# skhu101/TDNN-F_NAS

Hardware: AMD Instinct MI355X
Metric: LF-MMI training frames/sec per node (SWBD 7q TDNN-F) (higher is better)
Workload: dtype f32

## Files before the change

### include/tdnnf_hip.h

```cpp
#ifndef TDNNF_HIP_H_
#define TDNNF_HIP_H_

#include <stddef.h>
#include <stdint.h>

#ifdef __cplusplus
extern "C" {
#endif

#define TDNNF_OK 0
#define TDNNF_EINVAL 1
#define TDNNF_EHIP 2

#define TDNNF_MAX_OFFSETS 16

typedef struct {
  float *data;
  int rows, cols, stride;
} tdnnf_mat;

typedef void *tdnnf_stream;
typedef struct tdnnf_ng tdnnf_ng;

const char *tdnnf_last_error(void);
// ... 213 lines not shown
int tdnnf_align_graphs_info(const tdnnf_align_graphs *, int graph, int *num_states, int *num_arcs, int *max_in_degree);
size_t tdnnf_align_workspace_bytes(const tdnnf_align_graphs *, int num_utts, const int *utt_graph, const int *utt_frames);
int tdnnf_align_best_path(const tdnnf_align_graphs *, int num_utts, const int *utt_graph, const int *utt_frames, const int *utt_row_begin,
                          int row_stride, const tdnnf_mat *nnet_output, float acoustic_scale, int *pdf_out_dev, int *state_out_dev,
                          double *results_dev, void *workspace_dev, size_t workspace_bytes, tdnnf_stream);

int tdnnf_align_best_path_labels(const tdnnf_align_graphs *, int num_utts, const int *utt_graph, const int *utt_frames, const int *utt_row_begin,
                                 int row_stride, const tdnnf_mat *nnet_output, float acoustic_scale, int *pdf_out_dev, int *state_out_dev,
                                 int *label_out_dev, int *arc_out_dev , double *results_dev, void *workspace_dev,
                                 size_t workspace_bytes, tdnnf_stream);

size_t tdnnf_align_posteriors_workspace_bytes(const tdnnf_align_graphs *, int num_utts, const int *utt_graph, const int *utt_frames,
                                              int want_posteriors);
int tdnnf_align_posteriors(const tdnnf_align_graphs *, int num_utts, const int *utt_graph, const int *utt_frames, const int *utt_row_begin,
                           int row_stride, const tdnnf_mat *nnet_output, float acoustic_scale, float weight, tdnnf_mat *post_out ,
                           double *results_dev, void *workspace_dev, size_t workspace_bytes, tdnnf_stream);

int tdnnf_align_graphs_pdfs(const tdnnf_align_graphs *, int graph, int *num, int *pdfs_out);
int tdnnf_align_posteriors_compact_layout(const tdnnf_align_graphs *, int num_utts, const int *utt_graph, const int *utt_frames, long long *elems_out,
                                          long long *utt_begin_out);
int tdnnf_align_posteriors_compact(const tdnnf_align_graphs *, int num_utts, const int *utt_graph, const int *utt_frames, const int *utt_row_begin,
                                   int row_stride, const tdnnf_mat *nnet_output, float acoustic_scale, float weight, float *post_compact_dev,
                                   size_t post_compact_elems, double *results_dev, void *workspace_dev, size_t workspace_bytes, tdnnf_stream);

size_t tdnnf_align_posteriors_sparse_workspace_bytes(const tdnnf_align_graphs *, int num_utts, const int *utt_graph, const int *utt_frames,
                                                     int max_per_frame);
int tdnnf_align_posteriors_sparse(const tdnnf_align_graphs *, int num_utts, const int *utt_graph, const int *utt_frames, const int *utt_row_begin,
                                  int row_stride, const tdnnf_mat *nnet_output, float acoustic_scale, float weight, float min_post, int max_per_frame,
                                  int *pdf_out_dev, float *post_out_dev, int *count_out_dev, double *results_dev, void *workspace_dev,
                                  size_t workspace_bytes, tdnnf_stream);

int tdnnf_align_graphs_labels(const tdnnf_align_graphs *, int graph, int *num, int *labels_out);
int tdnnf_align_label_posteriors_compact_layout(const tdnnf_align_graphs *, int num_utts, const int *utt_graph, const int *utt_frames,
                                                long long *elems_out, long long *utt_begin_out);
int tdnnf_align_label_posteriors_compact(const tdnnf_align_graphs *, int num_utts, const int *utt_graph, const int *utt_frames,
                                         const int *utt_row_begin, int row_stride, const tdnnf_mat *nnet_output, float acoustic_scale, float weight,
                                         float *post_compact_dev, size_t post_compact_elems, double *results_dev, void *workspace_dev,
                                         size_t workspace_bytes, tdnnf_stream);
size_t tdnnf_align_label_posteriors_sparse_workspace_bytes(const tdnnf_align_graphs *, int num_utts, const int *utt_graph, const int *utt_frames,
                                                           int max_per_frame);
int tdnnf_align_label_posteriors_sparse(const tdnnf_align_graphs *, int num_utts, const int *utt_graph, const int *utt_frames,
                                        const int *utt_row_begin, int row_stride, const tdnnf_mat *nnet_output, float acoustic_scale, float weight,
                                        float min_post, int max_per_frame, int *label_out_dev, float *post_out_dev, int *count_out_dev,
                                        double *results_dev, void *workspace_dev, size_t workspace_bytes, tdnnf_stream);

int tdnnf_ng_create(int rank, int update_period, float num_samples_history, float alpha, tdnnf_ng **out);
void tdnnf_ng_destroy(tdnnf_ng *);
int tdnnf_ng_freeze(tdnnf_ng *, int freeze);
int tdnnf_ng_precondition(tdnnf_ng *, tdnnf_mat *X, float *scale_host, tdnnf_stream);
size_t tdnnf_ng_stats_pass_workspace_bytes(int rank, int Di, int num_taps, int N);
int tdnnf_ng_stats_pass(const tdnnf_tdnn_indexes *ix, const tdnnf_mat *X, int Di, const float *eff_dev, const float *WT_dev,
                        const float *W_dev, int ldw, const float *bias_dev, tdnnf_mat *H, double *sumsq_dev, int sumsq_cap, int form,
                        void *workspace_dev, size_t workspace_bytes, tdnnf_stream);
const float *tdnnf_ng_scale_dev(const tdnnf_ng *);

size_t tdnnf_constrain_orthonormal_workspace_bytes(int rows, int cols);
int tdnnf_constrain_orthonormal(float scale, float *M_dev, int rows, int cols, int ld, void *workspace_dev,
                                size_t workspace_bytes, tdnnf_stream);
int tdnnf_axpy(const float *x_dev, float a, float *y_dev, size_t n, tdnnf_stream);
int tdnnf_dot(const float *x_dev, const float *y_dev, size_t n, double *result_host, tdnnf_stream);
size_t tdnnf_max_change_workspace_bytes(int num_comp);
int tdnnf_update_with_max_change(float *params_dev, float *delta_dev, int num_comp, const long long *comp_begin_host,
                                 const float *max_change_host, float max_param_change, float max_change_scale,
                                 float scale, int zero_delta, void *workspace_dev, size_t workspace_bytes,
                                 float *info_dev, tdnnf_stream);

int tdnnf_splice_input(const tdnnf_mat *feats, const tdnnf_mat *ivectors, int num_seq, int num_splice,
                       tdnnf_mat *out, tdnnf_stream);
int tdnnf_reorder_rows(const tdnnf_mat *in, int num_seq, int rho, int to_rho, tdnnf_mat *out, tdnnf_stream);

#define TDNNF_NET_MAX_LAYERS 32
typedef struct {
  int feat_dim, ivector_dim, num_pdfs;
  int hidden_dim, prefinal_small_dim;
  int num_layers;
  int bottleneck_dim[TDNNF_NET_MAX_LAYERS];
  int time_stride[TDNNF_NET_MAX_LAYERS];
  float bypass_scale;
  int frames_per_chunk, num_sequences;
  int frame_subsampling;
  float leaky_hmm, xent_regularize, chain_l2_regularize;
  float l2_hidden, l2_output;
  float max_change_hidden, max_change_output, max_param_change;
  float relu_self_repair_scale;
  float batchnorm_stats_scale;
  int darts_num_offsets;
  int darts_flags;
  float darts_temp_proportion;
  int use_natural_gradient;
  int bn_num_choices;
  int bn_choice_dims[8];
  int bn_mode;
  float bn_flops_scale;
  float bn_temp_proportion;
  int cv_update;
  int gemm_precision;
  int use_layer_offsets;
  int offset_left[TDNNF_NET_MAX_LAYERS];
  int offset_right[TDNNF_NET_MAX_LAYERS];
  int use_dropout;
} tdnnf_net_config;
typedef struct tdnnf_net tdnnf_net;

typedef struct tdnnf_egs_reader tdnnf_egs_reader;
typedef struct tdnnf_egs_writer tdnnf_egs_writer;
typedef struct tdnnf_eg tdnnf_eg;
// ... 116 lines not shown
```

### tdnn-f_nas_amd/csrc/abi_ng.hip

```cpp
#include <stdint.h>
#include <string.h>

#include <algorithm>

#include "gemm_f32.h"
#include "ng.h"

using namespace tdnnf;

extern "C" {

const float *tdnnf_ng_scale_dev(const tdnnf_ng *ng) { return ng && ng->dev ? ng->scale_f : nullptr; }

size_t tdnnf_ng_stats_pass_workspace_bytes(int rank, int Di, int num_taps, int N) { return ng_pform_ws_bytes(pad4(rank), Di, num_taps, N) + 64; }

int tdnnf_ng_stats_pass(const tdnnf_tdnn_indexes *ix, const tdnnf_mat *X, int Di, const float *eff, const float *WT, const float *W, int ldw,
                        const float *bias, tdnnf_mat *H, double *sumsq, int sumsq_cap, int use_valu, void *workspace, size_t workspace_bytes,
                        tdnnf_stream stream) {
  TDNNF_REQUIRE(ix && X && X->data && H && H->data && Di > 0 && ix->num_offsets >= 1 && ix->num_offsets <= kMaxSeg && ix->row_stride >= 1,
                "ng_stats_pass: bad arguments");
  const int K = ix->num_offsets, N = H->rows, Rp = H->cols;
  for (int i = 0; i < K; i++)
    TDNNF_REQUIRE(ix->row_offsets[i] >= 0 && (long long)(N - 1) * ix->row_stride + ix->row_offsets[i] < X->rows && Di <= X->cols,
                  "ng_stats_pass: tap %d reads outside X (%d x %d)", i, X->rows, X->cols);
  TDNNF_REQUIRE(!sumsq || sumsq_cap >= rows_gemm_sumsq_blocks(N), "ng_stats_pass: sumsq needs %d entries", rows_gemm_sumsq_blocks(N));
  hipStream_t s = (hipStream_t)stream;
  NgInput in;
  memset(&in, 0, sizeof(in));
  in.x = view(X); in.ix = *ix; in.Di = Di; in.ones = bias ? 1 : 0; in.N = N; in.eff = eff;
  if (use_valu == 2) {
    TDNNF_REQUIRE(W && ldw >= K * Di && sumsq && H->stride == Rp && workspace && ng_pform_ok(Rp, in, workspace_bytes),
                  "ng_stats_pass: the one-pass form takes >= 2 taps of one matrix whole 128-row tiles apart, N %% 128 == 0, N >= 32768, taps x rank <= 64, no coefficients");
    return ng_pform_pass(W, Rp, ldw, bias, in, H->data, sumsq, workspace, s);
  }
  if (use_valu) {
    const NgRowdotArgs v = ng_pass_rowdot_args(WT, Rp, bias, in, H->data, H->stride, sumsq, sumsq_cap);
    TDNNF_REQUIRE(WT && ng_rowdot_ok(v), "ng_stats_pass: the vector-ALU kernel takes rank 20 / 40 / 80 and 16-byte aligned rows");
    TDNNF_HIP(ng_rowdot(v, s));
    return TDNNF_OK;
  }
  TDNNF_REQUIRE(W && ldw >= K * Di, "ng_stats_pass: the MFMA form needs W (rank x ldw)");
  GemmPrecisionScope exact_f32(2);
  TDNNF_HIP(rows_gemm(ng_pass_gemm_args(W, ldw, Rp, bias, in, H->data, H->stride, sumsq), true, s));
  return TDNNF_OK;
}

int tdnnf_ng_create(int rank, int update_period, float num_samples_history, float alpha, tdnnf_ng **out) {
  TDNNF_REQUIRE(out && rank >= 0 && update_period >= 1 && num_samples_history > 0 && alpha >= 0, "ng_create: bad configuration");
  tdnnf_ng *ng = new tdnnf_ng();
  ng->rank = rank;
  ng->Rp = 0;
  ng->update_period = update_period;
  ng->t = 0;
  ng->D = ng->Dp = 0;
  ng->frozen = 0;
  ng->num_samples_history = num_samples_history;
  ng->alpha = alpha;
  ng->epsilon = 1.0e-10f;
  ng->delta = 5.0e-04f;
  ng->rho = 0;
  ng->dev = nullptr;
  ng->pin = nullptr;
  ng->scratch = nullptr;
  ng->scratch_floats = 0;
  ng->pending = 0;
  ng->job_done = 0;
  ng->ev_job = nullptr;
  ng->ev_wait = nullptr;
  ng->must_reorth = false;
  *out = ng;
  return TDNNF_OK;
}

int tdnnf_ng_freeze(tdnnf_ng *ng, int freeze) {
  TDNNF_REQUIRE(ng, "ng_freeze: null object");
  ng->frozen = freeze ? 1 : 0;
  return TDNNF_OK;
}

void tdnnf_ng_destroy(tdnnf_ng *ng) {
  if (!ng) return;
  if (ng->pending) ng_pool_wait(ng);
  hipFree(ng->dev);
  hipHostFree(ng->pin);
  hipFree(ng->scratch);
  if (ng->ev_job) hipEventDestroy(ng->ev_job);
  delete ng;
}

int tdnnf_ng_precondition(tdnnf_ng *ng, tdnnf_mat *X, float *scale_host, tdnnf_stream stream) {
  TDNNF_REQUIRE(ng && mat_ok(X) && X->rows > 0 && X->cols > 0, "ng_precondition: bad arguments");
  hipStream_t s = (hipStream_t)stream;
  NgCallScope scope;
  if (X->cols == 1) {
    if (scale_host) *scale_host = 1.0f;
    return TDNNF_OK;
  }
// ... 37 lines not shown
```

### tdnn-f_nas_amd/csrc/abi_tdnn.hip

```cpp
#include <dlfcn.h>
#include <stdlib.h>
#include <string.h>

#include <string>

#include "common.h"
#include "gemm_f32.h"
#include "planes_gemm.h"

namespace tdnnf {

static thread_local std::string g_last_error;

void set_error(const char *fmt, ...) {
  char buf[1024];
  va_list ap;
  va_start(ap, fmt);
  vsnprintf(buf, sizeof(buf), fmt, ap);
  va_end(ap);
  g_last_error = buf;
}
int hip_status(hipError_t e, const char *what) {
  set_error("HIP error %d (%s) in %s", (int)e, hipGetErrorString(e), what);
  return TDNNF_EHIP;
// ... 4 lines not shown
  return o;
}

namespace {
typedef int (*roctx_push_t)(const char *);
typedef int (*roctx_pop_t)();
roctx_push_t g_roctx_push = nullptr;
roctx_pop_t g_roctx_pop = nullptr;
bool roctx_ready() {
  static const bool ok = [] {
    const char *e = getenv("TDNNF_ROCTX");
    if (e && atoi(e) == 0) return false;
    for (const char *lib : {"librocprofiler-sdk-roctx.so", "librocprofiler-sdk-roctx.so.1", "libroctx64.so", "libroctx64.so.4"}) {
      void *h = dlopen(lib, RTLD_NOW | RTLD_GLOBAL);
      if (!h) continue;
      g_roctx_push = (roctx_push_t)dlsym(h, "roctxRangePushA");
      g_roctx_pop = (roctx_pop_t)dlsym(h, "roctxRangePop");
      if (g_roctx_push && g_roctx_pop) return true;
    }
    return false;
  }();
  return ok;
}
}
TraceRange::TraceRange(const char *name) : on(roctx_ready()) {
  if (on) g_roctx_push(name);
}
TraceRange::~TraceRange() {
  if (on) g_roctx_pop();
}

bool tdnn_rows_ok(const tdnnf_tdnn_indexes *ix, int rows_in, int N) {
  if (!ix || ix->num_offsets < 1 || ix->num_offsets > TDNNF_MAX_OFFSETS || ix->row_stride < 1) return false;
  for (int i = 0; i < ix->num_offsets; i++) {
    const long long need = (long long)ix->row_offsets[i] + (long long)ix->row_stride * N - (ix->row_stride - 1);
    if (ix->row_offsets[i] < 0 || (N > 0 && rows_in < need)) return false;
  }
  return true;
}

}

using namespace tdnnf;

extern "C" {

const char *tdnnf_last_error(void) { return g_last_error.c_str(); }
int tdnnf_abi_version(void) { return 1; }

static int *option_slot(const char *name) {
  Options &o = options();
  if (!name) return nullptr;
  const struct { const char *n; int *p; } table[] = {{"ng_grouped", &o.ng_grouped}, {"ng_fuse", &o.ng_fuse}, {"ng_early_in", &o.ng_early_in},
                                                     {"wgrad_stream", &o.wgrad_stream}, {"gemm_ring", &o.gemm_ring}, {"planes", &o.planes}, {"den_split", &o.den_split}, {"phase_events", &o.phase_events}, {"wgrad_lag", &o.wgrad_lag}, {"ng_bk", &o.ng_bk}, {"ng_valu", &o.ng_valu}, {"ng_pform", &o.ng_pform}, {"planes_group", &o.planes_group}, {"xent_behind_den", &o.xent_behind_den}, {"ng_early_fork", &o.ng_early_fork}, {"ng_diag_skip", &o.ng_diag_skip}, {"wgrad_small", &o.wgrad_small}, {"splitk_per_cu", &o.splitk_per_cu}, {"gemm_alt_taps", &o.gemm_alt_taps}, {"reverse_passes", &o.reverse_passes}, {"splitk_partial_round", &o.splitk_partial_round}, {"wgrad_on_caller", &o.wgrad_on_caller}, {"den_mw_test_abort", &o.den_mw_test_abort}, {"planes_check_bound", &o.planes_check_bound}, {"den_gamma_pairs", &o.den_gamma_pairs}, {"num_form", &o.num_form}, {"align_form", &o.align_form}, {"align_checkpoint", &o.align_checkpoint}, {"align_path_checkpoint", &o.align_path_checkpoint}, {"num_frontier_cap", &o.num_frontier_cap}, {"gemm_arith_test", &o.gemm_arith_test}};
  for (auto &e : table)
    if (strcmp(e.n, name) == 0) return e.p;
  return nullptr;
}
int tdnnf_set_option(const char *name, int value) {
  int *p = option_slot(name);
  TDNNF_REQUIRE(p, "set_option: unknown option '%s' (ng_grouped, ng_fuse, ng_early_in, wgrad_stream, gemm_ring, planes, den_split, align_checkpoint, align_path_checkpoint)", name ? name : "(null)");
  *p = value;
  return TDNNF_OK;
}
int tdnnf_get_option(const char *name, int *value) {
  int *p = option_slot(name);
  TDNNF_REQUIRE(p && value, "get_option: unknown option '%s'", name ? name : "(null)");
  *value = *p;
  return TDNNF_OK;
}

}

namespace tdnnf {
int tdnn_propagate_impl(const tdnnf_tdnn_indexes *ix, const tdnnf_mat *in, const float *W, int ldw, int Do, int Di,
                        const float *bias, const float *eff_coef, int init_mode, int relu, tdnnf_mat *out, tdnnf_stream stream,
                        float *colstats, int *colstats_rows) {
  TDNNF_REQUIRE(mat_ok(in) && mat_ok(out) && W, "tdnn_propagate: bad matrices");
  TDNNF_REQUIRE(Do > 0 && Di > 0 && in->cols == Di && out->cols == Do, "tdnn_propagate: dims: in.cols=%d Di=%d out.cols=%d Do=%d",
                in ? in->cols : -1, Di, out ? out->cols : -1, Do);
  TDNNF_REQUIRE(tdnn_rows_ok(ix, in->rows, out->rows), "tdnn_propagate: input has too few rows for the time offsets");
  TDNNF_REQUIRE(ldw >= ix->num_offsets * Di, "tdnn_propagate: ldw < K*Di");
  TDNNF_REQUIRE(init_mode >= 0 && init_mode <= 2 && (init_mode != 1 || bias), "tdnn_propagate: init_mode 1 needs a bias");
  RowsGemmArgs a;
  memset(&a, 0, sizeof(a));
  a.A = in->data;
  a.lda = (long long)in->stride * ix->row_stride;
  a.B = W;
  a.ldb = ldw;
  a.C = out->data;
  a.ldc = out->stride;
  a.M = out->rows;
  a.N = Do;
  a.bias = bias;
  a.coef = eff_coef;
  a.init_mode = init_mode;
  a.relu = relu;
  a.colstats = colstats;
  a.colstats_rows = colstats_rows;
  a.nseg = ix->num_offsets;
  for (int i = 0; i < a.nseg; i++) {
    a.seg[i].a_off = (long long)ix->row_offsets[i] * in->stride;
    a.seg[i].b_off = (long long)i * Di;
    a.seg[i].klen = Di;
    a.seg[i].m_lo = 0;
    a.seg[i].m_hi = out->rows;
  }
// ... 201 lines not shown
```

### tdnn-f_nas_amd/csrc/common.h

```cpp
#pragma once
#include <hip/hip_runtime.h>
#include <stdarg.h>
#include <stdio.h>

#include "tdnnf_hip.h"

namespace tdnnf {

struct MatView {
  float *data;
  int rows, cols, stride;
};
inline MatView view(const tdnnf_mat *m) { return MatView{m->data, m->rows, m->cols, m->stride}; }

void set_error(const char *fmt, ...);
int hip_status(hipError_t e, const char *what);

inline bool mat_ok(const tdnnf_mat *m) {
  return m && m->rows >= 0 && m->cols >= 0 && m->stride >= m->cols && (m->data || m->rows * m->cols == 0);
}
inline bool same_dim(const tdnnf_mat *a, const tdnnf_mat *b) { return a->rows == b->rows && a->cols == b->cols; }

inline bool vec4_ok(const MatView &m) {
  return (reinterpret_cast<uintptr_t>(m.data) & 15) == 0 && m.stride % 4 == 0 && m.cols % 4 == 0;
}

#define TDNNF_REQUIRE(cond, ...)            \
  do {                                      \
    if (!(cond)) {                          \
      ::tdnnf::set_error(__VA_ARGS__);      \
      return TDNNF_EINVAL;                  \
    }                                       \
  } while (0)

#define TDNNF_HIP(expr)                                         \
  do {                                                          \
    hipError_t e__ = (expr);                                    \
    if (e__ != hipSuccess) return ::tdnnf::hip_status(e__, #expr); \
  } while (0)

#define TDNNF_LAUNCH_CHECK() TDNNF_HIP(hipGetLastError())

struct Options {
  int ng_grouped = 1;
  int ng_fuse = 1;
  int ng_early_in = 1;
  int wgrad_stream = -1;
  int gemm_ring = 1;
  int planes = 1;
  int den_mw_test_abort = 0;
  int planes_group = 1;
  int planes_check_bound = 0;
  int wgrad_lag = 3;
  int wgrad_on_caller = 0;
  int splitk_partial_round = 1;
  int reverse_passes = 0;
  int gemm_alt_taps = 1;
  int splitk_per_cu = 2;
  int wgrad_small = 0;
  int ng_bk = 0;
  int ng_early_fork = 1;
  int xent_behind_den = -1;
  int ng_pform = 1;
  int ng_valu = 0;
  int ng_diag_skip = 0;
  int phase_events = 0;
  int den_split = -1;
  int num_form = 0;
  int gemm_arith_test = 0;
  int num_frontier_cap = 0;
  int align_form = 0;
  int align_checkpoint = 0;
  int align_path_checkpoint = 0;
  int den_gamma_pairs = 0;
};
Options &options();

struct TraceRange {
  explicit TraceRange(const char *name);
  ~TraceRange();
  bool on;
};

__host__ __device__ inline float floor_keep_nan(float x, float f) { return x < f ? f : x; }

inline int grid_for(long long work, int block, int cap = 2048) {
  long long g = (work + block - 1) / block;
  if (g > cap) g = cap;
  if (g < 1) g = 1;
  return (int)g;
}
#ifdef __HIPCC__
template <class T>
struct as_given { typedef T type; };
template <class... P>
__attribute__((visibility("hidden"))) inline hipError_t launch_vec_or_scalar(bool vec, int rows, int cols, void (*k4)(P...), void (*k1)(P...), hipStream_t s, typename as_given<P>::type... args) {
  const long long work = (long long)rows * (vec ? cols / 4 : cols);
  void (*k)(P...) = vec ? k4 : k1;
  hipLaunchKernelGGL(k, dim3(grid_for(work, 256)), dim3(256), 0, s, args...);
  return hipGetLastError();
}
#endif

inline unsigned long long tdnnf_decision(unsigned long long step, unsigned long long k) {
  unsigned long long z = step * 0x9E3779B97F4A7C15ULL + k * 0xBF58476D1CE4E5B9ULL + 0x94D049BB133111EBULL;
  z = (z ^ (z >> 30)) * 0xBF58476D1CE4E5B9ULL;
  z = (z ^ (z >> 27)) * 0x94D049BB133111EBULL;
  return (z ^ (z >> 31)) >> 8;
}

bool log_softmax_propagate_with_aux(const tdnnf_mat *in, tdnnf_mat *out, tdnnf_mat *aux, float aux_scale, hipStream_t s);
float chain_supervision_weight(const tdnnf_supervision *sp);
bool chain_supervision_needs_assign(const tdnnf_supervision *sp);
size_t chain_split_region_bytes(const tdnnf_den_graph *g, int B, int T);
int chain_den(const tdnnf_den_graph *g, const tdnnf_supervision *sp, const tdnnf_mat *y, float leaky, tdnnf_mat *deriv, void *ws, hipStream_t s,
              bool beside_other_work = false, hipStream_t caller_aux = nullptr, hipEvent_t ev_recursions = nullptr, bool *ev_recorded = nullptr);
// ... 25 lines not shown
```

### tdnn-f_nas_amd/csrc/fused.h

```cpp
#pragma once
#include "common.h"

namespace tdnnf {

struct PlanesSink {
  void *P;
  long long R;
  const float *rec;
};
hipError_t bn_apply_bypass(MatView x, const float *memo, int D, int period, MatView prev, float bypass, MatView out, hipStream_t s,
                           const float *mask = nullptr, int B = 1, const PlanesSink *planes = nullptr);

struct BwdPlanes {
  void *P;
  long long R;
  int lead;
  float *rec;
};

struct NgFuse {
  const float *W;
  int Rp, ldw;
  float *H;
  double *part;
  int part_cap;
};
bool bn_relu_bwd_ng_ok(MatView x, MatView dz, MatView d_aff, int Rp);
bool bn_relu_bwd_ng_pays(int rows);

size_t bn_relu_bwd_workspace_bytes(int rows, int cols);
hipError_t bn_relu_bwd(MatView x, MatView dz, float *memo, float target_rms, bool bn_test_mode, double *relu_stats, bool store_relu_stats,
                       bool self_repair, float self_repair_scale, MatView d_aff, float *bias_acc, float bias_scale,
                       void *ws, size_t ws_bytes, hipStream_t s, const float *mask = nullptr, int B = 1,
                       const NgFuse *ng = nullptr,
                       double *oderiv_stats = nullptr,
                       const BwdPlanes *planes = nullptr);

}
```

### tdnn-f_nas_amd/csrc/fused.hip

```cpp
#include <algorithm>

#include "batchnorm.h"
#include "device.h"
#include "ew_dev.h"
#include "fused.h"
#include "gemm_f32.h"
#include "launch_forms.h"
#include "planes_gemm.h"

namespace tdnnf {
namespace {

__device__ __forceinline__ void store_planes4(const PlanesSink &pk, float ps, long long ra, int c, const float (&v)[4]) {
  typedef _Float16 h4 __attribute__((ext_vector_type(4)));
  h4 hi, lo;
#pragma unroll
  for (int j = 0; j < 4; j++) {
    const float w = v[j] * ps;
    hi[j] = (_Float16)w;
    lo[j] = (_Float16)(w - (float)hi[j]);
  }
  const int kb = c >> 4, k = c & 15, half = (k >> 3) ^ (int)((ra >> 3) & 1);
  _Float16 *dst = reinterpret_cast<_Float16 *>(pk.P) + (((long long)kb * 2) * pk.R + ra) * 16 + half * 8 + (k & 7);
  *reinterpret_cast<h4 *>(dst) = hi;
  *reinterpret_cast<h4 *>(dst + pk.R * 16) = lo;
}

template <int VEC, bool PLANES>
__global__ __launch_bounds__(256) void bn_apply_bypass_kernel(MatView x, const float *mean, const float *scale, int D, int period,
                                                              MatView prev, float bypass, MatView out, const float *mask, int B, PlanesSink pk, int rev) {
  const int cv = x.cols / VEC;
  const float ps = PLANES ? pk.rec[0] : 1.0f;
  const int ncb = PLANES ? cv / 8 : 1;
  const long long total = PLANES ? (long long)((x.rows + 7) / 8) * 8 * cv : (long long)x.rows * cv;
  for (long long e0 = blockIdx.x * 256LL + threadIdx.x; e0 < total; e0 += gridDim.x * 256LL) {
    const long long e = rev ? total - 1 - e0 : e0;
    int r, c;
    if (PLANES) {
      const long long blk = e >> 6;
      r = (int)(blk / ncb) * 8 + (int)((e >> 3) & 7);
      c = ((int)(blk % ncb) * 8 + (int)(e & 7)) * VEC;
      if (r >= x.rows) continue;
    } else {
      r = (int)(e / cv);
      c = (int)(e % cv) * VEC;
    }
    const int cd = c % period;
    if (cd >= D) continue;
    float xv[4], pv[4] = {0, 0, 0, 0}, o[4];
    ld(x.data + (long long)r * x.stride + c, xv, VEC == 4);
    if (prev.data) ld(prev.data + (long long)r * prev.stride + c, pv, VEC == 4);
    const float *mk = mask ? mask + (long long)(x.cols > D ? c / period : r % B) * D + cd : nullptr;
    float mu[4], sc[4], mv[4] = {1.f, 1.f, 1.f, 1.f};
    ld(mean + cd, mu, VEC == 4);
    ld(scale + cd, sc, VEC == 4);
    if (mk) ld(mk, mv, VEC == 4);
#pragma unroll
    for (int j = 0; j < VEC; j++) o[j] = (xv[j] - mu[j]) * sc[j] * mv[j] + bypass * pv[j];
    st(out.data + (long long)r * out.stride + c, o, VEC == 4);
    if constexpr (PLANES && VEC == 4) store_planes4(pk, ps, r, c, o);
// ... 272 lines not shown
      }
      *reinterpret_cast<float4 *>(As + (rr + 32 * i) * LD + c4 * 4) = make_float4(o[i][0], o[i][1], o[i][2], o[i][3]);
    }
#pragma unroll
    for (int j = 0; j < NT; j++) {
      const int idx = t + 256 * j, n = idx >> 3, kk = (idx & 7) * 4;
      *reinterpret_cast<float4 *>(Bs + n * LD + kk) = wv[j];
    }
    if (k0 + BK < D) request(k0 + BK);
#pragma unroll
    for (int i = 0; i < 4; i++) {
      const int r = r0 + rr + 32 * i;
      if (FULL || r < x.rows) {
        st(d_aff.data + (long long)r * d_aff.stride + col, o[i], true);
        if constexpr (PLANES) store_planes4(pk, pks, (long long)pk_lead + r, col, o[i]);
      }
    }
#pragma unroll
    for (int j = 0; j < 4; j++) {
      float v = cs[j];
      v += __shfl_xor(v, 8, 64);
      v += __shfl_xor(v, 16, 64);
      v += __shfl_xor(v, 32, 64);
      if (lane < 8) colred[wave][lane * 4 + j] = v;
    }
    __syncthreads();
    {
      const float *as = As + (wave * 32 + li) * LD + lh * 4;
      const float *bs = Bs + li * LD + lh * 4;
#pragma unroll
      for (int kg = 0; kg < BK / 8; kg++) {
        const float4 a = *reinterpret_cast<const float4 *>(as + kg * 8);
#pragma unroll
        for (int j = 0; j < NT; j++) {
          const float4 b = *reinterpret_cast<const float4 *>(bs + j * 32 * LD + kg * 8);
          acc[j] = __builtin_amdgcn_mfma_f32_32x32x2f32(a.x, b.x, acc[j], 0, 0, 0);
          acc[j] = __builtin_amdgcn_mfma_f32_32x32x2f32(a.y, b.y, acc[j], 0, 0, 0);
          acc[j] = __builtin_amdgcn_mfma_f32_32x32x2f32(a.z, b.z, acc[j], 0, 0, 0);
          acc[j] = __builtin_amdgcn_mfma_f32_32x32x2f32(a.w, b.w, acc[j], 0, 0, 0);
        }
      }
    }
    if (t < BK) partial[(long long)blk * D + k0 + t] = (colred[0][t] + colred[1][t]) + (colred[2][t] + colred[3][t]);
    __syncthreads();
  }
#pragma unroll
  for (int j = 0; j < NT; j++) {
    const int n = j * 32 + li;
#pragma unroll
    for (int e = 0; e < 16; e++) {
      const int r = r0 + wave * 32 + (e & 3) + 8 * (e >> 2) + 4 * lh;
      if (n < ng.Rp && r < x.rows) ng.H[(long long)r * ng.Rp + n] = acc[j][e];
    }
  }
  double v = ssq;
  for (int o = 32; o > 0; o >>= 1) v += __shfl_xor(v, o, 64);
  if (lane == 0) red[wave] = v;
  __syncthreads();
  if (t == 0) ng.part[blk] = (red[0] + red[1]) + (red[2] + red[3]);
  if (blk == 0)
    for (int i = gridDim.x + t; i < ng.part_cap; i += 256) ng.part[i] = 0.0;
}

template <int NT, bool MASK, bool PLANES>
__global__ __launch_bounds__(256) void bn_relu_bwd_apply_ng_kernel(MatView x, MatView dz, const float *memo, int D, const double *repair_stats,
                                                                   float self_repair_scale, MatView d_aff, float *partial, const float *mask, int B,
                                                                   NgFuse ng, PlanesSink pk, int pk_lead, int rev) {
  const int blk = rev ? (int)gridDim.x - 1 - (int)blockIdx.x : (int)blockIdx.x;
  if (blk * 128 + 128 <= x.rows)
    bn_relu_bwd_apply_ng_body<NT, MASK, true, PLANES>(x, dz, memo, D, repair_stats, self_repair_scale, d_aff, partial, mask, B, ng, pk, pk_lead, blk);
  else bn_relu_bwd_apply_ng_body<NT, MASK, false, PLANES>(x, dz, memo, D, repair_stats, self_repair_scale, d_aff, partial, mask, B, ng, pk, pk_lead, blk);
}

}

hipError_t bn_apply_bypass(MatView x, const float *memo, int D, int period, MatView prev, float bypass, MatView out, hipStream_t s, const float *mask, int B,
                           const PlanesSink *planes) {
  if (x.rows == 0) return hipSuccess;
  const bool vec = vec4_ok(x) && vec4_ok(out) && (!prev.data || vec4_ok(prev)) && D % 4 == 0 && (reinterpret_cast<uintptr_t>(memo) & 15) == 0 &&
                   (!mask || (reinterpret_cast<uintptr_t>(mask) & 15) == 0);
  const long long work = (long long)x.rows * (vec ? x.cols / 4 : x.cols);
  if (planes && !(vec && x.cols == D && D % 32 == 0 && planes->P && planes->rec)) return hipErrorInvalidValue;
  ProfHbmRange prof(4, 4.0 * x.rows * x.cols * ((prev.data ? 3.0 : 2.0) + (planes ? 1.0 : 0.0)), s);
  const PlanesSink none{nullptr, 0, nullptr};
  const int rev = vec && !planes ? options().reverse_passes & 1 : 0;
  count_fused(kFusedBypassFirst + (planes ? kFusedPlanes : vec ? kFusedVec4 : kFusedScalar) * 8 + (x.cols > D ? kFusedFlagSuper : 0) + (mask ? kFusedFlagMask : 0) +
              (rev ? kFusedFlagRev : 0));
  if (planes) hipLaunchKernelGGL((bn_apply_bypass_kernel<4, true>), dim3(grid_for((long long)((x.rows + 7) / 8) * 8 * (x.cols / 4), 256)), dim3(256), 0, s, x, memo, memo + 2 * D, D, period, prev, bypass, out, mask, B, *planes, 0);
  else if (vec) hipLaunchKernelGGL((bn_apply_bypass_kernel<4, false>), dim3(grid_for(work, 256)), dim3(256), 0, s, x, memo, memo + 2 * D, D, period, prev, bypass, out, mask, B, none, rev);
  else hipLaunchKernelGGL((bn_apply_bypass_kernel<1, false>), dim3(grid_for(work, 256)), dim3(256), 0, s, x, memo, memo + 2 * D, D, period, prev, bypass, out, mask, B, none, 0);
  return hipGetLastError();
}

bool bn_relu_bwd_ng_ok(MatView x, MatView dz, MatView d_aff, int Rp) {
  return vec4_ok(x) && vec4_ok(dz) && vec4_ok(d_aff) && x.cols % 32 == 0 && Rp >= 1 && Rp <= 96 && x.rows >= 1;
}

bool bn_relu_bwd_ng_pays(int rows) {
  const int slots = 2 * device_cus();
  const int blocks = (rows + 127) / 128, rounds = (blocks + slots - 1) / slots;
  return 4 * blocks >= 3 * rounds * slots;
}

size_t bn_relu_bwd_workspace_bytes(int rows, int cols) {
  ColReducePlan p = colreduce_plan(rows, cols);
  const size_t blocks128 = ((size_t)rows + 127) / 128;
// ... 87 lines not shown
```

### tdnn-f_nas_amd/csrc/gemm_f32.h

```cpp
#pragma once
#include <hip/hip_runtime.h>
#include <stddef.h>
#include <stdint.h>
#include <string.h>

#include <vector>

#include "prof.h"

namespace tdnnf {

constexpr int kMaxSeg = 16;

struct GemmSeg {
  long long a_off;
  long long b_off;
  int klen;
  int m_lo, m_hi;
};

struct RowsGemmArgs {
  const float *A;
  long long lda;
  const float *B;
  long long ldb;
  float *C;
  long long ldc;
  int M, N;
  const float *bias;
  const float *coef;
  int init_mode;
  int relu;
  int c_vec;
  const float *add;
  long long ldadd;
  float add_scale;
  int add_lo, add_hi;
  int ksplit;
  int kchunk;
  float *partial;
  double *sumsq;
  int sumsq_cap;
  float *colstats;
  int *colstats_rows;
  int colstats_stride;
  int prec;
  int serial_epilogue;
  int alt_seg_order;
  int nseg;
  GemmSeg seg[kMaxSeg];
  const float *col_scale;
  const float *col_offset;
  int post_add;
  const int *row_map;
};
inline bool rows_gemm_has_post(const RowsGemmArgs &a) { return a.col_scale || a.col_offset || a.post_add || a.row_map; }

struct SplitKScratchOverride {
  float *prev_buf;
  size_t prev_bytes;
  SplitKScratchOverride(float *buf, size_t bytes);
  ~SplitKScratchOverride();
};

struct GemmPrecisionScope {
  int prev;
  explicit GemmPrecisionScope(int prec);
  ~GemmPrecisionScope();
};
int gemm_precision_default();
struct TransposedWeightsScope {
  const float *prev_w, *prev_wt;
  long long prev_n;
  TransposedWeightsScope(const float *w_base, const float *wt_base, long long n);
  ~TransposedWeightsScope();
};
const float *transposed_weights(const float *W);

inline bool aligned16(const void *p) { return (reinterpret_cast<uintptr_t>(p) & 15) == 0; }

inline int rows_gemm_colstats_cap(int M) { return (M + 63) / 64 + 64; }
inline int rows_gemm_sumsq_blocks(int M) { return (M + 127) / 128 > 1024 ? (M + 127) / 128 : 1024; }

hipError_t rows_gemm(const RowsGemmArgs &args, bool b_kcontig, hipStream_t stream);
inline hipError_t rows_gemm_1seg(const float *A, long long lda, const float *B, long long ldb, bool b_kcontig, float *C, long long ldc, int M, int N, int K,
                                 int init_mode, const float *coef, double *sumsq, hipStream_t stream) {
  RowsGemmArgs a;
  memset(&a, 0, sizeof(a));
  a.A = A; a.lda = lda; a.B = B; a.ldb = ldb; a.C = C; a.ldc = ldc; a.M = M; a.N = N;
  a.init_mode = init_mode; a.coef = coef; a.sumsq = sumsq; a.nseg = 1;
  a.seg[0].klen = K; a.seg[0].m_lo = 0; a.seg[0].m_hi = M;
  return rows_gemm(a, b_kcontig, stream);
}

struct RowsGemmGroup;
// ... 28 lines not shown
```

### tdnn-f_nas_amd/csrc/launch_forms.h

```cpp
#pragma once
#include <atomic>

namespace tdnnf {

enum RowsForm {
  kFormPlain,
  kFormRing,
  kFormSplitK,
  kFormPartialS2,
  kFormPartialS8 = kFormPartialS2 + 6,
  kFormMainSplitTail,
  kFormMainPlainTail,
  kFormSumsqPlain,
  kFormSumsqSplitK,
  kFormPost,
  kFormGrouped,
  kRowsForms
};
constexpr int kRowsTiles = 9, kRowsAriths = 3;

template <int WM, int WN, int TM, int TN, int BK>
constexpr int rows_tile_index() {
  constexpr int BM = WM * TM * 32, BN = WN * TN * 32;
  constexpr int t = (BM == 128 && BN == 32 && BK == 32) ? 0 : (BM == 128 && BN == 32 && BK == 64) ? 1 : (BM == 128 && BN == 64 && BK == 32) ? 2
                  : (BM == 128 && BN == 96 && BK == 16) ? 3 : (BM == 128 && BN == 96 && BK == 32) ? 4 : (BM == 128 && BN == 160 && BK == 16) ? 5
                  : (BM == 64 && BN == 128 && BK == 16) ? 6 : (BM == 128 && BN == 128 && BK == 16) ? 7 : (BM == 128 && BN == 128 && BK == 32) ? 8 : -1;
  static_assert(t >= 0, "a rows GEMM tile without a counter: add it here and to kRowsTileNames (launch_forms.hip)");
  return t;
}
constexpr int rows_form_index(int tile, int arith, int form) { return (tile * kRowsAriths + arith) * kRowsForms + form; }

enum {
  kPlanesPlain = kRowsTiles * kRowsAriths * kRowsForms,
  kPlanesMainSplitTail,
  kPlanesMainPlainTail,
  kWgradFirst,
  kWgradPlanes = kWgradFirst + 5 * kRowsAriths,
  kWgradLastSlabs,
  kRowsLastSlices,
  kRowsVec4Launches,
  kRowsScalarLaunches,
  kPlanesAltChunked,
  kLaunchFormCounters
};

std::atomic<long long> *launch_form_counters();
inline void count_form(int index) { launch_form_counters()[index].fetch_add(1, std::memory_order_relaxed); }
inline void note_rows_slices(int ksplit) { launch_form_counters()[kRowsLastSlices].store(ksplit, std::memory_order_relaxed); }
inline void note_wgrad_slabs(int splits) { launch_form_counters()[kWgradLastSlabs].store(splits, std::memory_order_relaxed); }

enum { kFusedVec4, kFusedScalar, kFusedPlanes, kFusedKinds };
constexpr int kFusedFlagSuper = 1, kFusedFlagMask = 2, kFusedFlagRev = 4;
constexpr int kFusedNgFlagMask = 1, kFusedNgFlagPlanes = 2, kFusedNgFlagRev = 4;
enum FusedForm {
  kFusedBypassFirst,
  kFusedReduceFirst = kFusedBypassFirst + kFusedKinds * 8,
  kFusedFinalizeTrain = kFusedReduceFirst + 4,
  kFusedFinalizeTest,
  kFusedApplyFirst,
  kFusedApplyUnrolled = kFusedApplyFirst + kFusedKinds * 4,
  kFusedApplyTail,
  kFusedApplyShortChunk,
  kFusedNgFirst,
  kFusedNgPartialBlock = kFusedNgFirst + 3 * 8,
  kFusedNgFullBlocks,
  kFusedRepair,
  kFusedFormCounters
};
std::atomic<long long> *fused_form_counters();
inline void count_fused(int index) { fused_form_counters()[index].fetch_add(1, std::memory_order_relaxed); }

}
```

### tdnn-f_nas_amd/csrc/launch_forms.hip

```cpp
#include "launch_forms.h"

#include <stdio.h>

#include "common.h"

namespace tdnnf {

std::atomic<long long> *launch_form_counters() {
  static std::atomic<long long> counters[kLaunchFormCounters];
  return counters;
}

std::atomic<long long> *fused_form_counters() {
  static std::atomic<long long> counters[kFusedFormCounters];
  return counters;
}

namespace {
const char *const kFusedKindNames[kFusedKinds] = {"vec4", "scalar", "planes"};
const char *const kRowsTileNames[kRowsTiles] = {"128x32k32", "128x32k64", "128x64k32", "128x96k16", "128x96k32", "128x160k16", "64x128k16", "128x128k16", "128x128k32"};
const char *const kArithNames[kRowsAriths] = {"f32", "bf16x3", "bf16x6"};
const char *const kRowsFormNames[kRowsForms] = {"plain", "ring", "splitk", "partial_s2", "partial_s3", "partial_s4", "partial_s5", "partial_s6", "partial_s7", "partial_s8",
                                                "main_split_tail", "main_plain_tail", "sumsq_plain", "sumsq_splitk", "post", "grouped"};
const char *const kWgradTileNames[5] = {"128x128", "160x128", "128x160", "32x128", "64x64"};
}

}

using namespace tdnnf;

extern "C" {

const char *tdnnf_gemm_launch_form_name(int index) {
  static thread_local char buf[64];
  if (index < 0 || index >= kLaunchFormCounters) return nullptr;
  if (index < kPlanesPlain) {
    const int form = index % kRowsForms, arith = (index / kRowsForms) % kRowsAriths, tile = index / (kRowsForms * kRowsAriths);
    snprintf(buf, sizeof(buf), "rows.%s.%s.%s", kRowsTileNames[tile], kArithNames[arith], kRowsFormNames[form]);
  } else if (index == kPlanesPlain) {
    snprintf(buf, sizeof(buf), "planes.plain");
  } else if (index == kPlanesMainSplitTail) {
    snprintf(buf, sizeof(buf), "planes.main_split_tail");
  } else if (index == kPlanesMainPlainTail) {
    snprintf(buf, sizeof(buf), "planes.main_plain_tail");
  } else if (index < kWgradPlanes) {
    const int i = index - kWgradFirst;
    snprintf(buf, sizeof(buf), "wgrad.%s.%s", kWgradTileNames[i / kRowsAriths], kArithNames[i % kRowsAriths]);
  } else if (index == kWgradPlanes) {
    snprintf(buf, sizeof(buf), "wgrad.planes");
  } else if (index == kWgradLastSlabs) {
    snprintf(buf, sizeof(buf), "wgrad.last_slabs");
  } else if (index == kRowsLastSlices) {
    snprintf(buf, sizeof(buf), "rows.last_slices");
  } else if (index == kRowsVec4Launches) {
    snprintf(buf, sizeof(buf), "rows.launches_vec4");
  } else if (index == kRowsScalarLaunches) {
    snprintf(buf, sizeof(buf), "rows.launches_scalar");
  } else {
    snprintf(buf, sizeof(buf), "planes.alt_chunked");
  }
  return buf;
}

int tdnnf_gemm_launch_forms(long long *counts, int capacity, int reset) {
  std::atomic<long long> *c = launch_form_counters();
  for (int i = 0; i < kLaunchFormCounters; i++) {
    if (counts && i < capacity) counts[i] = c[i].load(std::memory_order_relaxed);
    if (reset) c[i].store(0, std::memory_order_relaxed);
  }
  return kLaunchFormCounters;
}

const char *tdnnf_fused_launch_form_name(int index) {
  static thread_local char buf[64];
  if (index < 0 || index >= kFusedFormCounters) return nullptr;
  if (index < kFusedReduceFirst) {
    const int i = index - kFusedBypassFirst, f = i % 8;
    snprintf(buf, sizeof(buf), "apply_bypass.%s%s%s%s", kFusedKindNames[i / 8], f & kFusedFlagSuper ? ".super" : "", f & kFusedFlagMask ? ".mask" : "",
             f & kFusedFlagRev ? ".rev" : "");
  } else if (index < kFusedFinalizeTrain) {
    const int i = index - kFusedReduceFirst;
    snprintf(buf, sizeof(buf), "bwd.reduce.%s.%s", i & 2 ? "scalar" : "vec4", i & 1 ? "stats" : "nostats");
  } else if (index == kFusedFinalizeTrain) {
    snprintf(buf, sizeof(buf), "bwd.finalize.train");
  } else if (index == kFusedFinalizeTest) {
    snprintf(buf, sizeof(buf), "bwd.finalize.test");
  } else if (index < kFusedApplyUnrolled) {
    const int i = index - kFusedApplyFirst, f = i % 4;
    snprintf(buf, sizeof(buf), "bwd.apply.%s%s%s", kFusedKindNames[i / 4], f & 1 ? ".mask" : "", f & 2 ? ".rev" : "");
  } else if (index == kFusedApplyUnrolled) {
    snprintf(buf, sizeof(buf), "bwd.apply.rows_unrolled");
  } else if (index == kFusedApplyTail) {
    snprintf(buf, sizeof(buf), "bwd.apply.rows_tail");
  } else if (index == kFusedApplyShortChunk) {
    snprintf(buf, sizeof(buf), "bwd.apply.short_last_chunk");
  } else if (index < kFusedNgPartialBlock) {
    const int i = index - kFusedNgFirst, f = i % 8;
    snprintf(buf, sizeof(buf), "bwd.apply_ng.nt%d%s%s%s", i / 8 + 1, f & kFusedNgFlagMask ? ".mask" : "", f & kFusedNgFlagPlanes ? ".planes" : "",
             f & kFusedNgFlagRev ? ".rev" : "");
  } else if (index == kFusedNgPartialBlock) {
    snprintf(buf, sizeof(buf), "bwd.apply_ng.partial_block");
  } else if (index == kFusedNgFullBlocks) {
    snprintf(buf, sizeof(buf), "bwd.apply_ng.full_blocks");
  } else {
    snprintf(buf, sizeof(buf), "bwd.repair");
  }
  return buf;
}

int tdnnf_fused_launch_forms(long long *counts, int capacity, int reset) {
  std::atomic<long long> *c = fused_form_counters();
  for (int i = 0; i < kFusedFormCounters; i++) {
// ... 8 lines not shown
```

### tdnn-f_nas_amd/csrc/net.h

```cpp
#pragma once
#include <hip/hip_runtime.h>

#include <algorithm>
#include <string>
#include <utility>
#include <vector>

#include <map>

#include "batchnorm.h"
#include "common.h"
#include "planes_gemm.h"
#include "tdnnf_hip.h"

namespace tdnnf {
struct RowsGemmGroup;
struct PlanesSplitGroup;

struct NgGroup;
struct NgFin;
struct UpdGroup;

struct Grid {
  int t0, step, n;
// ... 42 lines not shown
  int c_arch, arch_draw0;
  float *arch_p, *arch_mask, *lin_masked;
};

}

struct tdnnf_net {
  tdnnf_net_config cfg = {};
  std::vector<tdnnf::CompDesc> comps;
  long long num_params = 0;
  float *params = nullptr, *grads = nullptr;
  float *paramsT = nullptr;
  int planes_np = 0;
  struct PlaneSlot {
    void *P = nullptr, *PT = nullptr;
    size_t bytesP = 0, bytesPT = 0;
    float *scale = nullptr;
    long long last[5] = {-1, -1, -1, -1, -1};
  };
  std::map<const float *, PlaneSlot> plane_slots;
  std::vector<tdnnf::PlanesOperand> pw;
  std::vector<float *> pw_scale;
  void *planes_ws = nullptr;
  double *fro_buf = nullptr;
  int B = 0, T = 0, Tout = 0;
  tdnnf::Grid g_lda = {}, g_feat = {};
  tdnnf::Tdnn tdnn1 = {};
  std::vector<tdnnf::TdnnfLayer> layers;
  int c_lda = 0, c_prefinal_l = 0;
  struct Head {
    int c_affine = 0, c_linear = 0, c_output = 0;
    float *aff_relu = nullptr, *bn1_out = nullptr, *lin_out = nullptr, *bn2_out = nullptr, *y = nullptr;
    float *bn1_memo = nullptr, *bn2_memo = nullptr;
    double *bn1_stats = nullptr, *bn2_stats = nullptr, *relu_stats = nullptr;
  } head[2];
  float *xent_logsoftmax = nullptr;
  char *arena = nullptr;
  size_t arena_bytes = 0;
  float *lda_in = nullptr, *lda_out = nullptr, *t1_relu = nullptr, *t1_bn = nullptr;
  float *t1_bn_memo = nullptr;
  double *t1_bn_stats = nullptr, *t1_relu_stats = nullptr;
  float *prefinal_l_out = nullptr;
  float *dA = nullptr, *dB = nullptr, *dC = nullptr, *d_small = nullptr, *d_small2 = nullptr;
  float *d_y = nullptr, *d_xent = nullptr;
  float *tapgrad = nullptr;
  double *tapdots = nullptr;
  const float *draws = nullptr;
  std::vector<tdnnf_ng *> ng_in, ng_out;
  float *orthoT = nullptr;
  struct NgComp {
    float *H_in = nullptr, *H_out = nullptr, *T = nullptr, *bsum = nullptr;
    double *part_in = nullptr, *part_out = nullptr;
    int N = 0;
  };
  std::vector<NgComp> ngc;
  float *ng_bsum_all = nullptr;
  size_t ng_bsum_floats = 0;
  float *ngTmp = nullptr;
  void *ng_side_ws = nullptr;
  size_t ngset_ws_bytes = 0;
  struct NgBucket {
    int key;
    std::vector<int> comps;
    tdnnf::NgGroup *group;
  };
  std::vector<NgBucket> ng_buckets;
  std::vector<int> ng_cur;
  tdnnf::NgFin *ngfin = nullptr;
  bool ng_grouped = true;
  hipEvent_t ev_ngc = nullptr;
  hipStream_t s3 = nullptr;
  hipEvent_t ev_s3 = nullptr;
  hipEvent_t ev_fin0 = nullptr, ev_fin = nullptr;
  float *s3_scratch = nullptr;
  size_t s3_scratch_bytes = 0;
  bool wg_on = false;
  hipStream_t s4 = nullptr;
  hipEvent_t ev_pg[4] = {nullptr, nullptr, nullptr, nullptr}, ev_pg_in = nullptr;
  int wg_lag = 3;
  float *dC2 = nullptr, *dS[2] = {nullptr, nullptr};
  unsigned pg_count = 0;
  void *ws4 = nullptr;
  void *ws2 = nullptr;
  float *s2_scratch = nullptr;
  float *s4_scratch = nullptr;
  hipStream_t s5 = nullptr;
  void *ws5 = nullptr;
  float *s5_scratch = nullptr;
  struct EarlyIn {
    unsigned char xin[256];
    long long recorded = -1, done = -1;
  };
  std::vector<EarlyIn> early;
  long long fb_count = 0;
  bool early_on = false, early_any = false;
  bool early_group = false;
  tdnnf::RowsGemmGroup *early_launch = nullptr;
  tdnnf::PlanesSplitGroup *wsplit_group = nullptr;
  hipEvent_t ev_early_in = nullptr, ev_early = nullptr;
  size_t s4_scratch_bytes = 0;
  bool wg_two = false;
  float *gtmp = nullptr;
  std::vector<char> oderiv_nonzero_own;
  std::vector<char> *oderiv_nonzero = &oderiv_nonzero_own;
  tdnnf::BnSync bn_sync{nullptr, nullptr, nullptr, 1};
  enum { kPhases = 8 };
// ... 83 lines not shown
```

### tdnn-f_nas_amd/csrc/net_arena.hip

```cpp
#include <string>

#include "common.h"
#include "fused.h"
#include "gemm_f32.h"
#include "gemm_ring.h"
#include "net_model.h"
#include "ng.h"

namespace tdnnf {
namespace {

struct Rows {
  int N0, No;
  int max_rows;
  int max_lin_rows;
  int big_rows() const { return std::max(max_rows, std::max(N0, No)); }
};
Rows rows_of(const tdnnf_net *n) {
  Rows r{N_of(n->g_lda, n->B), n->Tout * n->B, 0, 0};
  r.max_rows = r.N0;
  for (auto &L : n->layers) {
    r.max_rows = std::max(r.max_rows, std::max(N_of(L.gout, n->B), N_of(L.gin, n->B)));
    r.max_lin_rows = std::max(r.max_lin_rows, N_of(L.lin.out, n->B));
  }
  return r;
}
float *small_mat(const tdnnf_net *n, Arena &A, const Rows &r) {
  return A.mat(std::max(r.max_lin_rows, r.No), std::max(n->cfg.prefinal_small_dim, 512));
}
size_t bsum_floats(const CompDesc &cd) { return ((size_t)cd.rows + 15) & ~(size_t)15; }

void take_activations(tdnnf_net *n, Arena &A, const Rows &r) {
  const tdnnf_net_config &c = n->cfg;
  const int B = n->B, Hd = c.hidden_dim, S = c.prefinal_small_dim, P = c.num_pdfs;
  const int lda_dim = 3 * c.feat_dim + c.ivector_dim;
  n->lda_in = A.mat(r.N0, lda_dim);
  n->lda_out = A.mat(r.N0, lda_dim);
  n->t1_relu = A.mat(r.N0, Hd);
  n->t1_bn = A.mat(r.N0, Hd);
  n->t1_bn_memo = A.take<float>(bn_memo_floats(Hd));
  n->t1_bn_stats = A.take<double>(bn_stats_doubles(Hd));
  n->t1_relu_stats = A.take<double>(relu_stats_doubles(Hd));
  for (auto &L : n->layers) {
    const int nl = N_of(L.lin.out, B), no = N_of(L.gout, B);
    L.lin_out = A.mat(nl, L.bn);
    L.lin_perm = L.perm ? A.mat(nl, L.bn) : nullptr;
    L.arch_p = L.arch_mask = L.lin_masked = nullptr;
    if (L.c_arch >= 0) {
      L.arch_p = A.take<float>(8);
      L.arch_mask = A.take<float>(L.bn + 4);
      L.lin_masked = A.mat(nl, L.bn);
    }
    L.relu_out = A.mat(no, Hd);
    L.noop_out = A.mat(no, Hd);
    L.bn_memo = A.take<float>(bn_memo_floats(Hd));
    L.lin.memo = L.lin.darts ? A.take<float>(2 * TDNNF_MAX_OFFSETS) : nullptr;
    L.aff.memo = L.aff.darts ? A.take<float>(2 * TDNNF_MAX_OFFSETS) : nullptr;
    L.lin.active = L.lin.darts ? A.take<int>(TDNNF_MAX_OFFSETS + 1) : nullptr;
    L.aff.active = L.aff.darts ? A.take<int>(TDNNF_MAX_OFFSETS + 1) : nullptr;
    L.bn_stats = A.take<double>(bn_stats_doubles(Hd));
// ... 87 lines not shown
  slot(n->dC, r.big_rows(), Hd, true);
  slot(n->d_small, small_rows, small_cols, true);
  slot(n->d_small2, small_rows, small_cols, true);
  n->planes_ws = A.take<char>(planes_sumsq_ws_bytes() + 64);
  n->fro_buf = A.take<double>(finalize_grid(std::max(Hd, S)) + 8);
  for (size_t i = 0; i < n->comps.size(); i++) {
    const CompDesc &cd = n->comps[i];
    if (cd.plain || cd.rows < 2 || (int)i == n->c_lda) continue;
    PlanesOperand &o = n->pw[i];
    o.rows = cd.rows; o.cols = cd.cols; o.ld = cd.cols; o.np = np; o.lead = 0;
    o.R = planes_slot_t_rows(cd.rows);
    o.Rt = planes_slot_t_rows(cd.cols);
    o.P = A.take<char>(planes_bytes(np, o.R, planes_kblocks(cd.cols)) + 64);
    o.PT = A.take<char>(planes_bytes(np, o.Rt, planes_t_kblocks(cd.rows)) + 64);
    n->pw_scale[i] = A.take<float>(4);
    o.scale = n->pw_scale[i];
  }
}

size_t take_ortho_transpose(tdnnf_net *n, Arena &A) {
  size_t tall = 0, tall_ws = 0;
  for (auto &cd : n->comps)
    if (cd.orthonormal != 0.f && cd.rows > cd.cols) {
      tall = std::max(tall, (size_t)cd.rows * cd.cols);
      tall_ws = std::max(tall_ws, tdnnf_constrain_orthonormal_workspace_bytes(cd.cols, cd.rows));
    }
  n->orthoT = tall ? A.take<float>(tall + 16) : nullptr;
  return tall_ws;
}

size_t take_natural_gradient(tdnnf_net *n, Arena &A, const Rows &r) {
  n->s3_scratch = nullptr;
  n->s3_scratch_bytes = 0;
  n->ng_grouped = options().ng_grouped != 0;
  n->ngc.assign(n->comps.size(), tdnnf_net::NgComp());
  if (!n->cfg.use_natural_gradient) return 0;
  size_t ng_ws = 0, mtmp = 0;
  for (const WeightComp &w : weight_comps(n)) {
    const CompDesc &cd = n->comps[w.comp];
    if (!cd.updatable || cd.plain) continue;
    const int Dx = cd.cols + (cd.has_bias ? 1 : 0), ldT = (Dx + 3) & ~3, rows = w.rows_out;
    int rank_in, rank_out;
    ng_ranks(cd, &rank_in, &rank_out);
    const int Rpi = (rank_in + 3) & ~3, Rpo = (rank_out + 3) & ~3;
    mtmp = std::max(mtmp, std::max((size_t)cd.rows * Rpi, (size_t)Rpo * ldT));
    ng_ws = std::max(ng_ws, std::max(ng_stats_workspace_bytes(rank_in, Dx, w.K, rows), ng_stats_workspace_bytes(rank_out, cd.rows, 1, rows)));
    auto &C = n->ngc[w.comp];
    C.N = rows;
    C.H_in = A.take<float>((size_t)rows * Rpi + 64);
    C.H_out = A.take<float>((size_t)rows * Rpo + 64);
    C.T = A.take<float>((size_t)cd.rows * ldT + 16);
    C.part_in = A.take<double>((size_t)rows_gemm_sumsq_blocks(rows) + 8);
    C.part_out = A.take<double>((size_t)rows_gemm_sumsq_blocks(rows) + 8);
  }
  size_t tot = 0;
  for (size_t i = 0; i < n->comps.size(); i++)
    if (n->ngc[i].N > 0) tot += bsum_floats(n->comps[i]);
  n->ng_bsum_floats = tot;
  n->ng_bsum_all = A.take<float>(tot + 16);
  size_t o = 0;
  for (size_t i = 0; i < n->comps.size(); i++)
    if (n->ngc[i].N > 0) {
      n->ngc[i].bsum = n->ng_bsum_all ? n->ng_bsum_all + o : nullptr;
      o += bsum_floats(n->comps[i]);
    }
  n->ngset_ws_bytes = wgrad_workspace_bytes(80, 80, 1, r.big_rows()) + 256;
  n->ngTmp = A.take<float>(mtmp + 64);
  n->ng_side_ws = A.take<char>(n->ngset_ws_bytes);
  n->s3_scratch_bytes = 16u << 20;
  n->s3_scratch = A.take<float>(n->s3_scratch_bytes / sizeof(float));
  return ng_ws;
}

void take_workspace(tdnnf_net *n, Arena &A, const Rows &r, size_t ng_ws, size_t tall_ws) {
  const tdnnf_net_config &c = n->cfg;
  const int Hd = c.hidden_dim, S = c.prefinal_small_dim, P = c.num_pdfs;
  size_t ws = 0;
  auto upd = [&](size_t b) { ws = std::max(ws, b); };
  for (const WeightComp &w : weight_comps(n)) {
    const CompDesc &cd = n->comps[w.comp];
    upd(wgrad_workspace_bytes(cd.rows, cd.cols / w.K, w.K, w.rows_out));
  }
  upd(colreduce_bytes(r.max_rows, Hd));
  upd(sizeof(float) * 2 * (size_t)Hd * rows_gemm_colstats_cap(r.big_rows()));
  upd(bn_relu_bwd_workspace_bytes(r.max_rows, Hd));
  for (auto &L : n->layers) upd(tdnnf_constrain_orthonormal_workspace_bytes(L.bn, L.lin.K * Hd));
  upd(colreduce_bytes(r.No, P));
  upd(tdnnf_constrain_orthonormal_workspace_bytes(S, Hd));
  upd(tdnnf_max_change_workspace_bytes((int)n->comps.size()));
  upd(ng_ws);
  upd(tall_ws);
  if (c.bn_num_choices > 0) upd(sizeof(float) * (size_t)((r.max_lin_rows + 511) / 512 + 1) * 512);
  n->ws_bytes = ws + 256;
  n->ws = A.take<char>(n->ws_bytes);
}

void take_side_streams(tdnnf_net *n, Arena &A) {
  n->early_on = n->cfg.use_natural_gradient && n->ng_grouped && (options().ng_early_in >= 2 || (options().ng_early_in != 0 && !n->wg_on));
  n->early_group = n->early_on && n->wg_on && options().ng_early_in == 3;
  const bool s4_used = n->wg_on || n->early_on;
  n->ws4 = s4_used ? A.take<char>(n->ws_bytes) : nullptr;
  n->s4_scratch_bytes = s4_used ? (32u << 20) : 0;
  n->s4_scratch = s4_used ? A.take<float>(n->s4_scratch_bytes / sizeof(float)) : nullptr;
  const bool two = n->wg_on && options().wgrad_stream != 1;
  n->ws2 = two ? A.take<char>(n->ws_bytes) : nullptr;
  n->s2_scratch = two ? A.take<float>(n->s4_scratch_bytes / sizeof(float)) : nullptr;
// ... 44 lines not shown
```

### tdnn-f_nas_amd/csrc/net_step_grad.hip

```cpp
#include "net_step.h"

namespace tdnnf {
namespace {
__global__ void add_scaled_taps_kernel(const float *G, const float *coef, float *acc, int Do, int KDi, int Di) {
  const long long total = (long long)Do * KDi;
  for (long long e = blockIdx.x * 256LL + threadIdx.x; e < total; e += gridDim.x * 256LL) acc[e] += coef[(e % KDi) / Di] * G[e];
}
__global__ void scaled_taps_to_kernel(const float *G, const float *coef, int Do, int KDi, int Di, float *T, int ldT) {
  const long long total = (long long)Do * KDi;
  for (long long e = blockIdx.x * 256LL + threadIdx.x; e < total; e += gridDim.x * 256LL) {
    const int o = (int)(e / KDi), c = (int)(e % KDi);
    T[(size_t)o * ldT + c] = (coef ? coef[c / Di] : 1.0f) * G[e];
  }
}
__global__ void commit_grads_kernel(float *grads, const float *gtmp, long long n, const double *results) {
  if (results[5] == 0.0) return;
  for (long long i = blockIdx.x * 256LL + threadIdx.x; i < n; i += gridDim.x * 256LL) grads[i] += gtmp[i];
}
}

int Step::wait_last_wgrads(hipStream_t st, unsigned streams) {
  for (unsigned b = 1; b <= streams && b <= n->pg_count; b++) TDNNF_HIP(hipStreamWaitEvent(st, n->ev_pg[(n->pg_count - b) & 3], 0));
  return TDNNF_OK;
}
float *Step::bias_target(int comp) const {
  if (n->comps[comp].lr_factor == 0.f) return nullptr;
  if (!use_ng) return net_Bg(n, comp);
  return n->ngc[comp].bsum;
}
Step::WgradSide Step::wgrad_side(bool on_caller) const {
  if (!n->wg_on || on_caller) return {s, n->ws, nullptr};
  const int ns = (n->wg_two ? 2 : 1) + (n->s5 ? 1 : 0), k = (int)(n->pg_count % (unsigned)ns);
  if (k == 0) return {n->s4, n->ws4, n->s4_scratch};
  if (k == 1 && n->wg_two) return {n->s2, n->ws2, n->s2_scratch};
  return {n->s5, n->ws5, n->s5_scratch};
}
int Step::handed_off(hipStream_t sw, bool on_caller) {
  if (!n->wg_on || on_caller) return TDNNF_OK;
  TDNNF_HIP(hipEventRecord(n->ev_pg[n->pg_count & 3], sw));
  const unsigned lag = lag3 ? 3u : 1u;
  if (n->pg_count >= lag) TDNNF_HIP(hipStreamWaitEvent(s, n->ev_pg[(n->pg_count - lag) & 3], 0));
  n->pg_count++;
  return TDNNF_OK;
}
int Step::param_grad(int comp, const tdnnf_tdnn_indexes &ix, int K, int Di, int Do, tdnnf_mat *x, tdnnf_mat *dyv, const float *eff, bool bias_done,
                     const int *active, int max_active, bool from_tapgrad) {
  const int ldw = K * Di;
  float *bias_acc = net_Bg(n, comp);
  if (n->comps[comp].lr_factor == 0.f) return TDNNF_OK;
  const bool on_caller = n->wg_on && options().wgrad_on_caller != 0 && n->early_any && !den_joined;
  if (on_caller) caller_used = true;
  const WgradSide side = wgrad_side(on_caller);
  const hipStream_t sw = side.st;
  void *const wsw = side.ws;
  if (n->wg_on && !on_caller) CK(record_wait(n->ev_pg_in, s, sw));
  SplitKScratchOverride sw_scratch(side.scratch, side.scratch ? n->s4_scratch_bytes : 0);
  if (!use_ng) {
    CK(tdnn_update_simple_impl(&ix, x, dyv, Do, Di, eff, 1.0f, net_Wg(n, comp), ldw, bias_done ? nullptr : bias_acc, wsw, n->ws_bytes, active, max_active, sw));
    return handed_off(sw, on_caller);
  }
  const int N = dyv->rows, ones = bias_acc ? 1 : 0, Dx = ldw + ones, ldT = (Dx + 3) & ~3;
  auto &C = n->ngc[comp];
  TDNNF_REQUIRE(C.T && C.N == N, "net_forward_backward: component %s has no natural-gradient buffers for %d rows", n->comps[comp].name.c_str(), N);
  float *T = C.T;
  const bool grouped = n->ng_grouped && ng_dim(n->ng_in[comp]) != 0 && ng_dim(n->ng_out[comp]) != 0;
  const bool overwrite = !from_tapgrad && !active && eff == nullptr && (ones || ldT == ldw);
  if (!overwrite) TDNNF_HIP(hipMemsetAsync(T, 0, sizeof(float) * (size_t)Do * ldT, sw));
  if (from_tapgrad)
    hipLaunchKernelGGL(scaled_taps_to_kernel, dim3(grid_for((long long)Do * ldw, 256)), dim3(256), 0, sw, n->tapgrad, eff, Do, ldw, Di, T, ldT);
  else
    CK(tdnn_update_simple_impl(&ix, x, dyv, Do, Di, eff, 1.0f, T, ldT, nullptr, wsw, n->ws_bytes, active, max_active, sw, overwrite));
  if (ones) {
    if (!bias_done) TDNNF_HIP(colsum_add(view(dyv), 1.0f, C.bsum, wsw, sw));
    if (!grouped) ng_set_column(C.bsum, Do, T, ldT, ldw, sw);
  }
  NgInput xin;
  memset(&xin, 0, sizeof(xin));
  xin.x = view(x); xin.ix = ix; xin.Di = Di; xin.ones = ones; xin.N = N; xin.eff = eff; xin.active = active; xin.max_active = max_active;
  static_assert(sizeof(NgInput) <= sizeof(tdnnf_net::EarlyIn::xin), "EarlyIn::xin too small");
  if (n->early_on && n->early[comp].done == n->fb_count) {
    TDNNF_REQUIRE(memcmp(n->early[comp].xin, &xin, sizeof(xin)) == 0, "net_forward_backward: the input of component %s moved between minibatches",
                  n->comps[comp].name.c_str());
    if (n->early_group) {
      TDNNF_HIP(hipStreamWaitEvent(sw, n->ev_early, 0));
      CK(ng_stats_main_finish(n->ng_in[comp], xin, C.H_in, wsw, n->ws_bytes, sw));
    }
  } else {
    CK(ng_stats_main(n->ng_in[comp], xin, C.H_in, C.part_in, wsw, n->ws_bytes, sw));
  }
  if (n->early_on) {
    memcpy(n->early[comp].xin, &xin, sizeof(xin));
    n->early[comp].recorded = n->fb_count;
  }
  NgInput yin;
  memset(&yin, 0, sizeof(yin));
  yin.x = view(dyv); yin.ix.row_stride = 1; yin.ix.num_offsets = 1; yin.Di = Do; yin.N = N;
  if (fused_comp == comp) {
    fused_comp = -1;
    CK(ng_stats_main_finish(n->ng_out[comp], yin, C.H_out, wsw, n->ws_bytes, sw));
  } else {
    CK(ng_stats_main(n->ng_out[comp], yin, C.H_out, C.part_out, wsw, n->ws_bytes, sw));
  }
  if (grouped) {
    n->ng_cur.push_back(comp);
  } else {
    CK(record_wait(n->ev_ngc, sw, n->s3));
    SplitKScratchOverride side_scratch(n->s3_scratch, n->s3_scratch_bytes);
    CK(ng_chain_one(n->ng_in[comp], n->ng_out[comp], C.H_in, C.part_in, C.H_out, C.part_out, T, Do, Dx, ldT, ldw, net_Wg(n, comp), bias_acc,
                    n->ng_side_ws, n->ngset_ws_bytes, n->ngTmp, n->s3));
  }
  CK(handed_off(sw, on_caller));
  if (from_tapgrad && n->wg_on) TDNNF_HIP(hipStreamWaitEvent(s, n->ev_pg[(n->pg_count - 1) & 3], 0));
  return TDNNF_OK;
}
int Step::affine_grad(int comp, const PlanesOperand &p_dy, const PlanesOperand &p_x, tdnnf_mat *x, tdnnf_mat *dyv, bool bias_done) {
  PlanesHintScope ph(hint_of(p_dy), hint_of(p_x));
  return param_grad(comp, ix1, 1, x->cols, dyv->cols, x, dyv, nullptr, bias_done, nullptr, 0, false);
}
int Step::tdnn_wgrad(Tdnn &td, const PlanesOperand &p_dy, const PlanesOperand &p_x, tdnnf_mat *x, tdnnf_mat *dyv, const float *eff, bool bias_done) {
  PlanesHintScope ph(hint_of(p_dy), hint_of(p_x));
  const int ldw = td.K * td.Di;
  bool tap_ready = false;
  if (td.darts && !(c.darts_flags & TDNNF_DARTS_UNIFORM_SAMPLE)) {
    tap_ready = true;
    TDNNF_HIP(hipMemsetAsync(n->tapgrad, 0, sizeof(float) * (size_t)td.Do * ldw, s));
    CK(tdnnf_tdnn_update_simple(&td.ix, x, dyv, td.Do, td.Di, nullptr, 1.0f, n->tapgrad, ldw, nullptr, n->ws, n->ws_bytes, s));
    CK(tdnnf_tdnn_darts_alpha_update(n->tapgrad, ldw, net_W(n, td.comp), ldw, td.Do, td.Di, td.K, td.memo, c.darts_flags, td.share,
                                     c.darts_temp_proportion, 1.0f, net_Ag(n, td.comp), n->tapdots, s));
    if (!use_ng) {
      hipLaunchKernelGGL(add_scaled_taps_kernel, dim3(grid_for((long long)td.Do * ldw, 256)), dim3(256), 0, s, n->tapgrad, eff,
                         net_Wg(n, td.comp), td.Do, ldw, td.Di);
      if (!bias_done) TDNNF_HIP(colsum_add(view(dyv), 1.0f, net_Bg(n, td.comp), n->ws, s));
      return TDNNF_OK;
    }
  }
  const bool compact = two_taps(td);
  return param_grad(td.comp, td.ix, td.K, td.Di, td.Do, x, dyv, eff, bias_done, compact ? td.active : nullptr, compact ? 2 : 0, tap_ready);
}
int Step::close_bucket(int key) {
  if (use_ng) CK(ng_close(key));
  for (auto &gb : n->buckets) {
    if (gb.close_key != key) continue;
    hipStream_t cs = s;
    if (!use_ng && n->wg_on && n->pg_count > 0) CK(wait_last_wgrads(s, side_streams()));
    if (use_ng) {
      CK(record_wait(gb.handoff, s, n->s3));
      cs = n->s3;
    }
    const long long cnt = gb.end - gb.begin;
    if (cnt > 0)
      hipLaunchKernelGGL(commit_grads_kernel, dim3(grid_for(cnt, 256)), dim3(256), 0, cs, n->grads + gb.begin, n->gtmp + gb.begin, cnt, results);
    TDNNF_HIP(hipEventRecord(gb.ready, cs));
  }
  return TDNNF_OK;
// ... 21 lines not shown
      early_refresh = early_refresh || did;
    }
  }
  if (early_refresh) TDNNF_HIP(hipEventRecord(n->ev_fin, n->s3));
  return TDNNF_OK;
}
int Step::finish_refreshes() {
  if (use_ng && n->ng_grouped) {
    if (!n->ngfin) {
      bool ready = false;
      for (tdnnf_ng *g : all_ng()) ready = ready || ng_dim(g) != 0;
      if (ready) CK(ng_fin_create(all_ng(), &n->ngfin));
    }
    if (n->ngfin) {
      int did = 0;
      SplitKScratchOverride side_scratch(n->s3_scratch, n->s3_scratch_bytes);
      CK(ng_fin_run(n->ngfin, n->s3, true, &did));
      if (did) {
        TDNNF_HIP(hipEventRecord(n->ev_fin, n->s3));
        early_refresh = true;
      }
    }
  }
  if (early_refresh) TDNNF_HIP(hipStreamWaitEvent(s, n->ev_fin, 0));
  return TDNNF_OK;
}
bool Step::is_head_comp(int comp) const {
  return comp == n->c_prefinal_l || comp == n->head[0].c_affine || comp == n->head[0].c_linear || comp == n->head[0].c_output ||
         comp == n->head[1].c_affine || comp == n->head[1].c_linear || comp == n->head[1].c_output;
}
bool Step::early_eligible(int comp, int which) const {
  const auto &E = n->early[comp];
  if (E.done == n->fb_count || (which == 0 && is_head_comp(comp))) return false;
  if (E.recorded != n->fb_count - 1 || !n->ng_in[comp] || !n->ng_out[comp] || ng_dim(n->ng_in[comp]) == 0 || ng_dim(n->ng_out[comp]) == 0) return false;
  return n->comps[comp].lr_factor != 0.f && n->ngc[comp].H_in;
}
int Step::launch_early_in(int which) {
  if (!(use_ng && n->early_on)) return TDNNF_OK;
  std::vector<int> who;
  for (int comp = (int)n->comps.size() - 1; comp >= 0; comp--)
    if (early_eligible(comp, which)) who.push_back(comp);
  if (who.empty()) return TDNNF_OK;
  CK(record_wait(n->ev_early_in, s, n->s4));
  if (early_refresh) TDNNF_HIP(hipStreamWaitEvent(n->s4, n->ev_fin, 0));
  NgInput xin;
  if (n->early_group) {
    std::vector<RowsGemmArgs> calls;
    std::vector<int> grouped;
    for (int comp : who) {
      memcpy(&xin, n->early[comp].xin, sizeof(xin));
      RowsGemmArgs a;
      CK(ng_stats_main_prepare(n->ng_in[comp], xin, n->ngc[comp].H_in, n->ngc[comp].part_in, n->s4, &a));
      if (!rows_gemm_group_ok(a)) continue;
      calls.push_back(a);
      grouped.push_back(comp);
    }
    if (calls.empty()) return TDNNF_OK;
    TDNNF_HIP(rows_gemm_group(calls, &n->early_launch, n->s4));
    for (int comp : grouped) n->early[comp].done = n->fb_count;
  } else {
    SplitKScratchOverride early_scratch(n->s4_scratch, n->s4_scratch_bytes);
    for (int comp : who) {
      memcpy(&xin, n->early[comp].xin, sizeof(xin));
      CK(ng_stats_main(n->ng_in[comp], xin, n->ngc[comp].H_in, n->ngc[comp].part_in, n->ws4, n->ws_bytes, n->s4));
      n->early[comp].done = n->fb_count;
    }
  }
  TDNNF_HIP(hipEventRecord(n->ev_early, n->s4));
  n->early_any = true;
  return TDNNF_OK;
}
int Step::out_stats_fuse(int comp, MatView xv, MatView dzv, MatView dv, NgFuse &f) {
  fused_comp = -1;
  if (!c.use_natural_gradient || n->ng_out.empty() || !n->ng_out[comp] || n->comps[comp].lr_factor == 0.f) return 0;
  if (options().ng_fuse == 0) return 0;
  const bool fuse_always = options().ng_fuse == 2;
  auto &C = n->ngc[comp];
  const float *W = nullptr;
  int Rp = 0, ldw = 0;
  CK(ng_external_begin(n->ng_out[comp], dv.cols, &W, &Rp, &ldw, s));
  if (!W || !bn_relu_bwd_ng_ok(xv, dzv, dv, Rp) || !(fuse_always || bn_relu_bwd_ng_pays(dv.rows))) return 0;
  f.W = W; f.Rp = Rp; f.ldw = ldw; f.H = C.H_out; f.part = C.part_out; f.part_cap = rows_gemm_sumsq_blocks(dv.rows);
  fused_comp = comp;
  return 1;
}
int Step::ng_close(int key) {
  if (n->ng_cur.empty()) return TDNNF_OK;
  bool closes = false;
  for (auto &gb : n->buckets) closes = closes || gb.close_key == key;
  if (!closes) return TDNNF_OK;
  tdnnf_net::NgBucket *nb = nullptr;
  for (auto &b : n->ng_buckets)
    if (b.key == key) nb = &b;
  if (!nb) {
    std::vector<NgGroupComp> gc;
    for (int comp : n->ng_cur) {
      const CompDesc &cd = n->comps[comp];
      auto &C = n->ngc[comp];
      NgGroupComp g;
      g.in = n->ng_in[comp]; g.out = n->ng_out[comp];
      g.T = C.T; g.Do = cd.rows; g.ldw = cd.cols; g.Dx = cd.cols + (cd.has_bias ? 1 : 0); g.ldT = (g.Dx + 3) & ~3;
      g.bsum = cd.has_bias ? C.bsum : nullptr;
      g.H_in = C.H_in; g.H_out = C.H_out; g.part_in = C.part_in; g.part_out = C.part_out; g.N = C.N;
      g.W_acc = net_Wg(n, comp); g.bias_acc = net_Bg(n, comp);
      gc.push_back(g);
    }
    NgGroup *grp = nullptr;
    CK(ng_group_create(gc, &grp));
    n->ng_buckets.push_back(tdnnf_net::NgBucket{key, n->ng_cur, grp});
    nb = &n->ng_buckets.back();
  }
  TDNNF_REQUIRE(nb->comps == n->ng_cur, "net_forward_backward: the components of gradient bucket %d changed between minibatches", key);
  if (n->wg_on && n->pg_count > 0) {
    CK(wait_last_wgrads(n->s3, side_streams()));
    if (caller_used) CK(record_wait(n->ev_ngc, s, n->s3));
    caller_used = false;
  } else {
    CK(record_wait(n->ev_ngc, s, n->s3));
  }
  if (n->early_any) TDNNF_HIP(hipStreamWaitEvent(n->s3, n->ev_early, 0));
  CK(ng_group_run(nb->group, n->s3));
  n->ng_cur.clear();
  return TDNNF_OK;
}

}
```

### tdnn-f_nas_amd/csrc/ng.h

```cpp
#pragma once
#include <hip/hip_runtime.h>
#include <stddef.h>

#include <vector>

#include "common.h"
#include "gemm_f32.h"
#include "tdnnf_hip.h"

struct tdnnf_ng {
  int rank, Rp, update_period, t, D, Dp, frozen;
  float num_samples_history, alpha, epsilon, delta, rho;
  std::vector<float> d;
  float *dev;
  float *W, *WT, *WWT, *wlast, *J, *W1, *Kd, *Ld, *Ad, *coeff, *tmpR, *neg_one, *scale_f;
  double *scal;
  float *pin;
  float *h_K, *h_L, *h_At, *h_coeff, *h_scale;
  double *h_tr0;
  float *scratch;
  size_t scratch_floats;
  int pending, job_done, job_N;
  hipEvent_t ev_job;
  hipEvent_t ev_wait;
  int device;
  bool cur_upd;
  int cur_N, cur_ones;
  std::vector<float> d_next;
  float rho_next;
  bool must_reorth;
  std::vector<double> sqrt_e1, inv_sqrt_e1;
};

#define TDNNF_NG_LOCAL __attribute__((visibility("hidden")))

namespace tdnnf {

inline int pad4(int x) { return (x + 3) & ~3; }
inline size_t pad4z(size_t x) { return (x + 3) & ~(size_t)3; }

struct NgCallScope {
  ProfClassOverride prof_as_ng{3};
  GemmPrecisionScope exact_f32{2};
};

struct NgInput {
  MatView x;
  tdnnf_tdnn_indexes ix;
  int Di, ones, N;
  const float *eff;
  const int *active;
  int max_active;
};

constexpr int kWtPadRows = 64;
struct NgRowdotArgs {
  const float *X;
  long long ldx;
  int row_stride;
  int nseg, Di;
  long long seg_off[16];
  const float *eff;
  const float *WT;
  int Rp;
  const float *bias;
  float *H;
  int ldh, N;
  double *part;
  int part_cap;
};
bool ng_rowdot_ok(const NgRowdotArgs &a);
hipError_t ng_rowdot(const NgRowdotArgs &a, hipStream_t s);

size_t ng_stats_workspace_bytes(int rank, int D, int K, int N);
int ng_stats_step(tdnnf_ng *ng, const NgInput &in, float *H, void *ws, size_t ws_bytes, hipStream_t s);
int ng_stats_main(tdnnf_ng *ng, const NgInput &in, float *H, double *part, void *ws, size_t ws_bytes, hipStream_t s);
int ng_stats_side(tdnnf_ng *ng, const float *H, const double *part, void *ws, size_t ws_bytes, hipStream_t s);
int ng_stats_main_prepare(tdnnf_ng *ng, const NgInput &in, float *H, double *part, hipStream_t s, RowsGemmArgs *out);
int ng_stats_main_finish(tdnnf_ng *ng, const NgInput &in, const float *H, void *ws, size_t ws_bytes, hipStream_t s);
int ng_finalize_if_ready(tdnnf_ng *ng, hipStream_t s, int *did);
int ng_external_begin(tdnnf_ng *ng, int D, const float **W, int *Rp, int *ldw, hipStream_t s);
int ng_dim(const tdnnf_ng *ng);

size_t ng_project_tmp_floats(const tdnnf_ng *in, const tdnnf_ng *out, int Do, int ldT);
int ng_project(tdnnf_ng *in, tdnnf_ng *out, float *T, int Do, int Dx, int ldT, float *tmp, hipStream_t s);

TDNNF_NG_LOCAL void ng_set_column(const float *v, int rows, float *T, int ldT, int col, hipStream_t s);
TDNNF_NG_LOCAL int ng_chain_one(tdnnf_ng *in, tdnnf_ng *out, const float *H_in, const double *part_in, const float *H_out, const double *part_out,
                                float *T, int Do, int Dx, int ldT, int ldw, float *W_acc, float *bias_acc, void *side_ws, size_t side_ws_bytes, float *tmp, hipStream_t s);

inline bool ng_updating(const tdnnf_ng *ng) { return !ng->frozen && (ng->t <= 10 || (ng->t - 10) % ng->update_period == 0); }
TDNNF_NG_LOCAL int ng_init_default(tdnnf_ng *ng, int D, hipStream_t s);
TDNNF_NG_LOCAL int ng_finalize(tdnnf_ng *ng, hipStream_t s);
TDNNF_NG_LOCAL void ng_refresh_submit(tdnnf_ng *ng, int N, hipEvent_t wait_event);
TDNNF_NG_LOCAL void ng_refresh_installed(tdnnf_ng *ng);
TDNNF_NG_LOCAL RowsGemmArgs ng_pass_gemm_args(const float *W, int ldw, int Rp, const float *bias, const NgInput &in, float *H, int ldh, double *part);
TDNNF_NG_LOCAL NgRowdotArgs ng_pass_rowdot_args(const float *WT, int Rp, const float *bias, const NgInput &in, float *H, int ldh, double *part,
                                                int part_cap);
TDNNF_NG_LOCAL size_t ng_pform_ws_bytes(int Rp, int Di, int K, int N);
TDNNF_NG_LOCAL bool ng_pform_ok(int Rp, const NgInput &in, size_t ws_bytes);
TDNNF_NG_LOCAL int ng_pform_pass(const float *W, int Rp, int ldw, const float *bias, const NgInput &in, float *H, double *part, void *ws, hipStream_t s);


struct NgGroupComp {
  tdnnf_ng *in, *out;
  float *T;
  int Do, Dx, ldT, ldw;
  const float *bsum;
  const float *H_in, *H_out;
  const double *part_in, *part_out;
  int N;
  float *W_acc, *bias_acc;
};
struct NgGroup;
int ng_group_create(const std::vector<NgGroupComp> &comps, NgGroup **out);
void ng_group_destroy(NgGroup *g);
int ng_group_run(NgGroup *g, hipStream_t s);
struct NgFin;
int ng_fin_create(const std::vector<tdnnf_ng *> &objs, NgFin **out);
void ng_fin_destroy(NgFin *f);
int ng_fin_run(NgFin *f, hipStream_t s, bool wait, int *did);
void ng_pool_wait(tdnnf_ng *ng);
bool ng_pool_done(tdnnf_ng *ng);
int ng_finalize_one(tdnnf_ng *ng, hipStream_t s);

}
```

### tdnn-f_nas_amd/csrc/ng_group.hip

```cpp
#include <math.h>
#include <string.h>

#include <algorithm>
#include <vector>

#include "gemm_f32.h"
#include "ggemm.h"
#include "ng.h"
#include "ng_group_kernels.h"

namespace tdnnf {

struct NgGroup {
  std::vector<NgGroupComp> comps;
  std::vector<tdnnf_ng *> objs;
  char *dev = nullptr;
  PairDesc *pairs = nullptr;
  CompDesc *cdesc = nullptr;
  float *lpart = nullptr;
  int npairs = 0, nslabs = 0, commit_blocks = 0;
  size_t l_lds = 0;
  DevList stage[4], kstage;
  hipEvent_t ev_staged = nullptr;
};

int ng_group_create(const std::vector<NgGroupComp> &comps, NgGroup **out) {
  TDNNF_REQUIRE(out && !comps.empty(), "ng_group_create: no components");
  NgGroup *g = new NgGroup();
  g->comps = comps;
  std::vector<PairDesc> pairs;
  std::vector<CompDesc> cdesc;
  GemmList st[4], kst;
  size_t qp_floats = 0;
  std::vector<size_t> q_off, p_off;
  int slab_total = 0, blk = 0;
  for (const NgGroupComp &c : comps) {
    TDNNF_REQUIRE(c.in && c.out && c.in->D == c.Dx && c.in->Dp == c.ldT && c.out->D == c.Do && c.in->rank > 0 && c.out->rank > 0 && c.in->Rp <= 96 &&
                      c.out->Rp <= 96 && c.N > 0,
                  "ng_group_create: a preconditioner is not initialised for its component (or its rank is outside 1..96)");
    q_off.push_back(qp_floats);
    qp_floats += ((size_t)c.Do * c.in->Rp + 63) & ~(size_t)63;
    p_off.push_back(qp_floats);
    qp_floats += ((size_t)c.out->Rp * c.ldT + 63) & ~(size_t)63;
    for (int side = 0; side < 2; side++) {
      tdnnf_ng *ng = side == 0 ? c.in : c.out;
      g->objs.push_back(ng);
      PairDesc p;
      memset(&p, 0, sizeof(p));
      p.H = side == 0 ? c.H_in : c.H_out;
      p.part = side == 0 ? c.part_in : c.part_out;
      p.Ld = ng->Ld;
      p.WWT = ng->WWT;
      p.scal = ng->scal;
      p.scale_f = ng->scale_f;
      p.Kd = ng->Kd;
      TDNNF_HIP(hipHostGetDevicePointer((void **)&p.hK, ng->h_K, 0));
      TDNNF_HIP(hipHostGetDevicePointer((void **)&p.hL, ng->h_L, 0));
      TDNNF_HIP(hipHostGetDevicePointer((void **)&p.h_tr0, ng->h_tr0, 0));
      p.ones_term = (side == 0 && c.bsum) ? (double)c.N : 0.0;
      p.N = c.N;
      p.Rp = ng->Rp;
      p.nt = (ng->Rp + 31) / 32;
      p.npart = rows_gemm_sumsq_blocks(c.N);
      int rps = std::max(256, (c.N + 31) / 32);
      rps = (rps + 7) & ~7;
      p.rows_per_slab = rps;
      p.nslab = (c.N + rps - 1) / rps;
      p.slab0 = slab_total;
      slab_total += p.nslab;
      pairs.push_back(p);
      kst.add(ng->J, ng->Dp, 1, ng->J, 1, ng->Dp, ng->Kd, ng->Rp, ng->Rp, ng->Rp, ng->Dp, 1.0f, 0);
    }
    CompDesc d;
    memset(&d, 0, sizeof(d));
    d.T = c.T;
    d.bsum = c.bsum;
    d.sa = c.in->scale_f;
    d.sb = c.out->scale_f;
    d.W_acc = c.W_acc;
    d.bias_acc = c.bias_acc;
    d.Do = c.Do;
    d.ldT = c.ldT;
    d.ldw = c.ldw;
    d.Dx = c.Dx;
    d.blk0 = blk;
    blk += (int)(((long long)c.Do * c.Dx + 1023) / 1024);
    cdesc.push_back(d);
  }
  g->npairs = (int)pairs.size();
  g->nslabs = slab_total;
  g->commit_blocks = blk;
  size_t bytes = 0;
  bytes = carve_room(bytes, sizeof(PairDesc) * pairs.size());
  bytes = carve_room(bytes, sizeof(CompDesc) * cdesc.size());
  bytes = carve_room(bytes, sizeof(float) * (size_t)slab_total * kLSlabFloats);
  bytes = carve_room(bytes, sizeof(float) * qp_floats);
  auto build = [&](float *qp) {
    for (auto &l : st) l = GemmList();
    for (size_t i = 0; i < comps.size(); i++) {
      const NgGroupComp &c = comps[i];
      float *Q = qp + q_off[i], *P = qp + p_off[i];
      const int Rx = c.in->Rp, Ry = c.out->Rp;
      st[0].add(c.T, c.ldT, 1, c.in->WT, Rx, 1, Q, Rx, c.Do, Rx, c.Dx, 1.0f, 0);
      st[1].add(Q, Rx, 1, c.in->W, c.in->Dp, 1, c.T, c.ldT, c.Do, c.ldT, Rx, -1.0f, 1);
      st[2].add(c.out->W, c.out->Dp, 1, c.T, c.ldT, 1, P, c.ldT, Ry, c.ldT, c.Do, 1.0f, 0);
      st[3].add(c.out->WT, Ry, 1, P, c.ldT, 1, c.T, c.ldT, c.Do, c.ldT, Ry, -1.0f, 1);
    }
  };
  build(nullptr);
  GemmList *lists[5] = {&st[0], &st[1], &st[2], &st[3], &kst};
  DevList *dls[5] = {&g->stage[0], &g->stage[1], &g->stage[2], &g->stage[3], &g->kstage};
  bytes = devlists_room(bytes, lists, 5) + 1024;
  if (hipMalloc((void **)&g->dev, bytes) != hipSuccess) {
    set_error("ng_group_create: cannot allocate %zu bytes", bytes);
    delete g;
    return TDNNF_EHIP;
  }
  char *cur = g->dev;
  g->pairs = carve<PairDesc>(cur, pairs.size());
  g->cdesc = carve<CompDesc>(cur, cdesc.size());
  g->lpart = carve<float>(cur, (size_t)slab_total * kLSlabFloats);
  float *qp = carve<float>(cur, qp_floats);
  build(qp);
  int rc = devlists_upload(cur, lists, dls, 5);
  if (rc) return rc;
  TDNNF_HIP(hipMemcpy(g->pairs, pairs.data(), sizeof(PairDesc) * pairs.size(), hipMemcpyHostToDevice));
  TDNNF_HIP(hipMemcpy(g->cdesc, cdesc.data(), sizeof(CompDesc) * cdesc.size(), hipMemcpyHostToDevice));
  TDNNF_HIP(hipEventCreateWithFlags(&g->ev_staged, hipEventDisableTiming | hipEventBlockingSync));
  g->l_lds = sizeof(float) * 2 * kLSlabFloats;
  static bool attr_done = false;
  if (!attr_done) {
    (void)hipFuncSetAttribute((const void *)ng_l_partial_kernel, hipFuncAttributeMaxDynamicSharedMemorySize, (int)g->l_lds);
    attr_done = true;
  }
  *out = g;
  return TDNNF_OK;
}

void ng_group_destroy(NgGroup *g) {
  if (!g) return;
  for (tdnnf_ng *ng : g->objs)
    if (ng->pending && ng->ev_wait == g->ev_staged) ng_pool_wait(ng);
  if (g->ev_staged) (void)hipEventDestroy(g->ev_staged);
  (void)hipFree(g->dev);
  delete g;
}

int ng_group_run(NgGroup *g, hipStream_t s) {
  TDNNF_REQUIRE(g, "ng_group_run: null group");
  const int nc = (int)g->comps.size();
  const bool upd = g->objs[0]->cur_upd;
  for (tdnnf_ng *ng : g->objs)
    TDNNF_REQUIRE(ng->cur_upd == upd && ng->cur_N > 0 && !ng->pending, "ng_group_run: the group's preconditioners are out of step");
  hipLaunchKernelGGL(ng_set_columns_kernel, dim3(nc), dim3(256), 0, s, g->cdesc);
  hipLaunchKernelGGL(ng_l_partial_kernel, dim3(g->nslabs), dim3(256), g->l_lds, s, g->pairs, g->npairs, g->lpart);
  hipLaunchKernelGGL(ng_l_finish_kernel, dim3(g->npairs), dim3(1024), 0, s, g->pairs, g->lpart);
  if (upd) {
    int rc = launch_list(g->kstage, s);
    if (rc) return rc;
    hipLaunchKernelGGL(ng_stage_kernel, dim3(g->npairs), dim3(256), 0, s, g->pairs);
    TDNNF_HIP(hipEventRecord(g->ev_staged, s));
  }
  for (int i = 0; i < 4; i++) {
    int rc = launch_list(g->stage[i], s);
    if (rc) return rc;
  }
  hipLaunchKernelGGL(ng_commit_group_kernel, dim3(g->commit_blocks), dim3(256), 0, s, g->cdesc, nc);
  TDNNF_LAUNCH_CHECK();
  for (tdnnf_ng *ng : g->objs) {
    if (upd) ng_refresh_submit(ng, ng->cur_N, g->ev_staged);
    ng->cur_N = 0;
    ng->t += 1;
  }
  return TDNNF_OK;
}

struct NgFin {
  std::vector<tdnnf_ng *> objs;
  char *dev = nullptr;
  FinDesc *fd = nullptr;
  int nf = 0, blocks = 0;
  DevList w1, wwt;
};

int ng_fin_create(const std::vector<tdnnf_ng *> &objs_in, NgFin **out) {
  TDNNF_REQUIRE(out, "ng_fin_create: null argument");
  NgFin *f = new NgFin();
  for (tdnnf_ng *ng : objs_in)
    if (ng && ng->rank > 0 && ng->D != 0) f->objs.push_back(ng);
  std::vector<FinDesc> fd;
  GemmList w1, wwt;
  int blk = 0;
  for (tdnnf_ng *ng : f->objs) {
    FinDesc d;
    d.J = ng->J; d.W = ng->W; d.W1 = ng->W1; d.WT = ng->WT; d.wlast = ng->wlast;
    TDNNF_HIP(hipHostGetDevicePointer((void **)&d.h_coeff, ng->h_coeff, 0));
    d.Rp = ng->Rp; d.D = ng->D; d.Dp = ng->Dp;
    d.blk0 = blk;
    blk += (int)(((long long)ng->Rp * ng->Dp + 1023) / 1024);
    fd.push_back(d);
    float *hAt = nullptr;
    TDNNF_HIP(hipHostGetDevicePointer((void **)&hAt, ng->h_At, 0));
    w1.add(hAt, ng->Rp, 1, ng->J, ng->Dp, 1, ng->W1, ng->Dp, ng->Rp, ng->Dp, ng->Rp, 1.0f, 0);
    wwt.add(ng->W, ng->Dp, 1, ng->W, 1, ng->Dp, ng->WWT, ng->Rp, ng->Rp, ng->Rp, ng->Dp, 1.0f, 0);
  }
  f->nf = (int)fd.size();
  f->blocks = blk;
  if (f->nf == 0) {
    *out = f;
    return TDNNF_OK;
  }
  GemmList *lists[2] = {&w1, &wwt};
  DevList *dls[2] = {&f->w1, &f->wwt};
  const size_t bytes = devlists_room(carve_room(0, sizeof(FinDesc) * fd.size()), lists, 2) + 1024;
  if (hipMalloc((void **)&f->dev, bytes) != hipSuccess) {
    set_error("ng_fin_create: cannot allocate %zu bytes", bytes);
    delete f;
    return TDNNF_EHIP;
  }
  char *cur = f->dev;
  f->fd = carve<FinDesc>(cur, fd.size());
  int rc = devlists_upload(cur, lists, dls, 2);
  if (rc) return rc;
  TDNNF_HIP(hipMemcpy(f->fd, fd.data(), sizeof(FinDesc) * fd.size(), hipMemcpyHostToDevice));
  *out = f;
  return TDNNF_OK;
}
// ... 43 lines not shown
```

### tdnn-f_nas_amd/csrc/ng_group_kernels.h

```cpp
#pragma once
#include <hip/hip_runtime.h>
#include <math.h>

#include "ggemm.h"

namespace tdnnf {
namespace {

struct PairDesc {
  const float *H;
  const double *part;
  float *Ld;
  const float *WWT;
  double *scal;
  float *scale_f;
  const float *Kd;
  float *hK, *hL;
  double *h_tr0;
  double ones_term;
  int N, Rp, nt, npart;
  int slab0, nslab, rows_per_slab;
};
__device__ __forceinline__ int ntile_pairs(int nt) { return nt * (nt + 1) / 2; }
constexpr int kLSlabFloats = 6 * 1024;

template <auto Start, class Desc>
__device__ __forceinline__ int last_start_le(const Desc *d, int n, int blk) {
  int lo = 0, hi = n - 1;
  while (lo < hi) {
    const int mid = (lo + hi + 1) >> 1;
    if (d[mid].*Start <= blk) lo = mid;
    else hi = mid - 1;
  }
  return lo;
}

template <int NT>
__device__ __forceinline__ void l_partial_body(const PairDesc &p, int slab, float *partial, float *lds) {
  constexpr int NP = NT * (NT + 1) / 2;
  const int t = threadIdx.x, lane = t & 63, wave = t >> 6, li = lane & 31, lh = lane >> 5;
  const int Rp = p.Rp, r0 = slab * p.rows_per_slab, r1 = min(p.N, r0 + p.rows_per_slab);
  f32x16 acc[NP];
#pragma unroll
  for (int q = 0; q < NP; q++)
#pragma unroll
    for (int r = 0; r < 16; r++) acc[q][r] = 0.f;
  bool cv[NT];
#pragma unroll
  for (int c = 0; c < NT; c++) cv[c] = c * 32 + li < Rp;
  constexpr int U = 4;
  for (int base = r0 + 2 * wave; base < r1; base += 8 * U) {
    float a[U][NT];
#pragma unroll
    for (int u = 0; u < U; u++) {
      const int row = base + 8 * u + lh;
      const float *h = p.H + (size_t)row * Rp + li;
#pragma unroll
      for (int c = 0; c < NT; c++) a[u][c] = (row < r1 && cv[c]) ? h[c * 32] : 0.f;
    }
#pragma unroll
    for (int u = 0; u < U; u++) {
      int q = 0;
#pragma unroll
      for (int i = 0; i < NT; i++)
#pragma unroll
        for (int j = i; j < NT; j++, q++) acc[q] = __builtin_amdgcn_mfma_f32_32x32x2f32(a[u][i], a[u][j], acc[q], 0, 0, 0);
    }
  }
  float *mine = lds + (size_t)(wave & 1) * NP * 1024;
  if (wave >= 2) {
#pragma unroll
    for (int q = 0; q < NP; q++)
#pragma unroll
      for (int r = 0; r < 16; r++) mine[(q * 16 + r) * 64 + lane] = acc[q][r];
  }
  __syncthreads();
  if (wave < 2) {
#pragma unroll
    for (int q = 0; q < NP; q++)
#pragma unroll
      for (int r = 0; r < 16; r++) acc[q][r] += mine[(q * 16 + r) * 64 + lane];
  }
  __syncthreads();
  if (wave == 1) {
#pragma unroll
    for (int q = 0; q < NP; q++)
#pragma unroll
      for (int r = 0; r < 16; r++) lds[(q * 16 + r) * 64 + lane] = acc[q][r];
  }
  __syncthreads();
  if (wave == 0) {
    float *out = partial + (size_t)(p.slab0 + slab) * kLSlabFloats;
#pragma unroll
    for (int q = 0; q < NP; q++)
#pragma unroll
      for (int r = 0; r < 16; r++) out[(q * 16 + r) * 64 + lane] = acc[q][r] + lds[(q * 16 + r) * 64 + lane];
  }
}

__global__ __launch_bounds__(256) void ng_l_partial_kernel(const PairDesc *pairs, int npairs, float *partial) {
  extern __shared__ float lds[];
  const PairDesc &p = pairs[last_start_le<&PairDesc::slab0>(pairs, npairs, (int)blockIdx.x)];
  const int slab = blockIdx.x - p.slab0;
  if (p.nt == 1) l_partial_body<1>(p, slab, partial, lds);
  else if (p.nt == 2) l_partial_body<2>(p, slab, partial, lds);
  else l_partial_body<3>(p, slab, partial, lds);
}

__global__ __launch_bounds__(1024) void ng_l_finish_kernel(const PairDesc *pairs, const float *partial) {
  __shared__ double red[3][16];
  const PairDesc &p = pairs[blockIdx.x];
  const int t = threadIdx.x, Rp = p.Rp, nt = p.nt;
  double a = 0, b = 0, c = 0;
  for (int i = t; i < p.npart; i += 1024) a += p.part[i];
  int q = 0;
  for (int ti = 0; ti < nt; ti++)
    for (int tj = ti; tj < nt; tj++, q++) {
      const int e = t, r = e >> 6, lane = e & 63;
      const int m = ti * 32 + (r & 3) + 8 * (r >> 2) + 4 * (lane >> 5), n = tj * 32 + (lane & 31);
      if (m >= Rp || n >= Rp) continue;
      const float *src = partial + (size_t)p.slab0 * kLSlabFloats + (size_t)q * 1024 + e;
      float v = 0.f;
      int s = 0;
      for (; s + 7 < p.nslab; s += 8) {
        float w[8];
#pragma unroll
        for (int u = 0; u < 8; u++) w[u] = src[(size_t)(s + u) * kLSlabFloats];
#pragma unroll
        for (int u = 0; u < 8; u++) v += w[u];
      }
      for (; s < p.nslab; s++) v += src[(size_t)s * kLSlabFloats];
      p.Ld[m * Rp + n] = v;
      const double w = (double)v * (double)p.WWT[m * Rp + n];
      if (ti != tj) {
        p.Ld[n * Rp + m] = v;
        c += 2.0 * w;
      } else {
        c += w;
        if (m == n) b += v;
      }
    }
  for (int o = 32; o > 0; o >>= 1) {
    a += __shfl_xor(a, o, 64);
    b += __shfl_xor(b, o, 64);
    c += __shfl_xor(c, o, 64);
  }
  if ((t & 63) == 0) {
    red[0][t >> 6] = a;
    red[1][t >> 6] = b;
    red[2][t >> 6] = c;
  }
  __syncthreads();
  if (t == 0) {
    double tr0 = p.ones_term, trL = 0, trLW = 0;
    for (int w = 0; w < 16; w++) {
      tr0 += red[0][w];
      trL += red[1][w];
      trLW += red[2][w];
    }
    const double tr1 = tr0 - 2.0 * trL + trLW;
    p.scal[0] = tr0;
    p.scal[1] = tr1;
    *p.scale_f = (tr0 <= 0.0 || !(tr1 > 0.0)) ? 1.0f : (float)sqrt(tr0 / tr1);
  }
}

__global__ __launch_bounds__(256) void ng_stage_kernel(const PairDesc *pairs) {
  const PairDesc &p = pairs[blockIdx.x];
  const int n = p.Rp * p.Rp;
  for (int i = threadIdx.x; i < n; i += 256) {
    p.hK[i] = p.Kd[i];
    p.hL[i] = p.Ld[i];
  }
  if (threadIdx.x == 0) *p.h_tr0 = p.scal[0];
}

struct CompDesc {
  float *T;
  const float *bsum, *sa, *sb;
  float *W_acc, *bias_acc;
  int Do, ldT, ldw, Dx;
  int blk0;
};
__global__ __launch_bounds__(256) void ng_set_columns_kernel(const CompDesc *comps) {
// ... 62 lines not shown
```

### tdnn-f_nas_amd/csrc/ng_kernels.h

```cpp
#pragma once
#include <hip/hip_runtime.h>

#include "gemm_f32.h"

namespace tdnnf {
namespace {

__global__ void stack_taps_kernel(const float *W, int Rp, int Dp, int Di, int K, float *WP) {
  const long long total = (long long)K * Rp * Di;
  for (long long e = blockIdx.x * 256LL + threadIdx.x; e < total; e += gridDim.x * 256LL) {
    const int k = (int)(e % Di), ir = (int)(e / Di), i = ir / Rp, r = ir % Rp;
    WP[e] = W[(size_t)r * Dp + (size_t)i * Di + k];
  }
}
struct PformTaps {
  int K, o[kMaxSeg];
};
__global__ __launch_bounds__(256) void pform_combine_kernel(const float *P, int ldp, PformTaps tp, int Rp, const float *bias, float *H, int N,
                                                            const double *psum, double *part, int part_cap) {
  const int m0 = blockIdx.x * 128, per = Rp / 4;
  for (int e = threadIdx.x; e < 128 * per; e += 256) {
    const int m = m0 + e / per, q = e % per;
    if (m >= N) break;
    float4 v = make_float4(0.f, 0.f, 0.f, 0.f);
    if (bias) v = *reinterpret_cast<const float4 *>(bias + 4 * q);
    for (int i = 0; i < tp.K; i++) {
      const float4 t = *reinterpret_cast<const float4 *>(P + (size_t)(m + tp.o[i]) * ldp + i * Rp + 4 * q);
      v.x += t.x; v.y += t.y; v.z += t.z; v.w += t.w;
    }
    *reinterpret_cast<float4 *>(H + (size_t)m * Rp + 4 * q) = v;
  }
  if (threadIdx.x == 0) {
    double sacc = 0;
    for (int i = 0; i < tp.K; i++) sacc += psum[blockIdx.x + tp.o[i] / 128];
    part[blockIdx.x] = sacc;
  }
  for (int i = gridDim.x + blockIdx.x * 256 + threadIdx.x; i < part_cap; i += gridDim.x * 256) part[i] = 0.0;
}
__global__ void scatter_col_kernel(const float *v, int R, float *J, int ld, int col) {
  const int r = blockIdx.x * blockDim.x + threadIdx.x;
  if (r < R) J[(size_t)r * ld + col] = v[r];
}
__global__ __launch_bounds__(256) void ng_scalars_kernel(const double *partial, int nb, double ones_term, const float *L, const float *WWT,
                                                         int Rp, double *scal, float *scale_f) {
  __shared__ double red[3][4];
  double a = 0, b = 0, c = 0;
  for (int i = threadIdx.x; i < nb; i += 256) a += partial[i];
  for (int i = threadIdx.x; i < Rp * Rp; i += 256) {
    const double l = L[i];
    c += l * (double)WWT[i];
    if (i / Rp == i % Rp) b += l;
  }
  for (int o = 32; o > 0; o >>= 1) {
    a += __shfl_xor(a, o, 64);
    b += __shfl_xor(b, o, 64);
    c += __shfl_xor(c, o, 64);
  }
  if ((threadIdx.x & 63) == 0) {
    red[0][threadIdx.x >> 6] = a;
    red[1][threadIdx.x >> 6] = b;
    red[2][threadIdx.x >> 6] = c;
  }
  __syncthreads();
  if (threadIdx.x == 0) {
    const double tr0 = (red[0][0] + red[0][1]) + (red[0][2] + red[0][3]) + ones_term;
    const double trL = (red[1][0] + red[1][1]) + (red[1][2] + red[1][3]);
    const double trLW = (red[2][0] + red[2][1]) + (red[2][2] + red[2][3]);
    const double tr1 = tr0 - 2.0 * trL + trLW;
    scal[0] = tr0;
    scal[1] = tr1;
    *scale_f = (tr0 <= 0.0 || !(tr1 > 0.0)) ? 1.0f : (float)sqrt(tr0 / tr1);
  }
}

__global__ void set_column_kernel(const float *v, int rows, float *T, int ldT, int col) {
  const int r = blockIdx.x * blockDim.x + threadIdx.x;
  if (r < rows) {
    T[(size_t)r * ldT + col] = v[r];
    for (int c = col + 1; c < ldT; c++) T[(size_t)r * ldT + c] = 0.f;
  }
}
__global__ void ng_commit_kernel(const float *T, int ldT, int Do, int ldw, const float *sa, const float *sb, float *W_acc, float *bias_acc) {
  const float sc = sa[0] * sb[0];
// ... 13 lines not shown
```

### tdnn-f_nas_amd/csrc/ng_stats.hip

```cpp
#include <string.h>

#include <algorithm>

#include "gemm_f32.h"
#include "ng.h"
#include "ng_kernels.h"

namespace tdnnf {
namespace {

size_t part_bytes(int N) { return ((size_t)rows_gemm_sumsq_blocks(N) * sizeof(double) + 63) & ~(size_t)63; }
size_t stats_ws_bytes(int Rp, int Di, int K, int N) {
  return part_bytes(N) + std::max(std::max(wgrad_workspace_bytes(Rp, Rp, 1, N), wgrad_workspace_bytes(Rp, Di, K, N)), ng_pform_ws_bytes(Rp, Di, K, N));
}

constexpr int kPformSpanCap = 4096;
struct TapSpan {
  int lo, hi;
};
TapSpan tap_span(const tdnnf_tdnn_indexes &ix) {
  TapSpan t{ix.row_offsets[0], ix.row_offsets[0]};
  for (int i = 1; i < ix.num_offsets; i++) {
    t.lo = std::min(t.lo, ix.row_offsets[i]);
    t.hi = std::max(t.hi, ix.row_offsets[i]);
  }
  return t;
}

}

size_t ng_pform_ws_bytes(int Rp, int Di, int K, int N) {
  if (K < 2 || K * Rp > 64) return 0;
  const size_t M = (size_t)N + kPformSpanCap;
  return sizeof(float) * ((size_t)K * Rp * Di + 64) + sizeof(float) * (M * K * Rp + 64) + sizeof(double) * ((size_t)rows_gemm_sumsq_blocks((int)M) + 8) + 256;
}
bool ng_pform_ok(int Rp, const NgInput &in, size_t ws_bytes) {
  const int K = in.ix.num_offsets, N = in.N;
  if (!options().ng_pform || K < 2 || K * Rp > 64 || in.eff || in.active || in.ix.row_stride != 1 || N % 128 != 0 || N < 32768) return false;
  const TapSpan sp = tap_span(in.ix);
  for (int i = 0; i < K; i++)
    if ((in.ix.row_offsets[i] - sp.lo) % 128 != 0) return false;
  if (sp.hi - sp.lo > kPformSpanCap || in.Di % 4 != 0 || (in.x.stride % 4) != 0 || in.Di < 1024) return false;
  return ws_bytes >= ng_pform_ws_bytes(Rp, in.Di, K, N);
}
int ng_pform_pass(const float *W, int Rp, int ldw, const float *bias, const NgInput &in, float *H, double *part, void *ws, hipStream_t s) {
  const int K = in.ix.num_offsets, N = in.N, Di = in.Di;
  const TapSpan sp = tap_span(in.ix);
  PformTaps tp;
  memset(&tp, 0, sizeof(tp));
  tp.K = K;
  for (int i = 0; i < K; i++) tp.o[i] = in.ix.row_offsets[i] - sp.lo;
  const int M = N + (sp.hi - sp.lo);
  float *WP = (float *)ws;
  float *P = WP + (((size_t)K * Rp * Di + 63) & ~(size_t)63);
  double *psum = (double *)(P + (((size_t)M * K * Rp + 63) & ~(size_t)63));
  hipLaunchKernelGGL(stack_taps_kernel, dim3(grid_for((long long)K * Rp * Di, 256)), dim3(256), 0, s, W, Rp, ldw, Di, K, WP);
  TDNNF_HIP(rows_gemm_1seg(in.x.data + (size_t)sp.lo * in.x.stride, in.x.stride, WP, Di, true, P, K * Rp, M, K * Rp, Di, 2, nullptr, psum, s));
  hipLaunchKernelGGL(pform_combine_kernel, dim3(N / 128), dim3(256), 0, s, P, K * Rp, tp, Rp, bias, H, N, psum, part,
                     rows_gemm_sumsq_blocks(N));
  TDNNF_HIP(hipGetLastError());
  return TDNNF_OK;
}

RowsGemmArgs ng_pass_gemm_args(const float *W, int ldw, int Rp, const float *bias, const NgInput &in, float *H, int ldh, double *part) {
  const int N = in.N, K = in.ix.num_offsets, Di = in.Di;
  RowsGemmArgs a;
  memset(&a, 0, sizeof(a));
  a.A = in.x.data; a.lda = (long long)in.x.stride * in.ix.row_stride; a.B = W; a.ldb = ldw; a.C = H; a.ldc = ldh; a.M = N; a.N = Rp;
  a.bias = bias;
  a.init_mode = bias ? 1 : 2;
  a.coef = in.eff;
  a.sumsq = part;
  a.nseg = K;
  for (int i = 0; i < K; i++) {
    a.seg[i].a_off = (long long)in.ix.row_offsets[i] * in.x.stride;
    a.seg[i].b_off = (long long)i * Di;
    a.seg[i].klen = Di;
    a.seg[i].m_lo = 0;
    a.seg[i].m_hi = N;
  }
  return a;
}
NgRowdotArgs ng_pass_rowdot_args(const float *WT, int Rp, const float *bias, const NgInput &in, float *H, int ldh, double *part, int part_cap) {
  const int K = in.ix.num_offsets;
  NgRowdotArgs v;
  memset(&v, 0, sizeof(v));
  v.X = in.x.data; v.ldx = in.x.stride; v.row_stride = in.ix.row_stride; v.nseg = K; v.Di = in.Di; v.eff = in.eff; v.WT = WT; v.Rp = Rp;
  v.bias = bias; v.H = H; v.ldh = ldh; v.N = in.N; v.part = part; v.part_cap = part_cap;
  for (int i = 0; i < K; i++) v.seg_off[i] = (long long)in.ix.row_offsets[i] * in.x.stride;
  return v;
}

namespace {

const float *ones_column(const tdnnf_ng *ng, const NgInput &in) { return in.ones ? ng->wlast : nullptr; }

int stats_after_h(tdnnf_ng *ng, const NgInput &in, const float *H, void *wg_ws, size_t wg_bytes, bool upd, hipStream_t s) {
  const int N = in.N, K = in.ix.num_offsets, Di = in.Di, Rp = ng->Rp, Dp = ng->Dp, D = ng->D;
  ng->cur_upd = upd;
  ng->cur_N = N;
  ng->cur_ones = in.ones;
  if (!upd) return TDNNF_OK;
  TDNNF_REQUIRE(wg_ws && wg_bytes >= wgrad_workspace_bytes(Rp, Di, K, N), "ng: workspace too small");
  TDNNF_HIP(hipMemsetAsync(ng->J, 0, sizeof(float) * (size_t)Rp * Dp, s));
  if (in.ones) TDNNF_HIP(hipMemsetAsync(ng->tmpR, 0, sizeof(float) * Rp, s));
  WgradArgs j;
  memset(&j, 0, sizeof(j));
  j.dY = H; j.lddy = Rp; j.X = in.x.data; j.ldx = in.x.stride; j.Do = Rp; j.Di = Di; j.K = K; j.N = N; j.row_stride = in.ix.row_stride;
  for (int i = 0; i < K; i++) j.row_offsets[i] = in.ix.row_offsets[i];
  j.coef = in.eff; j.scale = 1.f; j.G = ng->J; j.ldg = Dp; j.accumulate = 1; j.bias_acc = in.ones ? ng->tmpR : nullptr;
  j.active = in.active; j.max_active = in.max_active;
  TDNNF_HIP(wgrad(j, wg_ws, wg_bytes, s));
  if (in.ones) hipLaunchKernelGGL(scatter_col_kernel, dim3((Rp + 63) / 64), dim3(64), 0, s, ng->tmpR, Rp, ng->J, Dp, D - 1);
  return TDNNF_OK;
}

int stats_main(tdnnf_ng *ng, const NgInput &in, float *H, double *part, void *wg_ws, size_t wg_bytes, bool upd, hipStream_t s) {
  const int N = in.N, K = in.ix.num_offsets, Di = in.Di, Rp = ng->Rp, Dp = ng->Dp;
  const float *bias = ones_column(ng, in);
  const NgRowdotArgs v = ng_pass_rowdot_args(ng->WT, Rp, bias, in, H, Rp, part, rows_gemm_sumsq_blocks(N));
  const int skip = options().ng_diag_skip;
  if (skip && ng->D != 0 && (((skip & 1) && K == 2 && Di >= 1024) || ((skip & 2) && !(K == 2 && Di >= 1024)))) {
    TDNNF_HIP(hipMemsetAsync(H, 0, sizeof(float) * (size_t)N * Rp, s));
    TDNNF_HIP(hipMemsetAsync(part, 0, sizeof(double) * rows_gemm_sumsq_blocks(N), s));
  } else if (ng_pform_ok(Rp, in, wg_bytes)) {
    int rc = ng_pform_pass(ng->W, Rp, Dp, bias, in, H, part, wg_ws, s);
    if (rc) return rc;
  } else if (options().ng_valu && !in.active && ng_rowdot_ok(v)) {
    TDNNF_HIP(ng_rowdot(v, s));
  } else {
    TDNNF_HIP(rows_gemm(ng_pass_gemm_args(ng->W, Dp, Rp, bias, in, H, Rp, part), true, s));
  }
  return stats_after_h(ng, in, H, wg_ws, wg_bytes, upd, s);
}

int stats_side(tdnnf_ng *ng, const float *H, const double *part, void *wg_ws, size_t wg_bytes, hipStream_t s) {
  const int N = ng->cur_N, Rp = ng->Rp, Dp = ng->Dp;
  TDNNF_REQUIRE(wg_ws && wg_bytes >= wgrad_workspace_bytes(Rp, Rp, 1, N), "ng: workspace too small");
  WgradArgs w;
  memset(&w, 0, sizeof(w));
  w.dY = H; w.lddy = Rp; w.X = H; w.ldx = Rp; w.Do = Rp; w.Di = Rp; w.K = 1; w.N = N; w.row_stride = 1; w.scale = 1.f;
  w.G = ng->Ld; w.ldg = Rp; w.accumulate = 0;
  TDNNF_HIP(wgrad(w, wg_ws, wg_bytes, s));
  hipLaunchKernelGGL(ng_scalars_kernel, dim3(1), dim3(256), 0, s, part, rows_gemm_sumsq_blocks(N), ng->cur_ones ? (double)N : 0.0, ng->Ld, ng->WWT,
                     Rp, ng->scal, ng->scale_f);
  if (!ng->cur_upd) return TDNNF_OK;
  TDNNF_HIP(rows_gemm_1seg(ng->J, Dp, ng->J, Dp, true, ng->Kd, Rp, Rp, Rp, Dp, 2, nullptr, nullptr, s));
  const size_t fRR = (size_t)Rp * Rp;
  TDNNF_HIP(hipMemcpyAsync(ng->h_K, ng->Kd, sizeof(float) * fRR, hipMemcpyDeviceToHost, s));
  TDNNF_HIP(hipMemcpyAsync(ng->h_L, ng->Ld, sizeof(float) * fRR, hipMemcpyDeviceToHost, s));
  TDNNF_HIP(hipMemcpyAsync(ng->h_tr0, ng->scal, sizeof(double), hipMemcpyDeviceToHost, s));
  TDNNF_HIP(hipEventRecord(ng->ev_job, s));
  ng_refresh_submit(ng, N, ng->ev_job);
  return TDNNF_OK;
}

int stats_core(tdnnf_ng *ng, const NgInput &in, float *H, void *ws, size_t ws_bytes, bool upd, hipStream_t s) {
  TDNNF_REQUIRE(ws && ws_bytes >= stats_ws_bytes(ng->Rp, in.Di, in.ix.num_offsets, in.N), "ng: workspace too small");
  double *part = (double *)ws;
  void *wg_ws = (char *)ws + part_bytes(in.N);
  const size_t wg_bytes = ws_bytes - part_bytes(in.N);
  int rc = stats_main(ng, in, H, part, wg_ws, wg_bytes, upd, s);
  if (rc) return rc;
  return stats_side(ng, H, part, wg_ws, wg_bytes, s);
}

int init_from(tdnnf_ng *ng, const NgInput &in, int D, float *H, void *ws, size_t ws_bytes, hipStream_t s) {
  int rc = ng_init_default(ng, D, s);
  if (rc) return rc;
  if (ng->rank > 0) {
    const int iters = in.N <= ng->rank ? 1 : 3;
    for (int i = 0; i < iters; i++) {
      if ((rc = stats_core(ng, in, H, ws, ws_bytes, true, s))) return rc;
      if ((rc = ng_finalize(ng, s))) return rc;
    }
  }
  ng->t = 0;
  return TDNNF_OK;
}

int input_dim(const NgInput &in) { return in.ix.num_offsets * in.Di + (in.ones ? 1 : 0); }

struct NgFirstUse {
  const NgInput &in;
  float *H;
  void *ws;
  size_t ws_bytes;
};
int begin_call(tdnnf_ng *ng, int D, const NgFirstUse *first, bool reset_cur_N, hipStream_t s) {
  if (ng->D == 0 && first) {
    int rc = init_from(ng, first->in, D, first->H, first->ws, first->ws_bytes, s);
    if (rc) return rc;
  }
  TDNNF_REQUIRE(ng->D == D, "ng: dimension changed from %d to %d", ng->D, D);
  if (reset_cur_N) ng->cur_N = 0;
  return ng_finalize(ng, s);
}

}

size_t ng_stats_workspace_bytes(int rank, int D, int K, int N) {
  const int Rp = pad4(std::max(1, std::min(rank, D - 1)));
  const int Di = K > 0 ? D / K : D;
  return stats_ws_bytes(Rp, Di, std::max(K, 1), N) + 64;
}
int ng_dim(const tdnnf_ng *ng) { return ng->D; }

int ng_stats_step(tdnnf_ng *ng, const NgInput &in, float *H, void *ws, size_t ws_bytes, hipStream_t s) {
  const int K = in.ix.num_offsets;
  TDNNF_REQUIRE(ng && H && in.N > 0 && K >= 1 && K <= kMaxSeg && in.Di > 0, "ng_stats_step: bad arguments");
  NgCallScope scope;
  const NgFirstUse first{in, H, ws, ws_bytes};
  int rc = begin_call(ng, input_dim(in), &first, false, s);
  if (rc || ng->rank == 0) return rc;
  rc = stats_core(ng, in, H, ws, ws_bytes, ng_updating(ng), s);
  ng->t += 1;
  return rc;
}

int ng_stats_main(tdnnf_ng *ng, const NgInput &in, float *H, double *part, void *ws, size_t ws_bytes, hipStream_t s) {
  const int K = in.ix.num_offsets;
  TDNNF_REQUIRE(ng && H && part && in.N > 0 && K >= 1 && K <= kMaxSeg && in.Di > 0, "ng_stats_main: bad arguments");
  NgCallScope scope;
  const NgFirstUse first{in, H, ws, ws_bytes};
  int rc = begin_call(ng, input_dim(in), &first, true, s);
  if (rc || ng->rank == 0) return rc;
  return stats_main(ng, in, H, part, ws, ws_bytes, ng_updating(ng), s);
}

int ng_stats_main_prepare(tdnnf_ng *ng, const NgInput &in, float *H, double *part, hipStream_t s, RowsGemmArgs *out) {
  const int K = in.ix.num_offsets, D = input_dim(in);
  TDNNF_REQUIRE(ng && H && part && out && in.N > 0 && K >= 1 && K <= kMaxSeg && ng->D == D, "ng_stats_main_prepare: bad arguments");
  if (ng->rank == 0) {
    memset(out, 0, sizeof(*out));
    ng->cur_N = 0;
    return TDNNF_OK;
  }
  NgCallScope scope;
  int rc = begin_call(ng, D, nullptr, true, s);
  if (rc) return rc;
  *out = ng_pass_gemm_args(ng->W, ng->Dp, ng->Rp, ones_column(ng, in), in, H, ng->Rp, part);
  return TDNNF_OK;
}
int ng_stats_main_finish(tdnnf_ng *ng, const NgInput &in, const float *H, void *ws, size_t ws_bytes, hipStream_t s) {
  TDNNF_REQUIRE(ng && H && ng->D != 0 && ng->rank > 0 && in.N > 0, "ng_stats_main_finish: bad arguments");
  NgCallScope scope;
  return stats_after_h(ng, in, H, ws, ws_bytes, ng_updating(ng), s);
}

int ng_external_begin(tdnnf_ng *ng, int D, const float **W, int *Rp, int *ldw, hipStream_t s) {
  TDNNF_REQUIRE(ng && W && Rp && ldw, "ng_external_begin: bad arguments");
  *W = nullptr;
  if (ng->D == 0 || ng->rank == 0) return TDNNF_OK;
  int rc = begin_call(ng, D, nullptr, true, s);
  if (rc) return rc;
  *W = ng->W;
  *Rp = ng->Rp;
  *ldw = ng->Dp;
  return TDNNF_OK;
}

int ng_stats_side(tdnnf_ng *ng, const float *H, const double *part, void *ws, size_t ws_bytes, hipStream_t s) {
  TDNNF_REQUIRE(ng && H && part, "ng_stats_side: bad arguments");
  if (ng->rank == 0 || ng->cur_N == 0) return TDNNF_OK;
  NgCallScope scope;
  int rc = stats_side(ng, H, part, ws, ws_bytes, s);
  ng->t += 1;
  return rc;
}

size_t ng_project_tmp_floats(const tdnnf_ng *in, const tdnnf_ng *out, int Do, int ldT) {
  const size_t q = in ? (size_t)Do * in->Rp : 0, p = out ? (size_t)out->Rp * ldT : 0;
  return std::max(q, p) + 16;
}

int ng_project(tdnnf_ng *in, tdnnf_ng *out, float *T, int Do, int Dx, int ldT, float *tmp, hipStream_t s) {
  TDNNF_REQUIRE(T && tmp && ldT % 4 == 0 && ldT >= Dx, "ng_project: bad arguments");
  NgCallScope scope;
  if (in && in->rank > 0) {
    TDNNF_REQUIRE(in->D == Dx && in->Dp == ldT, "ng_project: input-side dimension mismatch");
// ... 30 lines not shown
```

### tdnn-f_nas_amd/csrc/rows_gemm.hip

```cpp
#include <algorithm>
#include <cstring>
#include <vector>

#include "colreduce.h"
#include "common.h"
#include "device.h"
#include "gemm_f32.h"
#include "gemm_ring.h"
#include "launch_forms.h"
#include "planes_gemm.h"
#include "rows_gemm_kernels.h"

namespace tdnnf {
namespace {

float *g_scratch_override = nullptr;
size_t g_scratch_override_bytes = 0;
int g_gemm_prec = 0;
const float *g_tw_w = nullptr, *g_tw_wt = nullptr;
long long g_tw_n = 0;

struct KRange {
  long long ktot;
  bool k4;
// ... 215 lines not shown
    at.C = a.C + (long long)m_main * a.ldc;
    for (int i = 0; i < at.nseg; i++) {
      at.seg[i].m_lo -= m_main;
      at.seg[i].m_hi -= m_main;
    }
    at.add_lo -= m_main;
    at.add_hi -= m_main;
    if (stats) {
      at.colstats = a.colstats + (long long)main_mt * a.N;
      at.colstats_stride = am.colstats_stride;
    }
    if (tail_split) {
      {
        ProfScope ps(cls, flops * at.M / a.M, s);
        launch_split_k<WM, WN, TM, TN, BK>(at, (at.M + BM - 1) / BM, ntn, S_tail, ktot, scratch, b_kc, vec, s);
        count_rows_form<WM, WN, TM, TN, BK>(kFormMainSplitTail);
      }
      if (stats) {
        MatView ct{at.C, at.M, at.N, (int)at.ldc};
        hipError_t e = colreduce_partial_into(1, ct, ct, tail_plan.chunks, tail_plan.rows_per_chunk, am.colstats_stride, at.colstats, s);
        if (e != hipSuccess) return e;
      }
      return hipGetLastError();
    }
    ProfScope ps(cls, flops * at.M / a.M, s);
    const hipError_t e = launch_rows<WM, WN, TM, TN, BK>(at, b_kc, vec, s);
    count_rows_form<WM, WN, TM, TN, BK>(kFormMainPlainTail);
    return e;
  }
  ProfScope ps(cls, flops, s);
  if (stats) {
    RowsGemmArgs as = a;
    as.colstats_stride = ntm;
    *a.colstats_rows = ntm;
    return launch_rows<WM, WN, TM, TN, BK>(as, b_kc, vec, s);
  }
  return launch_rows<WM, WN, TM, TN, BK>(a, b_kc, vec, s);
}

template <int WM, int WN, int TM, int TN, int BK>
hipError_t launch_rows_sumsq(const RowsGemmArgs &a, bool b_kc, bool vec, hipStream_t s) {
  constexpr int BM = WM * TM * 32;
  const int tiles = (a.M + BM - 1) / BM, slots = rows_slots<WM, WN, TM, TN, BK>(0);
  const auto [ktot, k4] = k_range(a);
  float *scratch = nullptr;
  size_t scratch_bytes = 0;
  if (tiles * 4 <= slots && k4 && ktot >= 16 * BK && (scratch = splitk_scratch(&scratch_bytes))) {
    const long long kt = (ktot + BK - 1) / BK;
    int S = slots / tiles;
    if (S > kt / 4) S = (int)(kt / 4);
    if (S > 16) S = 16;
    const size_t need = sizeof(float) * (size_t)S * a.M * ((a.N + 3) & ~3);
    if (S >= 2 && need <= scratch_bytes && tiles * S <= a.sumsq_cap) {
      launch_split_k<WM, WN, TM, TN, BK>(a, tiles, 1, S, ktot, scratch, b_kc, vec, s);
      count_rows_form<WM, WN, TM, TN, BK>(kFormSumsqSplitK);
      return hipGetLastError();
    }
  }
  return launch_rows<WM, WN, TM, TN, BK>(a, b_kc, vec, s, kFormSumsqPlain);
}

template <int WM, int WN, int TM, int TN, int BK>
hipError_t launch_rows_post(const RowsGemmArgs &a, bool vec, int cls, double flops, hipStream_t s) {
  constexpr int BM = WM * TM * 32, BN = WN * TN * 32;
  const int ntm = (a.M + BM - 1) / BM, ntn = (a.N + BN - 1) / BN;
  constexpr size_t lds = rows_lds_bytes<BM, BN, BK>(true);
  static const bool opted = opt_in_lds(rows_gemm_post_kernel<WM, WN, TM, TN, BK, 4>, lds) && opt_in_lds(rows_gemm_post_kernel<WM, WN, TM, TN, BK, 1>, lds);
  (void)opted;
  ProfScope ps(cls, flops, s);
  note_launch(0, vec);
  count_rows_form<WM, WN, TM, TN, BK>(kFormPost);
  if (vec) hipLaunchKernelGGL((rows_gemm_post_kernel<WM, WN, TM, TN, BK, 4>), dim3(ntm * ntn), dim3(256), lds, s, a, ntm, ntn);
  else hipLaunchKernelGGL((rows_gemm_post_kernel<WM, WN, TM, TN, BK, 1>), dim3(ntm * ntn), dim3(256), lds, s, a, ntm, ntn);
  return hipGetLastError();
}

inline long long floordiv(long long a, long long b) { return a >= 0 ? a / b : -((-a + b - 1) / b); }

bool planes_try_rows(const RowsGemmArgs &a, bool b_kc, int np, double flops, hipStream_t s, hipError_t *err) {
  const PlanesOperand *ha = planes_hint_a(), *hb = planes_hint_b();
  if (!ha || !hb || ha->np != np || hb->np != np || !ha->P || a.sumsq || a.ksplit > 1 || a.nseg > 16) return false;
  if (ha->coef || (a.coef == nullptr) != (hb->coef == nullptr)) return false;
  long long coef_t0 = 0;
  if (a.coef) {
    coef_t0 = a.coef - hb->coef;
    if (coef_t0 < 0 || coef_t0 >= 16 || hb->coef_period <= 0) return false;
  }
  if (a.lda != ha->ld || a.A < ha->base || (a.A - ha->base) % ha->ld != 0) return false;
  const long long arow0 = (a.A - ha->base) / ha->ld;
  const int BM = planes_gemm_tile_rows(a.N), BN = planes_gemm_tile_cols(a.N);
  const long long m_pad = (long long)((a.M + BM - 1) / BM) * BM, n_pad = (long long)((a.N + BN - 1) / BN) * BN;
  PlanesGemmArgs g;
  memset(&g, 0, sizeof(g));
  g.np = np;
  g.A = ha->P; g.RA = ha->R; g.scale_a = ha->scale; g.scale_b = hb->scale;
  if (a.ldb != hb->ld || a.B < hb->base) return false;
  const long long boff0 = a.B - hb->base;
  if (b_kc) {
    if (!hb->P) return false;
    g.B = hb->P; g.RB = hb->R;
  } else {
    if (!hb->PT) return false;
    g.B = hb->PT; g.RB = hb->Rt;
  }
  for (int i = 0; i < a.nseg; i++) {
    const GemmSeg &sg = a.seg[i];
    const long long shift = floordiv(sg.a_off, ha->ld), c0 = sg.a_off - shift * ha->ld;
    if (c0 % 16 != 0 || c0 + sg.klen > ha->cols || sg.klen <= 0) return false;
    const long long first = arow0 + shift;
    const int lo = sg.m_lo > 0 ? sg.m_lo : 0, hi = sg.m_hi < a.M ? sg.m_hi : a.M;
    if (hi <= lo) return false;
    if (first + lo < 0 || first + hi > ha->rows) return false;
// ... 99 lines not shown
        count_form(gt.ksplit >= 2 ? kPlanesMainSplitTail : kPlanesMainPlainTail);
        if (gt.ksplit >= 2) {
          *err = planes_gemm(gt, s);
          if (*err == hipSuccess) *err = planes_splitk_finish(gt, s);
        } else {
          gt.ksplit = 0;
          gt.partial = nullptr;
          *err = planes_gemm(gt, s);
        }
        if (stats && *err == hipSuccess) {
          MatView ct{gt.C, tail_rows, a.N, (int)gt.ldc};
          *err = colreduce_partial_into(1, ct, ct, tail_plan.chunks, tail_plan.rows_per_chunk, gm.colstats_stride, a.colstats + (long long)main_mt * a.N, s);
        }
        return true;
      }
    }
  }
  count_form(kPlanesPlain);
  *err = planes_gemm(g, s);
  return true;
}

}

SplitKScratchOverride::SplitKScratchOverride(float *buf, size_t bytes) : prev_buf(g_scratch_override), prev_bytes(g_scratch_override_bytes) {
  g_scratch_override = buf;
  g_scratch_override_bytes = bytes;
}
SplitKScratchOverride::~SplitKScratchOverride() {
  g_scratch_override = prev_buf;
  g_scratch_override_bytes = prev_bytes;
}
GemmPrecisionScope::GemmPrecisionScope(int prec) : prev(g_gemm_prec) { g_gemm_prec = prec; }
GemmPrecisionScope::~GemmPrecisionScope() { g_gemm_prec = prev; }
int gemm_precision_default() { return g_gemm_prec; }
TransposedWeightsScope::TransposedWeightsScope(const float *w_base, const float *wt_base, long long n) : prev_w(g_tw_w), prev_wt(g_tw_wt), prev_n(g_tw_n) {
  g_tw_w = w_base;
  g_tw_wt = wt_base;
  g_tw_n = n;
}
TransposedWeightsScope::~TransposedWeightsScope() {
  g_tw_w = prev_w;
  g_tw_wt = prev_wt;
  g_tw_n = prev_n;
}
const float *transposed_weights(const float *W) {
  if (!g_tw_w || !g_tw_wt || W < g_tw_w || W >= g_tw_w + g_tw_n) return nullptr;
  return g_tw_wt + (W - g_tw_w);
}

hipError_t rows_gemm(const RowsGemmArgs &a_in, bool b_kc, hipStream_t s) {
  if (a_in.M <= 0 || a_in.N <= 0 || a_in.nseg <= 0) return hipSuccess;
  RowsGemmArgs a = a_in;
  a.c_vec = aligned16(a.C) && a.ldc % 4 == 0 && (a.init_mode != 1 || aligned16(a.bias)) && (!a.add || (aligned16(a.add) && a.ldadd % 4 == 0));
  const bool vec = operands_vec4(a);
  const int waste128 = ((a.N + 127) / 128) * 128 - a.N, waste160 = ((a.N + 159) / 160) * 160 - a.N;
  const long long ktot = k_range(a).ktot;
  double flops = 0;
  for (int i = 0; i < a.nseg; i++) flops += 2.0 * usable_rows(a.seg[i], a.M) * a.N * a.seg[i].klen;
  if (prof_on()) {
    double a_elems = 0, b_elems = 0;
    bool taps = true;
    for (int i = 1; i < a.nseg; i++)
      taps = taps && a.seg[i].klen == a.seg[0].klen && a.lda > 0 && (a.seg[i].a_off - a.seg[0].a_off) % a.lda == 0;
    if (taps) {
      long long lo = a.seg[0].a_off, hi = a.seg[0].a_off;
      for (int i = 1; i < a.nseg; i++) {
        lo = std::min(lo, a.seg[i].a_off);
        hi = std::max(hi, a.seg[i].a_off);
      }
      a_elems = ((double)a.M + (double)(hi - lo) / (double)a.lda) * a.seg[0].klen;
    }
    for (int i = 0; i < a.nseg; i++) {
      if (!taps) a_elems += (double)usable_rows(a.seg[i], a.M) * a.seg[i].klen;
      b_elems += (double)a.seg[i].klen * a.N;
    }
    double c_elems = (double)a.M * a.N * (a.init_mode == 0 ? 2.0 : 1.0);
    if (a.add) c_elems += (double)(std::min(a.add_hi, a.M) - std::max(a.add_lo, 0)) * a.N;
    prof_next_gemm(flops, 4.0 * (a_elems + b_elems + c_elems));
  }
  a.serial_epilogue = 0;
  a.alt_seg_order = options().gemm_alt_taps && is_two_tap_shift(a);
  if (rows_gemm_has_post(a)) {
    if (!b_kc || a.init_mode == 0 || a.sumsq || a.ksplit > 1 || (a.init_mode == 1 && !a.bias)) return hipErrorInvalidValue;
    a.prec = 0;
    a.colstats = nullptr;
    if (a.colstats_rows) *a.colstats_rows = 0;
    a.c_vec = a.c_vec && (!a.col_scale || aligned16(a.col_scale)) && (!a.col_offset || aligned16(a.col_offset));
    if (waste160 < waste128) return launch_rows_post<4, 1, 1, 5, 16>(a, vec, 1, flops, s);
    if ((long long)((a.M + 127) / 128) * ((a.N + 127) / 128) < 768) return launch_rows_post<2, 2, 1, 2, 16>(a, vec, 0, flops, s);
    if (ktot <= 512) return launch_rows_post<2, 2, 2, 2, 16>(a, vec, 0, flops, s);
    return launch_rows_post<2, 2, 2, 2, 32>(a, vec, 0, flops, s);
  }
  if (a.prec == 0) {
    a.prec = g_gemm_prec;
    if (a.prec == 0 && (options().gemm_arith_test == 1 || options().gemm_arith_test == 3)) a.prec = options().gemm_arith_test;
  }
  if (a.prec == 2) a.prec = 0;
  if (a.prec == 4 || (a.prec == 3 && options().planes)) {
    hipError_t pe = hipSuccess;
    if (planes_try_rows(a, b_kc, a.prec == 4 ? 2 : 3, flops, s, &pe)) return pe;
    if (a.prec == 4) a.prec = 0;
  }
  if (!(b_kc && vec)) a.prec = 0;
  if (a.colstats_rows) *a.colstats_rows = 0;
  if (!a.colstats_rows || a.prec != 0 || a.sumsq || a.N <= 32 || waste160 < waste128 || a.ksplit > 1) a.colstats = nullptr;
// ... 6 lines not shown
    if (a.N <= 96 && a.N > 64 && ((options().ng_bk & 4) || ktot >= 2048)) return launch_rows_sumsq<2, 2, 2, 2, 32>(a, b_kc, vec, s);
    if (a.N <= 96) return (options().ng_bk & 2) ? launch_rows_sumsq<4, 1, 1, 3, 32>(a, b_kc, vec, s) : launch_rows_sumsq<4, 1, 1, 3, 16>(a, b_kc, vec, s);
    return launch_rows_sumsq<2, 2, 2, 2, 32>(a, b_kc, vec, s);
  }
  if (a.N <= 32 && a.M >= 1024) {
    ProfScope ps(0, flops, s);
    return (options().ng_bk & 1) ? launch_rows<4, 1, 1, 1, 64>(a, b_kc, vec, s) : launch_rows<4, 1, 1, 1, 32>(a, b_kc, vec, s);
  }
  if (waste160 < waste128) return launch_rows_balanced<4, 1, 1, 5, 16>(a, b_kc, vec, 1, flops, s);
  {
    const long long tiles128 = (long long)((a.M + 127) / 128) * ((a.N + 127) / 128);
    const bool small = tiles128 < 768;
    if (small && a.prec == 0 && !a.sumsq) return launch_rows_balanced<2, 2, 1, 2, 16>(a, b_kc, vec, 0, flops, s);
    if ((ktot <= 512 && a.prec == 0) || a.prec == 3) return launch_rows_balanced<2, 2, 2, 2, 16>(a, b_kc, vec, 0, flops, s);
  }
  return launch_rows_balanced<2, 2, 2, 2, 32>(a, b_kc, vec, 0, flops, s);
}

struct RowsGemmGroup {
  std::vector<RowsGemmArgs> args;
  std::vector<int> first;
  RowsGemmArgs *d_args = nullptr;
  int *d_first = nullptr;
  int capacity = 0;
};
void rows_gemm_group_destroy(RowsGemmGroup *g) {
  if (!g) return;
  if (g->d_args) hipFree(g->d_args);
  if (g->d_first) hipFree(g->d_first);
  delete g;
}
bool rows_gemm_group_ok(const RowsGemmArgs &a) {
  if (a.M <= 0 || a.N <= 0 || a.N > 32 || !a.sumsq || a.nseg <= 0 || a.ksplit > 1 || a.colstats || a.add) return false;
  return operands_vec4(a);
}
hipError_t rows_gemm_group(const std::vector<RowsGemmArgs> &calls, RowsGemmGroup **cache, hipStream_t s) {
  if (calls.empty()) return hipSuccess;
  if (!*cache) *cache = new RowsGemmGroup();
  RowsGemmGroup &g = **cache;
  std::vector<RowsGemmArgs> prep(calls.size());
  std::vector<int> first(calls.size() + 1, 0);
  double flops = 0, bytes = 0;
  for (size_t i = 0; i < calls.size(); i++) {
    RowsGemmArgs a = calls[i];
    if (!rows_gemm_group_ok(a)) return hipErrorInvalidValue;
    a.c_vec = aligned16(a.C) && a.ldc % 4 == 0 && (a.init_mode != 1 || aligned16(a.bias));
    a.sumsq_cap = rows_gemm_sumsq_blocks(a.M);
    a.serial_epilogue = 0;
    a.ksplit = 0;
    a.partial = nullptr;
    a.prec = 0;
    a.colstats = nullptr;
    a.colstats_rows = nullptr;
    a.alt_seg_order = options().gemm_alt_taps && is_two_tap_shift(a);
    prep[i] = a;
    first[i + 1] = first[i] + (a.M + 127) / 128;
    const double kt = (double)k_range(a).ktot;
    flops += 2.0 * a.M * a.N * kt;
    bytes += 4.0 * ((double)a.M * kt + kt * a.N + (double)a.M * a.N);
  }
  const bool same = g.args.size() == prep.size() && memcmp(g.args.data(), prep.data(), sizeof(RowsGemmArgs) * prep.size()) == 0 && g.first == first;
  if (!same) {
    if (g.capacity < (int)prep.size()) {
      if (g.d_args) hipFree(g.d_args);
      if (g.d_first) hipFree(g.d_first);
      hipError_t e = hipMalloc((void **)&g.d_args, sizeof(RowsGemmArgs) * prep.size());
      if (e != hipSuccess) return e;
      e = hipMalloc((void **)&g.d_first, sizeof(int) * (prep.size() + 1));
      if (e != hipSuccess) return e;
      g.capacity = (int)prep.size();
    }
    g.args = prep;
    g.first = first;
    hipError_t e = hipMemcpyAsync(g.d_args, g.args.data(), sizeof(RowsGemmArgs) * prep.size(), hipMemcpyHostToDevice, s);
    if (e != hipSuccess) return e;
    e = hipMemcpyAsync(g.d_first, g.first.data(), sizeof(int) * first.size(), hipMemcpyHostToDevice, s);
    if (e != hipSuccess) return e;
  }
  constexpr size_t lds = rows_lds_bytes<128, 32, 32>(true);
  ProfGemmRange prof(3, flops, bytes, s);
  RowsGemmTasks t{g.d_args, g.d_first, (int)prep.size()};
  note_launch(0, true);
  count_rows_form<4, 1, 1, 1, 32>(kFormGrouped);
  hipLaunchKernelGGL((rows_gemm_group_kernel<4, 1, 1, 1, 32, true, 4>), dim3(first.back()), dim3(256), lds, s, t);
  return hipGetLastError();
}

}
```

### tdnn-f_nas_amd/csrc/rows_gemm_kernels.h

```cpp
#pragma once
#include "common.h"
#include "gemm_dev.h"
#include "gemm_f32.h"

namespace tdnnf {
namespace {

__device__ __forceinline__ void post_store4(const RowsGemmArgs &p, int m, int n, float4 v, float4 pre, float4 addv) {
  v.x += pre.x; v.y += pre.y; v.z += pre.z; v.w += pre.w;
  if (!p.post_add) { v.x += p.add_scale * addv.x; v.y += p.add_scale * addv.y; v.z += p.add_scale * addv.z; v.w += p.add_scale * addv.w; }
  if (p.relu) { v.x = floor_keep_nan(v.x, 0.f); v.y = floor_keep_nan(v.y, 0.f); v.z = floor_keep_nan(v.z, 0.f); v.w = floor_keep_nan(v.w, 0.f); }
  const float4 sc = p.col_scale ? *reinterpret_cast<const float4 *>(p.col_scale + n) : make_float4(1.f, 1.f, 1.f, 1.f);
  const float4 of = p.col_offset ? *reinterpret_cast<const float4 *>(p.col_offset + n) : make_float4(0.f, 0.f, 0.f, 0.f);
  const float as = p.post_add ? p.add_scale : 0.f;
  v.x = sc.x * v.x + of.x + as * addv.x;
  v.y = sc.y * v.y + of.y + as * addv.y;
  v.z = sc.z * v.z + of.z + as * addv.z;
  v.w = sc.w * v.w + of.w + as * addv.w;
  const int mo = p.row_map ? p.row_map[m] : m;
  if (mo >= 0) *reinterpret_cast<float4 *>(p.C + (long long)mo * p.ldc + n) = v;
}
__device__ __forceinline__ void post_store1(const RowsGemmArgs &p, int m, int n, float x) {
  if (p.init_mode == 1) x += p.bias[n];
  const float a = (p.add && m >= p.add_lo && m < p.add_hi) ? p.add[(long long)(m - p.add_lo) * p.ldadd + n] : 0.f;
  if (!p.post_add) x += p.add_scale * a;
  if (p.relu) x = floor_keep_nan(x, 0.f);
  x = (p.col_scale ? p.col_scale[n] : 1.f) * x + (p.col_offset ? p.col_offset[n] : 0.f) + (p.post_add ? p.add_scale * a : 0.f);
  const int mo = p.row_map ? p.row_map[m] : m;
  if (mo >= 0) p.C[(long long)mo * p.ldc + n] = x;
}

template <int WM, int WN, int TM, int TN, int BK, bool B_KC, int VEC, bool POST = false>
__device__ __forceinline__ void rows_gemm_block(const RowsGemmArgs &p, int ntm, int ntn, int bx, int gx) {
  constexpr int BM = WM * TM * 32, BN = WN * TN * 32;
  constexpr int LDAS = BK + 4;
  constexpr int LDBS = B_KC ? BK + 4 : BN + 4;
  constexpr int A_TILE = BM * LDAS;
  constexpr int B_TILE = B_KC ? BN * LDBS : BK * LDBS;
  constexpr int A_F4 = (BM * BK / 4 + 255) / 256;
  constexpr int B_F4 = (BN * BK / 4 + 255) / 256;
  constexpr int KF4 = BK / 4;
  extern __shared__ __attribute__((aligned(16))) float smem[];
  float *As = smem;
  float *Bs = smem + 2 * A_TILE;

  const int nblk = ntm * ntn;
  int bid = bx;
  {
    const int q = nblk / 8, r = nblk % 8, xcd = bid % 8, j = bid / 8;
    bid = (xcd < r ? xcd * (q + 1) : r * (q + 1) + (xcd - r) * q) + j;
  }
  int sp = 0;
  if (p.ksplit > 1) {
    sp = bx % p.ksplit;
    bid = bx / p.ksplit;
  }
// ... 168 lines not shown
          const float *q = bs + (kg * 8) * LDBS + i * 32;
          b[i] = make_float4(q[0], q[LDBS], q[2 * LDBS], q[3 * LDBS]);
        }
      }
#pragma unroll
      for (int i = 0; i < TM; i++)
#pragma unroll
        for (int j = 0; j < TN; j++) {
          acc[i][j] = __builtin_amdgcn_mfma_f32_32x32x2f32(a[i].x, b[j].x, acc[i][j], 0, 0, 0);
          acc[i][j] = __builtin_amdgcn_mfma_f32_32x32x2f32(a[i].y, b[j].y, acc[i][j], 0, 0, 0);
          acc[i][j] = __builtin_amdgcn_mfma_f32_32x32x2f32(a[i].z, b[j].z, acc[i][j], 0, 0, 0);
          acc[i][j] = __builtin_amdgcn_mfma_f32_32x32x2f32(a[i].w, b[j].w, acc[i][j], 0, 0, 0);
        }
    }
  };

  if (seg < p.nseg) {
    load_tile();
    store_tile(0);
    __syncthreads();
    int buf = 0;
    while (true) {
      kc += BK;
      if (kc >= klen) next_seg();
      const bool more = seg < p.nseg;
      if (more) load_tile();
      compute(buf);
      if (!more) break;
      store_tile(buf ^ 1);
      __syncthreads();
      buf ^= 1;
    }
  }

  constexpr int LDCS = BN + 4;
  constexpr int SMEM_FLOATS = 2 * (A_TILE + B_TILE);
  constexpr int HALF = (BM * LDCS <= SMEM_FLOATS) ? BM : ((BM / 2) * LDCS <= SMEM_FLOATS ? BM / 2 : BM / 4);
  static_assert(HALF * LDCS <= SMEM_FLOATS, "epilogue tile does not fit the staging LDS");
  static_assert(HALF % (TM * 32) == 0, "a wave's rows must not straddle epilogue passes");
  float *Cs = smem;
  const bool cvec = p.c_vec != 0;
  __syncthreads();
  if (p.sumsq) {
    double v = ssq;
    for (int o = 32; o > 0; o >>= 1) v += __shfl_xor(v, o, 64);
    double *red = reinterpret_cast<double *>(smem);
    if (lane == 0) red[wave] = v;
    __syncthreads();
    if (t == 0) p.sumsq[p.ksplit > 1 ? bx : bid] = (red[0] + red[1]) + (red[2] + red[3]);
    if (bx == 0)
      for (int i = gx + t; i < p.sumsq_cap; i += 256) p.sumsq[i] = 0.0;
    __syncthreads();
  }
  constexpr bool kColStats = 256 % (BN / 4) == 0 && (HALF * (BN / 4)) % 256 == 0;
  const bool colstats = kColStats && p.colstats && p.ksplit <= 1;
  float cs[4] = {0.f, 0.f, 0.f, 0.f}, cq[4] = {0.f, 0.f, 0.f, 0.f};
#pragma unroll
  for (int pass = 0; pass < BM / HALF; pass++) {
    if ((wm * TM * 32) / HALF == pass) {
#pragma unroll
      for (int i = 0; i < TM; i++)
#pragma unroll
        for (int j = 0; j < TN; j++)
#pragma unroll
          for (int r = 0; r < 16; r++) {
            const int row = (wm * TM + i) * 32 + (r & 3) + 8 * (r >> 2) + 4 * lh - pass * HALF;
            Cs[row * LDCS + (wn * TN + j) * 32 + li] = acc[i][j][r];
          }
    }
    constexpr int kSeg = HALF * (BN / 4) / 256;
    constexpr int kGrp = kSeg % 8 == 0 ? 8 : (kSeg % 5 == 0 ? 5 : (kSeg % 4 == 0 ? 4 : (kSeg % 2 == 0 ? 2 : 1)));
    constexpr bool kFastShape = (HALF * (BN / 4)) % 256 == 0;
    const bool fast_tile = kFastShape && cvec && p.ksplit <= 1 && !p.serial_epilogue && m0 + BM <= p.M && n0 + BN <= p.N;
    if (fast_tile) {
      __syncthreads();
#pragma unroll
      for (int g = 0; g < kSeg; g += kGrp) {
        float4 pre[kGrp], addv[kGrp];
        const float *zero = reinterpret_cast<const float *>(&g_zero4);
#pragma unroll
        for (int u = 0; u < kGrp; u++) {
          const int idx = t + 256 * (g + u), m = m0 + pass * HALF + idx / (BN / 4), n = n0 + (idx % (BN / 4)) * 4;
          const float *pp = p.init_mode == 0 ? p.C + (long long)m * p.ldc + n : (p.init_mode == 1 ? p.bias + n : zero);
          const float *pa = (p.add && m >= p.add_lo && m < p.add_hi) ? p.add + (long long)(m - p.add_lo) * p.ldadd + n : zero;
          pre[u] = *reinterpret_cast<const float4 *>(pp);
          addv[u] = *reinterpret_cast<const float4 *>(pa);
        }
#pragma unroll
        for (int u = 0; u < kGrp; u++) {
          const int idx = t + 256 * (g + u), row = idx / (BN / 4), c4 = (idx % (BN / 4)) * 4;
          const int m = m0 + pass * HALF + row, n = n0 + c4;
          float4 v = *reinterpret_cast<const float4 *>(Cs + row * LDCS + c4);
          if constexpr (POST) {
            post_store4(p, m, n, v, pre[u], addv[u]);
            continue;
          }
          v.x += pre[u].x + p.add_scale * addv[u].x;
          v.y += pre[u].y + p.add_scale * addv[u].y;
          v.z += pre[u].z + p.add_scale * addv[u].z;
          v.w += pre[u].w + p.add_scale * addv[u].w;
          if (p.relu) { v.x = floor_keep_nan(v.x, 0.f); v.y = floor_keep_nan(v.y, 0.f); v.z = floor_keep_nan(v.z, 0.f); v.w = floor_keep_nan(v.w, 0.f); }
          *reinterpret_cast<float4 *>(p.C + (long long)m * p.ldc + n) = v;
          if (kColStats && colstats) {
            cs[0] += v.x; cs[1] += v.y; cs[2] += v.z; cs[3] += v.w;
            cq[0] += v.x * v.x; cq[1] += v.y * v.y; cq[2] += v.z * v.z; cq[3] += v.w * v.w;
          }
        }
      }
      if (pass + 1 < BM / HALF) __syncthreads();
      continue;
    }
    __syncthreads();
    for (int idx = t; idx < HALF * (BN / 4); idx += 256) {
      const int row = idx / (BN / 4), c4 = (idx % (BN / 4)) * 4;
      const int m = m0 + pass * HALF + row, n = n0 + c4;
      if (m >= p.M || n >= p.N) continue;
      float4 v = *reinterpret_cast<const float4 *>(Cs + row * LDCS + c4);
      if (p.ksplit > 1) {
        const int ldp = (p.N + 3) & ~3;
        *reinterpret_cast<float4 *>(p.partial + ((long long)sp * p.M + m) * ldp + n) = v;
        continue;
      }
      if constexpr (POST) {
        if (cvec && n + 3 < p.N) {
          const float4 z = make_float4(0.f, 0.f, 0.f, 0.f);
          const float4 b = p.init_mode == 1 ? *reinterpret_cast<const float4 *>(p.bias + n) : z;
          const float4 o = (p.add && m >= p.add_lo && m < p.add_hi) ? *reinterpret_cast<const float4 *>(p.add + (long long)(m - p.add_lo) * p.ldadd + n) : z;
          post_store4(p, m, n, v, b, o);
        } else {
          const float vv[4] = {v.x, v.y, v.z, v.w};
#pragma unroll
          for (int e = 0; e < 4; e++)
            if (n + e < p.N) post_store1(p, m, n + e, vv[e]);
        }
        continue;
      }
      float *c = p.C + (long long)m * p.ldc + n;
      if (cvec && n + 3 < p.N) {
        if (p.init_mode == 1) {
          const float4 b = *reinterpret_cast<const float4 *>(p.bias + n);
          v.x += b.x; v.y += b.y; v.z += b.z; v.w += b.w;
        } else if (p.init_mode == 0) {
          const float4 o = *reinterpret_cast<const float4 *>(c);
          v.x += o.x; v.y += o.y; v.z += o.z; v.w += o.w;
        }
        if (p.add && m >= p.add_lo && m < p.add_hi) {
          const float4 o = *reinterpret_cast<const float4 *>(p.add + (long long)(m - p.add_lo) * p.ldadd + n);
          v.x += p.add_scale * o.x; v.y += p.add_scale * o.y; v.z += p.add_scale * o.z; v.w += p.add_scale * o.w;
        }
        if (p.relu) { v.x = floor_keep_nan(v.x, 0.f); v.y = floor_keep_nan(v.y, 0.f); v.z = floor_keep_nan(v.z, 0.f); v.w = floor_keep_nan(v.w, 0.f); }
        *reinterpret_cast<float4 *>(c) = v;
        if (colstats) {
          cs[0] += v.x; cs[1] += v.y; cs[2] += v.z; cs[3] += v.w;
          cq[0] += v.x * v.x; cq[1] += v.y * v.y; cq[2] += v.z * v.z; cq[3] += v.w * v.w;
        }
      } else {
        const float vv[4] = {v.x, v.y, v.z, v.w};
#pragma unroll
        for (int e = 0; e < 4; e++) {
          if (n + e < p.N) {
            float x = vv[e];
            if (p.init_mode == 1) x += p.bias[n + e];
            else if (p.init_mode == 0) x += c[e];
            if (p.add && m >= p.add_lo && m < p.add_hi) x += p.add_scale * p.add[(long long)(m - p.add_lo) * p.ldadd + n + e];
            if (p.relu) x = floor_keep_nan(x, 0.f);
            c[e] = x;
            if (colstats) { cs[e] += x; cq[e] += x * x; }
          }
        }
      }
    }
    if (pass + 1 < BM / HALF) __syncthreads();
  }
  if (kColStats && colstats) {
    constexpr int G = BN / 4;
    __syncthreads();
    float *red = smem;
#pragma unroll
    for (int e = 0; e < 4; e++) {
      red[((t / G) * BN + (t % G) * 4 + e) * 2] = cs[e];
      red[((t / G) * BN + (t % G) * 4 + e) * 2 + 1] = cq[e];
    }
    __syncthreads();
    if (t < BN && n0 + t < p.N) {
      float a0 = 0.f, a1 = 0.f;
#pragma unroll
      for (int g = 0; g < 256 / G; g++) {
        a0 += red[(g * BN + t) * 2];
        a1 += red[(g * BN + t) * 2 + 1];
      }
      p.colstats[(long long)tile_m * p.N + n0 + t] = a0;
      p.colstats[((long long)p.colstats_stride + tile_m) * p.N + n0 + t] = a1;
    }
  }
}

template <int WM, int WN, int TM, int TN, int BK, bool B_KC, int VEC, int TAG = 0>
__global__ __launch_bounds__(256) void rows_gemm_kernel(const RowsGemmArgs p, int ntm, int ntn) {
  rows_gemm_block<WM, WN, TM, TN, BK, B_KC, VEC>(p, ntm, ntn, (int)blockIdx.x, (int)gridDim.x);
}
template <int WM, int WN, int TM, int TN, int BK, int VEC>
__global__ __launch_bounds__(256) void rows_gemm_post_kernel(const RowsGemmArgs p, int ntm, int ntn) {
  rows_gemm_block<WM, WN, TM, TN, BK, true, VEC, true>(p, ntm, ntn, (int)blockIdx.x, (int)gridDim.x);
}
struct RowsGemmTasks {
  const RowsGemmArgs *args;
  const int *first;
  int ntasks;
};
template <int WM, int WN, int TM, int TN, int BK, bool B_KC, int VEC>
__global__ __launch_bounds__(256) void rows_gemm_group_kernel(RowsGemmTasks g) {
  int lo = 0, hi = g.ntasks;
  while (hi - lo > 1) {
    const int mid = (lo + hi) >> 1;
    if ((int)blockIdx.x >= g.first[mid]) lo = mid;
// ... 363 lines not shown
```

Before: 1.632 million.

## Compute per-tile partials of L = H^T H inside the NG stats pass kernels

The natural-gradient stats kernels (rows GEMM, one-pass combine, fused BN-ReLU backward sweep) now also write per-tile partial products of H^T H from their accumulators into a buffer. The later L computation can then sum these partials instead of re-reading H from global memory. Bias is folded into the accumulators before the partial is taken, and done flags track which launch forms produced partials. This adds LDS staging and extra output traffic in the pass kernels, plus arena buffers, and is enabled by default through a new option.

```diff
diff --git a/include/tdnnf_hip.h b/include/tdnnf_hip.h
--- a/include/tdnnf_hip.h
+++ b/include/tdnnf_hip.h
@@ -289,6 +289,9 @@
 int tdnnf_ng_stats_pass(const tdnnf_tdnn_indexes *ix, const tdnnf_mat *X, int Di, const float *eff_dev, const float *WT_dev,
                         const float *W_dev, int ldw, const float *bias_dev, tdnnf_mat *H, double *sumsq_dev, int sumsq_cap, int form,
                         void *workspace_dev, size_t workspace_bytes, tdnnf_stream);
+int tdnnf_ng_stats_pass_l(const tdnnf_tdnn_indexes *ix, const tdnnf_mat *X, int Di, const float *W_dev, int ldw, const float *bias_dev,
+                          tdnnf_mat *H, double *sumsq_dev, int sumsq_cap, int form, tdnnf_mat *dz, float *memo_dev, const float *mask_dev,
+                          int mask_rows, int l_from_h, float *L_dev, void *workspace_dev, size_t workspace_bytes, tdnnf_stream);
 const float *tdnnf_ng_scale_dev(const tdnnf_ng *);
 
 size_t tdnnf_constrain_orthonormal_workspace_bytes(int rows, int cols);
diff --git a/tdnn-f_nas_amd/csrc/abi_ng.hip b/tdnn-f_nas_amd/csrc/abi_ng.hip
--- a/tdnn-f_nas_amd/csrc/abi_ng.hip
+++ b/tdnn-f_nas_amd/csrc/abi_ng.hip
@@ -3,8 +3,10 @@
 
 #include <algorithm>
 
+#include "fused.h"
 #include "gemm_f32.h"
 #include "ng.h"
+#include "ng_l_tile.h"
 
 using namespace tdnnf;
 
@@ -43,6 +45,65 @@
   GemmPrecisionScope exact_f32(2);
   TDNNF_HIP(rows_gemm(ng_pass_gemm_args(W, ldw, Rp, bias, in, H->data, H->stride, sumsq), true, s));
   return TDNNF_OK;
+}
+
+int tdnnf_ng_stats_pass_l(const tdnnf_tdnn_indexes *ix, const tdnnf_mat *X, int Di, const float *W, int ldw, const float *bias, tdnnf_mat *H,
+                          double *sumsq, int sumsq_cap, int form, tdnnf_mat *dz, float *memo, const float *mask, int mask_rows, int l_from_h, float *L,
+                          void *workspace, size_t workspace_bytes, tdnnf_stream stream) {
+  TDNNF_REQUIRE(X && X->data && H && H->data && L && W && sumsq && (form == 0 || form == 2 || form == 3), "ng_stats_pass_l: bad arguments");
+  const int N = H->rows, Rp = H->cols;
+  TDNNF_REQUIRE(H->stride == Rp && Rp >= 1 && Rp <= 96 && N >= 1 && sumsq_cap >= rows_gemm_sumsq_blocks(N),
+                "ng_stats_pass_l: H must be dense, of rank <= 96, and sumsq hold %d entries", rows_gemm_sumsq_blocks(N));
+  hipStream_t s = (hipStream_t)stream;
+  float *tiles = nullptr;
+  void *sweep_ws = nullptr;
+  int done = 0;
+  auto run = [&]() -> int {
+    TDNNF_HIP(hipMalloc((void **)&tiles, sizeof(float) * (l_tile_partial_floats(N, Rp) + 64)));
+    const NgLPart lp{tiles, &done};
+    if (form == 3) {
+      TDNNF_REQUIRE(dz && dz->data && memo && X->rows == N && dz->rows == N && dz->cols == X->cols && ldw >= X->cols && (!mask || mask_rows >= 1),
+                    "ng_stats_pass_l: the fused sweep takes X and dz of N rows and W of rank x ldw, ldw >= their width");
+      const size_t wsb = bn_relu_bwd_workspace_bytes(N, X->cols);
+      TDNNF_HIP(hipMalloc(&sweep_ws, wsb));
+      NgFuse f;
+      f.W = W; f.Rp = Rp; f.ldw = ldw; f.H = H->data; f.part = sumsq; f.part_cap = rows_gemm_sumsq_blocks(N);
+      f.lpart = l_from_h ? nullptr : tiles;
+      TDNNF_HIP(bn_relu_bwd(view(X), view(dz), memo, 1.0f, false, nullptr, false, false, 0.f, view(dz), nullptr, 1.0f, sweep_ws, wsb, s, mask,
+                            mask ? mask_rows : 1, &f));
+      done = l_from_h ? 0 : 1;
+    } else {
+      TDNNF_REQUIRE(ix && Di > 0 && ix->num_offsets >= 1 && ix->num_offsets <= kMaxSeg && ix->row_stride >= 1 && ldw >= ix->num_offsets * Di,
+                    "ng_stats_pass_l: bad taps");
+      const int K = ix->num_offsets;
+      for (int i = 0; i < K; i++)
+        TDNNF_REQUIRE(ix->row_offsets[i] >= 0 && (long long)(N - 1) * ix->row_stride + ix->row_offsets[i] < X->rows && Di <= X->cols,
+                      "ng_stats_pass_l: tap %d reads outside X (%d x %d)", i, X->rows, X->cols);
+      NgInput in;
+      memset(&in, 0, sizeof(in));
+      in.x = view(X); in.ix = *ix; in.Di = Di; in.ones = bias ? 1 : 0; in.N = N;
+      if (form == 2) {
+        TDNNF_REQUIRE(workspace && ng_pform_ok(Rp, in, workspace_bytes), "ng_stats_pass_l: not a shape of the one-pass form");
+        int rc = ng_pform_pass(W, Rp, ldw, bias, in, H->data, sumsq, workspace, s, l_from_h ? nullptr : &lp);
+        if (rc) return rc;
+      } else {
+        GemmPrecisionScope exact_f32(2);
+        RowsGemmArgs a = ng_pass_gemm_args(W, ldw, Rp, bias, in, H->data, Rp, sumsq);
+        if (!l_from_h) {
+          a.lpart = tiles;
+          a.lpart_done = &done;
+        }
+        TDNNF_HIP(rows_gemm(a, true, s));
+      }
+    }
+    TDNNF_REQUIRE(l_from_h || done, "ng_stats_pass_l: the launch form this pass took leaves no tile partials of L");
+    return ng_l_standalone(H->data, l_from_h ? nullptr : tiles, N, Rp, L, s);
+  };
+  const int rc = run();
+  (void)hipStreamSynchronize(s);
+  (void)hipFree(tiles);
+  (void)hipFree(sweep_ws);
+  return rc;
 }
 
 int tdnnf_ng_create(int rank, int update_period, float num_samples_history, float alpha, tdnnf_ng **out) {
diff --git a/tdnn-f_nas_amd/csrc/abi_tdnn.hip b/tdnn-f_nas_amd/csrc/abi_tdnn.hip
--- a/tdnn-f_nas_amd/csrc/abi_tdnn.hip
+++ b/tdnn-f_nas_amd/csrc/abi_tdnn.hip
@@ -80,7 +80,7 @@
   Options &o = options();
   if (!name) return nullptr;
   const struct { const char *n; int *p; } table[] = {{"ng_grouped", &o.ng_grouped}, {"ng_fuse", &o.ng_fuse}, {"ng_early_in", &o.ng_early_in},
-                                                     {"wgrad_stream", &o.wgrad_stream}, {"gemm_ring", &o.gemm_ring}, {"planes", &o.planes}, {"den_split", &o.den_split}, {"phase_events", &o.phase_events}, {"wgrad_lag", &o.wgrad_lag}, {"ng_bk", &o.ng_bk}, {"ng_valu", &o.ng_valu}, {"ng_pform", &o.ng_pform}, {"planes_group", &o.planes_group}, {"xent_behind_den", &o.xent_behind_den}, {"ng_early_fork", &o.ng_early_fork}, {"ng_diag_skip", &o.ng_diag_skip}, {"wgrad_small", &o.wgrad_small}, {"splitk_per_cu", &o.splitk_per_cu}, {"gemm_alt_taps", &o.gemm_alt_taps}, {"reverse_passes", &o.reverse_passes}, {"splitk_partial_round", &o.splitk_partial_round}, {"wgrad_on_caller", &o.wgrad_on_caller}, {"den_mw_test_abort", &o.den_mw_test_abort}, {"planes_check_bound", &o.planes_check_bound}, {"den_gamma_pairs", &o.den_gamma_pairs}, {"num_form", &o.num_form}, {"align_form", &o.align_form}, {"align_checkpoint", &o.align_checkpoint}, {"align_path_checkpoint", &o.align_path_checkpoint}, {"num_frontier_cap", &o.num_frontier_cap}, {"gemm_arith_test", &o.gemm_arith_test}};
+                                                     {"wgrad_stream", &o.wgrad_stream}, {"gemm_ring", &o.gemm_ring}, {"planes", &o.planes}, {"den_split", &o.den_split}, {"phase_events", &o.phase_events}, {"wgrad_lag", &o.wgrad_lag}, {"ng_bk", &o.ng_bk}, {"ng_valu", &o.ng_valu}, {"ng_pform", &o.ng_pform}, {"ng_l_in_pass", &o.ng_l_in_pass}, {"planes_group", &o.planes_group}, {"xent_behind_den", &o.xent_behind_den}, {"ng_early_fork", &o.ng_early_fork}, {"ng_diag_skip", &o.ng_diag_skip}, {"wgrad_small", &o.wgrad_small}, {"splitk_per_cu", &o.splitk_per_cu}, {"gemm_alt_taps", &o.gemm_alt_taps}, {"reverse_passes", &o.reverse_passes}, {"splitk_partial_round", &o.splitk_partial_round}, {"wgrad_on_caller", &o.wgrad_on_caller}, {"den_mw_test_abort", &o.den_mw_test_abort}, {"planes_check_bound", &o.planes_check_bound}, {"den_gamma_pairs", &o.den_gamma_pairs}, {"num_form", &o.num_form}, {"align_form", &o.align_form}, {"align_checkpoint", &o.align_checkpoint}, {"align_path_checkpoint", &o.align_path_checkpoint}, {"num_frontier_cap", &o.num_frontier_cap}, {"gemm_arith_test", &o.gemm_arith_test}};
   for (auto &e : table)
     if (strcmp(e.n, name) == 0) return e.p;
   return nullptr;
diff --git a/tdnn-f_nas_amd/csrc/common.h b/tdnn-f_nas_amd/csrc/common.h
--- a/tdnn-f_nas_amd/csrc/common.h
+++ b/tdnn-f_nas_amd/csrc/common.h
@@ -62,6 +62,7 @@
   int ng_early_fork = 1;
   int xent_behind_den = -1;
   int ng_pform = 1;
+  int ng_l_in_pass = 1;
   int ng_valu = 0;
   int ng_diag_skip = 0;
   int phase_events = 0;
diff --git a/tdnn-f_nas_amd/csrc/fused.h b/tdnn-f_nas_amd/csrc/fused.h
--- a/tdnn-f_nas_amd/csrc/fused.h
+++ b/tdnn-f_nas_amd/csrc/fused.h
@@ -24,6 +24,7 @@
   float *H;
   double *part;
   int part_cap;
+  float *lpart;
 };
 bool bn_relu_bwd_ng_ok(MatView x, MatView dz, MatView d_aff, int Rp);
 bool bn_relu_bwd_ng_pays(int rows);
diff --git a/tdnn-f_nas_amd/csrc/fused.hip b/tdnn-f_nas_amd/csrc/fused.hip
--- a/tdnn-f_nas_amd/csrc/fused.hip
+++ b/tdnn-f_nas_amd/csrc/fused.hip
@@ -6,6 +6,7 @@
 #include "fused.h"
 #include "gemm_f32.h"
 #include "launch_forms.h"
+#include "ng_l_tile.h"
 #include "planes_gemm.h"
 
 namespace tdnnf {
@@ -384,6 +385,11 @@
       const int r = r0 + wave * 32 + (e & 3) + 8 * (e >> 2) + 4 * lh;
       if (n < ng.Rp && r < x.rows) ng.H[(long long)r * ng.Rp + n] = acc[j][e];
     }
+  }
+  if (ng.lpart) {
+    auto hval = [&](int c, int e) { return (FULL || r0 + wave * 32 + (e & 3) + 8 * (e >> 2) + 4 * lh < x.rows) ? acc[c][e] : 0.f; };
+    static_assert(BM * LD >= kLTileLdsFloats, "the tile partial's images do not fit the A tile");
+    l_tile_partial<NT, acc_t>(hval, (ng.Rp + 31) / 32, As, ng.lpart + (size_t)blk * l_tile_pairs(ng.Rp) * 1024);
   }
   double v = ssq;
   for (int o = 32; o > 0; o >>= 1) v += __shfl_xor(v, o, 64);
diff --git a/tdnn-f_nas_amd/csrc/gemm_f32.h b/tdnn-f_nas_amd/csrc/gemm_f32.h
--- a/tdnn-f_nas_amd/csrc/gemm_f32.h
+++ b/tdnn-f_nas_amd/csrc/gemm_f32.h
@@ -41,6 +41,8 @@
   float *partial;
   double *sumsq;
   int sumsq_cap;
+  float *lpart;
+  int *lpart_done;
   float *colstats;
   int *colstats_rows;
   int colstats_stride;
diff --git a/tdnn-f_nas_amd/csrc/launch_forms.h b/tdnn-f_nas_amd/csrc/launch_forms.h
--- a/tdnn-f_nas_amd/csrc/launch_forms.h
+++ b/tdnn-f_nas_amd/csrc/launch_forms.h
@@ -41,6 +41,8 @@
   kRowsVec4Launches,
   kRowsScalarLaunches,
   kPlanesAltChunked,
+  kNgLPairsInPass,
+  kNgLPairsFromH,
   kLaunchFormCounters
 };
 
diff --git a/tdnn-f_nas_amd/csrc/launch_forms.hip b/tdnn-f_nas_amd/csrc/launch_forms.hip
--- a/tdnn-f_nas_amd/csrc/launch_forms.hip
+++ b/tdnn-f_nas_amd/csrc/launch_forms.hip
@@ -56,8 +56,12 @@
     snprintf(buf, sizeof(buf), "rows.launches_vec4");
   } else if (index == kRowsScalarLaunches) {
     snprintf(buf, sizeof(buf), "rows.launches_scalar");
+  } else if (index == kPlanesAltChunked) {
+    snprintf(buf, sizeof(buf), "planes.alt_chunked");
+  } else if (index == kNgLPairsInPass) {
+    snprintf(buf, sizeof(buf), "ng.l_pairs_in_pass");
   } else {
-    snprintf(buf, sizeof(buf), "planes.alt_chunked");
+    snprintf(buf, sizeof(buf), "ng.l_pairs_from_h");
   }
   return buf;
 }
diff --git a/tdnn-f_nas_amd/csrc/net.h b/tdnn-f_nas_amd/csrc/net.h
--- a/tdnn-f_nas_amd/csrc/net.h
+++ b/tdnn-f_nas_amd/csrc/net.h
@@ -118,6 +118,8 @@
     float *H_in = nullptr, *H_out = nullptr, *T = nullptr, *bsum = nullptr;
     double *part_in = nullptr, *part_out = nullptr;
     int N = 0;
+    float *lpart_in = nullptr, *lpart_out = nullptr;
+    int l_done_in = 0, l_done_out = 0;
   };
   std::vector<NgComp> ngc;
   float *ng_bsum_all = nullptr;
diff --git a/tdnn-f_nas_amd/csrc/net_arena.hip b/tdnn-f_nas_amd/csrc/net_arena.hip
--- a/tdnn-f_nas_amd/csrc/net_arena.hip
+++ b/tdnn-f_nas_amd/csrc/net_arena.hip
@@ -6,6 +6,7 @@
 #include "gemm_ring.h"
 #include "net_model.h"
 #include "ng.h"
+#include "ng_l_tile.h"
 
 namespace tdnnf {
 namespace {
@@ -199,6 +200,10 @@
     C.T = A.take<float>((size_t)cd.rows * ldT + 16);
     C.part_in = A.take<double>((size_t)rows_gemm_sumsq_blocks(rows) + 8);
     C.part_out = A.take<double>((size_t)rows_gemm_sumsq_blocks(rows) + 8);
+    if (n->ng_grouped && options().ng_l_in_pass) {
+      C.lpart_in = A.take<float>(l_tile_partial_floats(rows, Rpi) + 64);
+      C.lpart_out = A.take<float>(l_tile_partial_floats(rows, Rpo) + 64);
+    }
   }
   size_t tot = 0;
   for (size_t i = 0; i < n->comps.size(); i++)
diff --git a/tdnn-f_nas_amd/csrc/net_step_grad.hip b/tdnn-f_nas_amd/csrc/net_step_grad.hip
--- a/tdnn-f_nas_amd/csrc/net_step_grad.hip
+++ b/tdnn-f_nas_amd/csrc/net_step_grad.hip
@@ -61,6 +61,7 @@
   }
   const int N = dyv->rows, ones = bias_acc ? 1 : 0, Dx = ldw + ones, ldT = (Dx + 3) & ~3;
   auto &C = n->ngc[comp];
+  const NgLPart l_in{C.lpart_in, &C.l_done_in}, l_out{C.lpart_out, &C.l_done_out};
   TDNNF_REQUIRE(C.T && C.N == N, "net_forward_backward: component %s has no natural-gradient buffers for %d rows", n->comps[comp].name.c_str(), N);
   float *T = C.T;
   const bool grouped = n->ng_grouped && ng_dim(n->ng_in[comp]) != 0 && ng_dim(n->ng_out[comp]) != 0;
@@ -86,7 +87,7 @@
       CK(ng_stats_main_finish(n->ng_in[comp], xin, C.H_in, wsw, n->ws_bytes, sw));
     }
   } else {
-    CK(ng_stats_main(n->ng_in[comp], xin, C.H_in, C.part_in, wsw, n->ws_bytes, sw));
+    CK(ng_stats_main(n->ng_in[comp], xin, C.H_in, C.part_in, wsw, n->ws_bytes, sw, &l_in));
   }
   if (n->early_on) {
     memcpy(n->early[comp].xin, &xin, sizeof(xin));
@@ -99,7 +100,7 @@
     fused_comp = -1;
     CK(ng_stats_main_finish(n->ng_out[comp], yin, C.H_out, wsw, n->ws_bytes, sw));
   } else {
-    CK(ng_stats_main(n->ng_out[comp], yin, C.H_out, C.part_out, wsw, n->ws_bytes, sw));
+    CK(ng_stats_main(n->ng_out[comp], yin, C.H_out, C.part_out, wsw, n->ws_bytes, sw, &l_out));
   }
   if (grouped) {
     n->ng_cur.push_back(comp);
@@ -227,6 +228,8 @@
       RowsGemmArgs a;
       CK(ng_stats_main_prepare(n->ng_in[comp], xin, n->ngc[comp].H_in, n->ngc[comp].part_in, n->s4, &a));
       if (!rows_gemm_group_ok(a)) continue;
+      a.lpart = n->ngc[comp].lpart_in;
+      a.lpart_done = &n->ngc[comp].l_done_in;
       calls.push_back(a);
       grouped.push_back(comp);
     }
@@ -237,7 +240,8 @@
     SplitKScratchOverride early_scratch(n->s4_scratch, n->s4_scratch_bytes);
     for (int comp : who) {
       memcpy(&xin, n->early[comp].xin, sizeof(xin));
-      CK(ng_stats_main(n->ng_in[comp], xin, n->ngc[comp].H_in, n->ngc[comp].part_in, n->ws4, n->ws_bytes, n->s4));
+      const NgLPart l_in{n->ngc[comp].lpart_in, &n->ngc[comp].l_done_in};
+      CK(ng_stats_main(n->ng_in[comp], xin, n->ngc[comp].H_in, n->ngc[comp].part_in, n->ws4, n->ws_bytes, n->s4, &l_in));
       n->early[comp].done = n->fb_count;
     }
   }
@@ -256,6 +260,8 @@
   CK(ng_external_begin(n->ng_out[comp], dv.cols, &W, &Rp, &ldw, s));
   if (!W || !bn_relu_bwd_ng_ok(xv, dzv, dv, Rp) || !(fuse_always || bn_relu_bwd_ng_pays(dv.rows))) return 0;
   f.W = W; f.Rp = Rp; f.ldw = ldw; f.H = C.H_out; f.part = C.part_out; f.part_cap = rows_gemm_sumsq_blocks(dv.rows);
+  f.lpart = C.lpart_out;
+  C.l_done_out = C.lpart_out ? 1 : 0;
   fused_comp = comp;
   return 1;
 }
@@ -277,6 +283,8 @@
       g.T = C.T; g.Do = cd.rows; g.ldw = cd.cols; g.Dx = cd.cols + (cd.has_bias ? 1 : 0); g.ldT = (g.Dx + 3) & ~3;
       g.bsum = cd.has_bias ? C.bsum : nullptr;
       g.H_in = C.H_in; g.H_out = C.H_out; g.part_in = C.part_in; g.part_out = C.part_out; g.N = C.N;
+      g.l_in = NgLPart{C.lpart_in, &C.l_done_in};
+      g.l_out = NgLPart{C.lpart_out, &C.l_done_out};
       g.W_acc = net_Wg(n, comp); g.bias_acc = net_Bg(n, comp);
       gc.push_back(g);
     }
diff --git a/tdnn-f_nas_amd/csrc/ng.h b/tdnn-f_nas_amd/csrc/ng.h
--- a/tdnn-f_nas_amd/csrc/ng.h
+++ b/tdnn-f_nas_amd/csrc/ng.h
@@ -53,6 +53,11 @@
   int max_active;
 };
 
+struct NgLPart {
+  float *buf;
+  int *done;
+};
+
 constexpr int kWtPadRows = 64;
 struct NgRowdotArgs {
   const float *X;
@@ -74,7 +79,7 @@
 
 size_t ng_stats_workspace_bytes(int rank, int D, int K, int N);
 int ng_stats_step(tdnnf_ng *ng, const NgInput &in, float *H, void *ws, size_t ws_bytes, hipStream_t s);
-int ng_stats_main(tdnnf_ng *ng, const NgInput &in, float *H, double *part, void *ws, size_t ws_bytes, hipStream_t s);
+int ng_stats_main(tdnnf_ng *ng, const NgInput &in, float *H, double *part, void *ws, size_t ws_bytes, hipStream_t s, const NgLPart *lp = nullptr);
 int ng_stats_side(tdnnf_ng *ng, const float *H, const double *part, void *ws, size_t ws_bytes, hipStream_t s);
 int ng_stats_main_prepare(tdnnf_ng *ng, const NgInput &in, float *H, double *part, hipStream_t s, RowsGemmArgs *out);
 int ng_stats_main_finish(tdnnf_ng *ng, const NgInput &in, const float *H, void *ws, size_t ws_bytes, hipStream_t s);
@@ -99,7 +104,9 @@
                                                 int part_cap);
 TDNNF_NG_LOCAL size_t ng_pform_ws_bytes(int Rp, int Di, int K, int N);
 TDNNF_NG_LOCAL bool ng_pform_ok(int Rp, const NgInput &in, size_t ws_bytes);
-TDNNF_NG_LOCAL int ng_pform_pass(const float *W, int Rp, int ldw, const float *bias, const NgInput &in, float *H, double *part, void *ws, hipStream_t s);
+TDNNF_NG_LOCAL int ng_pform_pass(const float *W, int Rp, int ldw, const float *bias, const NgInput &in, float *H, double *part, void *ws, hipStream_t s,
+                                 const NgLPart *lp = nullptr);
+TDNNF_NG_LOCAL int ng_l_standalone(const float *H, const float *tpart, int N, int Rp, float *L, hipStream_t s);
 
 
 struct NgGroupComp {
@@ -111,6 +118,7 @@
   const double *part_in, *part_out;
   int N;
   float *W_acc, *bias_acc;
+  NgLPart l_in, l_out;
 };
 struct NgGroup;
 int ng_group_create(const std::vector<NgGroupComp> &comps, NgGroup **out);
diff --git a/tdnn-f_nas_amd/csrc/ng_group.hip b/tdnn-f_nas_amd/csrc/ng_group.hip
--- a/tdnn-f_nas_amd/csrc/ng_group.hip
+++ b/tdnn-f_nas_amd/csrc/ng_group.hip
@@ -2,12 +2,15 @@
 #include <string.h>
 
 #include <algorithm>
+#include <deque>
 #include <vector>
 
 #include "gemm_f32.h"
 #include "ggemm.h"
+#include "launch_forms.h"
 #include "ng.h"
 #include "ng_group_kernels.h"
+#include "ng_l_tile.h"
 
 namespace tdnnf {
 
@@ -18,8 +21,11 @@
   PairDesc *pairs = nullptr;
   CompDesc *cdesc = nullptr;
   float *lpart = nullptr;
-  int npairs = 0, nslabs = 0, commit_blocks = 0;
+  int npairs = 0, nslabs = 0, commit_blocks = 0, reduce_blocks = 0;
   size_t l_lds = 0;
+  std::vector<const int *> l_done;
+  std::vector<PairDesc> h_pairs;
+  std::deque<std::vector<PairDesc>> uploads;
   DevList stage[4], kstage;
   hipEvent_t ev_staged = nullptr;
 };
@@ -33,7 +39,7 @@
   GemmList st[4], kst;
   size_t qp_floats = 0;
   std::vector<size_t> q_off, p_off;
-  int slab_total = 0, blk = 0;
+  int slab_total = 0, blk = 0, rblk = 0;
   for (const NgGroupComp &c : comps) {
     TDNNF_REQUIRE(c.in && c.out && c.in->D == c.Dx && c.in->Dp == c.ldT && c.out->D == c.Do && c.in->rank > 0 && c.out->rank > 0 && c.in->Rp <= 96 &&
                       c.out->Rp <= 96 && c.N > 0,
@@ -67,7 +73,15 @@
       p.rows_per_slab = rps;
       p.nslab = (c.N + rps - 1) / rps;
       p.slab0 = slab_total;
-      slab_total += p.nslab;
+      const NgLPart &lp = side == 0 ? c.l_in : c.l_out;
+      p.tpart = lp.buf;
+      p.ntile = (c.N + kLTileRows - 1) / kLTileRows;
+      p.trun = (p.ntile + kLTileSlabs - 1) / kLTileSlabs;
+      p.nslab_t = (p.ntile + p.trun - 1) / p.trun;
+      p.rblk0 = rblk;
+      if (lp.buf && lp.done) rblk += p.nslab_t * (p.nt * (p.nt + 1) / 2);
+      slab_total += lp.buf && lp.done ? std::max(p.nslab, p.nslab_t) : p.nslab;
+      g->l_done.push_back(lp.buf ? lp.done : nullptr);
       pairs.push_back(p);
       kst.add(ng->J, ng->Dp, 1, ng->J, 1, ng->Dp, ng->Kd, ng->Rp, ng->Rp, ng->Rp, ng->Dp, 1.0f, 0);
     }
@@ -90,6 +104,8 @@
   g->npairs = (int)pairs.size();
   g->nslabs = slab_total;
   g->commit_blocks = blk;
+  g->reduce_blocks = rblk;
+  g->h_pairs = pairs;
   size_t bytes = 0;
   bytes = carve_room(bytes, sizeof(PairDesc) * pairs.size());
   bytes = carve_room(bytes, sizeof(CompDesc) * cdesc.size());
@@ -153,7 +169,21 @@
   for (tdnnf_ng *ng : g->objs)
     TDNNF_REQUIRE(ng->cur_upd == upd && ng->cur_N > 0 && !ng->pending, "ng_group_run: the group's preconditioners are out of step");
   hipLaunchKernelGGL(ng_set_columns_kernel, dim3(nc), dim3(256), 0, s, g->cdesc);
-  hipLaunchKernelGGL(ng_l_partial_kernel, dim3(g->nslabs), dim3(256), g->l_lds, s, g->pairs, g->npairs, g->lpart);
+  bool changed = false, any_tiles = false, any_pass = false;
+  for (int i = 0; i < g->npairs; i++) {
+    const int in_pass = g->l_done[i] && *g->l_done[i] ? 1 : 0;
+    changed = changed || in_pass != g->h_pairs[i].in_pass;
+    g->h_pairs[i].in_pass = in_pass;
+    any_tiles = any_tiles || in_pass;
+    any_pass = any_pass || !in_pass;
+    count_form(in_pass ? kNgLPairsInPass : kNgLPairsFromH);
+  }
+  if (changed) {
+    g->uploads.push_back(g->h_pairs);
+    TDNNF_HIP(hipMemcpyAsync(g->pairs, g->uploads.back().data(), sizeof(PairDesc) * g->npairs, hipMemcpyHostToDevice, s));
+  }
+  if (any_pass) hipLaunchKernelGGL(ng_l_partial_kernel, dim3(g->nslabs), dim3(256), g->l_lds, s, g->pairs, g->npairs, g->lpart);
+  if (any_tiles) hipLaunchKernelGGL(ng_l_reduce_kernel, dim3(g->reduce_blocks), dim3(256), 0, s, g->pairs, g->npairs, g->lpart);
   hipLaunchKernelGGL(ng_l_finish_kernel, dim3(g->npairs), dim3(1024), 0, s, g->pairs, g->lpart);
   if (upd) {
     int rc = launch_list(g->kstage, s);
@@ -173,6 +203,49 @@
     ng->t += 1;
   }
   return TDNNF_OK;
+}
+
+int ng_l_standalone(const float *H, const float *tpart, int N, int Rp, float *L, hipStream_t s) {
+  TDNNF_REQUIRE((H || tpart) && L && N > 0 && Rp >= 1 && Rp <= 96, "ng_l_standalone: bad arguments");
+  PairDesc p;
+  memset(&p, 0, sizeof(p));
+  p.N = N; p.Rp = Rp; p.nt = (Rp + 31) / 32;
+  int rps = std::max(256, (N + 31) / 32);
+  rps = (rps + 7) & ~7;
+  p.rows_per_slab = rps;
+  p.nslab = (N + rps - 1) / rps;
+  p.ntile = (N + kLTileRows - 1) / kLTileRows;
+  p.trun = (p.ntile + kLTileSlabs - 1) / kLTileSlabs;
+  p.nslab_t = (p.ntile + p.trun - 1) / p.trun;
+  p.in_pass = tpart ? 1 : 0;
+  const int nslab = std::max(p.nslab, p.nslab_t), np = p.nt * (p.nt + 1) / 2;
+  size_t bytes = carve_room(0, sizeof(PairDesc));
+  bytes = carve_room(bytes, sizeof(float) * (size_t)nslab * kLSlabFloats);
+  bytes = carve_room(bytes, sizeof(float) * ((size_t)Rp * Rp + 4));
+  bytes = carve_room(bytes, sizeof(double) * 2) + 1024;
+  char *dev = nullptr;
+  TDNNF_HIP(hipMalloc((void **)&dev, bytes));
+  auto run = [&]() -> int {
+    TDNNF_HIP(hipMemsetAsync(dev, 0, bytes, s));
+    char *cur = dev;
+    PairDesc *dp = carve<PairDesc>(cur, 1);
+    float *slabs = carve<float>(cur, (size_t)nslab * kLSlabFloats);
+    float *wwt = carve<float>(cur, (size_t)Rp * Rp + 4);
+    double *scal = carve<double>(cur, 2);
+    p.H = H; p.tpart = tpart; p.Ld = L; p.WWT = wwt; p.scal = scal; p.scale_f = wwt + (size_t)Rp * Rp; p.part = scal; p.npart = 0;
+    TDNNF_HIP(hipMemcpyAsync(dp, &p, sizeof(p), hipMemcpyHostToDevice, s));
+    const size_t lds = sizeof(float) * 2 * kLSlabFloats;
+    (void)hipFuncSetAttribute((const void *)ng_l_partial_kernel, hipFuncAttributeMaxDynamicSharedMemorySize, (int)lds);
+    if (tpart) hipLaunchKernelGGL(ng_l_reduce_kernel, dim3(p.nslab_t * np), dim3(256), 0, s, dp, 1, slabs);
+    else hipLaunchKernelGGL(ng_l_partial_kernel, dim3(p.nslab), dim3(256), lds, s, dp, 1, slabs);
+    hipLaunchKernelGGL(ng_l_finish_kernel, dim3(1), dim3(1024), 0, s, dp, slabs);
+    TDNNF_LAUNCH_CHECK();
+    TDNNF_HIP(hipStreamSynchronize(s));
+    return TDNNF_OK;
+  };
+  const int rc = run();
+  (void)hipFree(dev);
+  return rc;
 }
 
 struct NgFin {
diff --git a/tdnn-f_nas_amd/csrc/ng_group_kernels.h b/tdnn-f_nas_amd/csrc/ng_group_kernels.h
--- a/tdnn-f_nas_amd/csrc/ng_group_kernels.h
+++ b/tdnn-f_nas_amd/csrc/ng_group_kernels.h
@@ -20,6 +20,10 @@
   double ones_term;
   int N, Rp, nt, npart;
   int slab0, nslab, rows_per_slab;
+  int in_pass;
+  const float *tpart;
+  int ntile, trun, nslab_t;
+  int rblk0;
 };
 __device__ __forceinline__ int ntile_pairs(int nt) { return nt * (nt + 1) / 2; }
 constexpr int kLSlabFloats = 6 * 1024;
@@ -102,15 +106,42 @@
   extern __shared__ float lds[];
   const PairDesc &p = pairs[last_start_le<&PairDesc::slab0>(pairs, npairs, (int)blockIdx.x)];
   const int slab = blockIdx.x - p.slab0;
+  if (p.in_pass || slab >= p.nslab) return;
   if (p.nt == 1) l_partial_body<1>(p, slab, partial, lds);
   else if (p.nt == 2) l_partial_body<2>(p, slab, partial, lds);
   else l_partial_body<3>(p, slab, partial, lds);
 }
 
+__global__ __launch_bounds__(256) void ng_l_reduce_kernel(const PairDesc *pairs, int npairs, float *partial) {
+  const PairDesc &p = pairs[last_start_le<&PairDesc::rblk0>(pairs, npairs, (int)blockIdx.x)];
+  const int np = ntile_pairs(p.nt), b = blockIdx.x - p.rblk0, slab = b / np, q = b % np;
+  if (!p.in_pass || slab >= p.nslab_t) return;
+  const int t0 = slab * p.trun, t1 = min(p.ntile, t0 + p.trun);
+  const float *src = p.tpart + ((size_t)t0 * np + q) * 1024 + 4 * threadIdx.x;
+  const size_t step = (size_t)np * 1024;
+  float4 v = make_float4(0.f, 0.f, 0.f, 0.f);
+  int i = t0;
+  for (; i + 3 < t1; i += 4) {
+    const float4 w0 = *reinterpret_cast<const float4 *>(src), w1 = *reinterpret_cast<const float4 *>(src + step),
+                 w2 = *reinterpret_cast<const float4 *>(src + 2 * step), w3 = *reinterpret_cast<const float4 *>(src + 3 * step);
+    v.x = (((v.x + w0.x) + w1.x) + w2.x) + w3.x;
+    v.y = (((v.y + w0.y) + w1.y) + w2.y) + w3.y;
+    v.z = (((v.z + w0.z) + w1.z) + w2.z) + w3.z;
+    v.w = (((v.w + w0.w) + w1.w) + w2.w) + w3.w;
+    src += 4 * step;
+  }
+  for (; i < t1; i++) {
+    const float4 w = *reinterpret_cast<const float4 *>(src);
+    v.x += w.x; v.y += w.y; v.z += w.z; v.w += w.w;
+    src += step;
+  }
+  *reinterpret_cast<float4 *>(partial + (size_t)(p.slab0 + slab) * kLSlabFloats + (size_t)q * 1024 + 4 * threadIdx.x) = v;
+}
+
 __global__ __launch_bounds__(1024) void ng_l_finish_kernel(const PairDesc *pairs, const float *partial) {
   __shared__ double red[3][16];
   const PairDesc &p = pairs[blockIdx.x];
-  const int t = threadIdx.x, Rp = p.Rp, nt = p.nt;
+  const int t = threadIdx.x, Rp = p.Rp, nt = p.nt, nslab = p.in_pass ? p.nslab_t : p.nslab;
   double a = 0, b = 0, c = 0;
   for (int i = t; i < p.npart; i += 1024) a += p.part[i];
   int q = 0;
@@ -122,14 +153,14 @@
       const float *src = partial + (size_t)p.slab0 * kLSlabFloats + (size_t)q * 1024 + e;
       float v = 0.f;
       int s = 0;
-      for (; s + 7 < p.nslab; s += 8) {
+      for (; s + 7 < nslab; s += 8) {
         float w[8];
 #pragma unroll
         for (int u = 0; u < 8; u++) w[u] = src[(size_t)(s + u) * kLSlabFloats];
 #pragma unroll
         for (int u = 0; u < 8; u++) v += w[u];
       }
-      for (; s < p.nslab; s++) v += src[(size_t)s * kLSlabFloats];
+      for (; s < nslab; s++) v += src[(size_t)s * kLSlabFloats];
       p.Ld[m * Rp + n] = v;
       const double w = (double)v * (double)p.WWT[m * Rp + n];
       if (ti != tj) {
diff --git a/tdnn-f_nas_amd/csrc/ng_kernels.h b/tdnn-f_nas_amd/csrc/ng_kernels.h
--- a/tdnn-f_nas_amd/csrc/ng_kernels.h
+++ b/tdnn-f_nas_amd/csrc/ng_kernels.h
@@ -2,6 +2,7 @@
 #include <hip/hip_runtime.h>
 
 #include "gemm_f32.h"
+#include "ng_l_tile.h"
 
 namespace tdnnf {
 namespace {
@@ -16,8 +17,11 @@
 struct PformTaps {
   int K, o[kMaxSeg];
 };
+template <bool LPART>
 __global__ __launch_bounds__(256) void pform_combine_kernel(const float *P, int ldp, PformTaps tp, int Rp, const float *bias, float *H, int N,
-                                                            const double *psum, double *part, int part_cap) {
+                                                            const double *psum, double *part, int part_cap, float *lpart) {
+  constexpr int LDH = 33;
+  __shared__ __attribute__((aligned(16))) float hs[LPART ? 128 * LDH + kLTileLdsFloats : 4];
   const int m0 = blockIdx.x * 128, per = Rp / 4;
   for (int e = threadIdx.x; e < 128 * per; e += 256) {
     const int m = m0 + e / per, q = e % per;
@@ -29,6 +33,20 @@
       v.x += t.x; v.y += t.y; v.z += t.z; v.w += t.w;
     }
     *reinterpret_cast<float4 *>(H + (size_t)m * Rp + 4 * q) = v;
+    if constexpr (LPART) {
+      float *h = hs + (e / per) * LDH + 4 * q;
+      h[0] = v.x; h[1] = v.y; h[2] = v.z; h[3] = v.w;
+    }
+  }
+  if constexpr (LPART) {
+    typedef float vec16 __attribute__((ext_vector_type(16)));
+    const int lane = threadIdx.x & 63, wave = threadIdx.x >> 6, li = lane & 31, lh = lane >> 5;
+    __syncthreads();
+    auto hval = [&](int, int e) {
+      const int row = wave * 32 + (e & 3) + 8 * (e >> 2) + 4 * lh;
+      return (li < Rp && m0 + row < N) ? hs[row * LDH + li] : 0.f;
+    };
+    l_tile_partial<1, vec16>(hval, 1, hs + 128 * LDH, lpart + (size_t)blockIdx.x * 1024);
   }
   if (threadIdx.x == 0) {
     double sacc = 0;
diff --git a/tdnn-f_nas_amd/csrc/ng_l_tile.h b/tdnn-f_nas_amd/csrc/ng_l_tile.h
--- /dev/null
+++ b/tdnn-f_nas_amd/csrc/ng_l_tile.h
@@ -0,0 +1,54 @@
+#pragma once
+#include <hip/hip_runtime.h>
+
+namespace tdnnf {
+
+constexpr int kLTileRows = 128;
+constexpr int kLTileLdsFloats = 4096;
+constexpr int kLTileSlabs = 64;
+
+__host__ __device__ inline int l_tile_pairs(int Rp) {
+  const int nt = (Rp + 31) / 32;
+  return nt * (nt + 1) / 2;
+}
+inline size_t l_tile_partial_floats(int N, int Rp) { return (size_t)((N + kLTileRows - 1) / kLTileRows) * l_tile_pairs(Rp) * 1024; }
+
+namespace {
+
+template <int NT, class Vec, class F>
+__device__ __forceinline__ void l_tile_partial(F h, int nt, float *lds, float *out) {
+  const int t = threadIdx.x, lane = t & 63, wave = t >> 6;
+  int q = 0;
+#pragma unroll
+  for (int i = 0; i < NT; i++)
+#pragma unroll
+    for (int j = i; j < NT; j++) {
+      if (j >= nt) continue;
+      Vec l;
+#pragma unroll
+      for (int e = 0; e < 16; e++) l[e] = 0.f;
+#pragma unroll
+      for (int e = 0; e < 16; e++) {
+        float a = h(i, e), b = h(j, e);
+        asm volatile("" : "+v"(a), "+v"(b));
+        l = __builtin_amdgcn_mfma_f32_32x32x2f32(a, b, l, 0, 0, 0);
+        asm volatile("" : "+v"(l)::"memory");
+      }
+      __syncthreads();
+#pragma unroll
+      for (int e = 0; e < 16; e++) lds[(wave * 16 + e) * 64 + lane] = l[e];
+      __syncthreads();
+      const float4 w0 = *reinterpret_cast<const float4 *>(lds + 4 * t), w1 = *reinterpret_cast<const float4 *>(lds + 1024 + 4 * t),
+                   w2 = *reinterpret_cast<const float4 *>(lds + 2048 + 4 * t), w3 = *reinterpret_cast<const float4 *>(lds + 3072 + 4 * t);
+      float4 v;
+      v.x = ((w0.x + w1.x) + w2.x) + w3.x;
+      v.y = ((w0.y + w1.y) + w2.y) + w3.y;
+      v.z = ((w0.z + w1.z) + w2.z) + w3.z;
+      v.w = ((w0.w + w1.w) + w2.w) + w3.w;
+      *reinterpret_cast<float4 *>(out + (size_t)q * 1024 + 4 * t) = v;
+      q++;
+    }
+}
+
+}
+}
diff --git a/tdnn-f_nas_amd/csrc/ng_stats.hip b/tdnn-f_nas_amd/csrc/ng_stats.hip
--- a/tdnn-f_nas_amd/csrc/ng_stats.hip
+++ b/tdnn-f_nas_amd/csrc/ng_stats.hip
@@ -43,7 +43,8 @@
   if (sp.hi - sp.lo > kPformSpanCap || in.Di % 4 != 0 || (in.x.stride % 4) != 0 || in.Di < 1024) return false;
   return ws_bytes >= ng_pform_ws_bytes(Rp, in.Di, K, N);
 }
-int ng_pform_pass(const float *W, int Rp, int ldw, const float *bias, const NgInput &in, float *H, double *part, void *ws, hipStream_t s) {
+int ng_pform_pass(const float *W, int Rp, int ldw, const float *bias, const NgInput &in, float *H, double *part, void *ws, hipStream_t s,
+                  const NgLPart *lp) {
   const int K = in.ix.num_offsets, N = in.N, Di = in.Di;
   const TapSpan sp = tap_span(in.ix);
   PformTaps tp;
@@ -56,9 +57,15 @@
   double *psum = (double *)(P + (((size_t)M * K * Rp + 63) & ~(size_t)63));
   hipLaunchKernelGGL(stack_taps_kernel, dim3(grid_for((long long)K * Rp * Di, 256)), dim3(256), 0, s, W, Rp, ldw, Di, K, WP);
   TDNNF_HIP(rows_gemm_1seg(in.x.data + (size_t)sp.lo * in.x.stride, in.x.stride, WP, Di, true, P, K * Rp, M, K * Rp, Di, 2, nullptr, psum, s));
-  hipLaunchKernelGGL(pform_combine_kernel, dim3(N / 128), dim3(256), 0, s, P, K * Rp, tp, Rp, bias, H, N, psum, part,
-                     rows_gemm_sumsq_blocks(N));
+  const bool l_in_pass = lp && lp->buf && Rp <= 32;
+  if (l_in_pass)
+    hipLaunchKernelGGL(pform_combine_kernel<true>, dim3(N / 128), dim3(256), 0, s, P, K * Rp, tp, Rp, bias, H, N, psum, part,
+                       rows_gemm_sumsq_blocks(N), lp->buf);
+  else
+    hipLaunchKernelGGL(pform_combine_kernel<false>, dim3(N / 128), dim3(256), 0, s, P, K * Rp, tp, Rp, bias, H, N, psum, part,
+                       rows_gemm_sumsq_blocks(N), (float *)nullptr);
   TDNNF_HIP(hipGetLastError());
+  if (l_in_pass && lp->done) *lp->done = 1;
   return TDNNF_OK;
 }
 
@@ -115,21 +122,27 @@
   return TDNNF_OK;
 }
 
-int stats_main(tdnnf_ng *ng, const NgInput &in, float *H, double *part, void *wg_ws, size_t wg_bytes, bool upd, hipStream_t s) {
+int stats_main(tdnnf_ng *ng, const NgInput &in, float *H, double *part, void *wg_ws, size_t wg_bytes, bool upd, hipStream_t s, const NgLPart *lp = nullptr) {
   const int N = in.N, K = in.ix.num_offsets, Di = in.Di, Rp = ng->Rp, Dp = ng->Dp;
   const float *bias = ones_column(ng, in);
+  if (lp && lp->done) *lp->done = 0;
   const NgRowdotArgs v = ng_pass_rowdot_args(ng->WT, Rp, bias, in, H, Rp, part, rows_gemm_sumsq_blocks(N));
   const int skip = options().ng_diag_skip;
   if (skip && ng->D != 0 && (((skip & 1) && K == 2 && Di >= 1024) || ((skip & 2) && !(K == 2 && Di >= 1024)))) {
     TDNNF_HIP(hipMemsetAsync(H, 0, sizeof(float) * (size_t)N * Rp, s));
     TDNNF_HIP(hipMemsetAsync(part, 0, sizeof(double) * rows_gemm_sumsq_blocks(N), s));
   } else if (ng_pform_ok(Rp, in, wg_bytes)) {
-    int rc = ng_pform_pass(ng->W, Rp, Dp, bias, in, H, part, wg_ws, s);
+    int rc = ng_pform_pass(ng->W, Rp, Dp, bias, in, H, part, wg_ws, s, lp);
     if (rc) return rc;
   } else if (options().ng_valu && !in.active && ng_rowdot_ok(v)) {
     TDNNF_HIP(ng_rowdot(v, s));
   } else {
-    TDNNF_HIP(rows_gemm(ng_pass_gemm_args(ng->W, Dp, Rp, bias, in, H, Rp, part), true, s));
+    RowsGemmArgs a = ng_pass_gemm_args(ng->W, Dp, Rp, bias, in, H, Rp, part);
+    if (lp && lp->buf) {
+      a.lpart = lp->buf;
+      a.lpart_done = lp->done;
+    }
+    TDNNF_HIP(rows_gemm(a, true, s));
   }
   return stats_after_h(ng, in, H, wg_ws, wg_bytes, upd, s);
 }
@@ -218,14 +231,15 @@
   return rc;
 }
 
-int ng_stats_main(tdnnf_ng *ng, const NgInput &in, float *H, double *part, void *ws, size_t ws_bytes, hipStream_t s) {
+int ng_stats_main(tdnnf_ng *ng, const NgInput &in, float *H, double *part, void *ws, size_t ws_bytes, hipStream_t s, const NgLPart *lp) {
   const int K = in.ix.num_offsets;
   TDNNF_REQUIRE(ng && H && part && in.N > 0 && K >= 1 && K <= kMaxSeg && in.Di > 0, "ng_stats_main: bad arguments");
+  if (lp && lp->done) *lp->done = 0;
   NgCallScope scope;
   const NgFirstUse first{in, H, ws, ws_bytes};
   int rc = begin_call(ng, input_dim(in), &first, true, s);
   if (rc || ng->rank == 0) return rc;
-  return stats_main(ng, in, H, part, ws, ws_bytes, ng_updating(ng), s);
+  return stats_main(ng, in, H, part, ws, ws_bytes, ng_updating(ng), s, lp);
 }
 
 int ng_stats_main_prepare(tdnnf_ng *ng, const NgInput &in, float *H, double *part, hipStream_t s, RowsGemmArgs *out) {
diff --git a/tdnn-f_nas_amd/csrc/rows_gemm.hip b/tdnn-f_nas_amd/csrc/rows_gemm.hip
--- a/tdnn-f_nas_amd/csrc/rows_gemm.hip
+++ b/tdnn-f_nas_amd/csrc/rows_gemm.hip
@@ -291,12 +291,18 @@
     if (S > 16) S = 16;
     const size_t need = sizeof(float) * (size_t)S * a.M * ((a.N + 3) & ~3);
     if (S >= 2 && need <= scratch_bytes && tiles * S <= a.sumsq_cap) {
-      launch_split_k<WM, WN, TM, TN, BK>(a, tiles, 1, S, ktot, scratch, b_kc, vec, s);
+      RowsGemmArgs as = a;
+      as.lpart = nullptr;
+      launch_split_k<WM, WN, TM, TN, BK>(as, tiles, 1, S, ktot, scratch, b_kc, vec, s);
       count_rows_form<WM, WN, TM, TN, BK>(kFormSumsqSplitK);
       return hipGetLastError();
     }
   }
-  return launch_rows<WM, WN, TM, TN, BK>(a, b_kc, vec, s, kFormSumsqPlain);
+  RowsGemmArgs ap = a;
+  const bool l_in_pass = WN == 1 && TM == 1 && TN <= 3 && a.lpart && a.prec == 0 && a.init_mode != 0 && !a.add && !a.relu && a.N <= TN * 32;
+  if (!l_in_pass) ap.lpart = nullptr;
+  else if (a.lpart_done) *a.lpart_done = 1;
+  return launch_rows<WM, WN, TM, TN, BK>(ap, b_kc, vec, s, kFormSumsqPlain);
 }
 
 template <int WM, int WN, int TM, int TN, int BK>
@@ -502,6 +508,8 @@
 hipError_t rows_gemm(const RowsGemmArgs &a_in, bool b_kc, hipStream_t s) {
   if (a_in.M <= 0 || a_in.N <= 0 || a_in.nseg <= 0) return hipSuccess;
   RowsGemmArgs a = a_in;
+  if (a.lpart_done) *a.lpart_done = 0;
+  if (!a.sumsq) a.lpart = nullptr;
   a.c_vec = aligned16(a.C) && a.ldc % 4 == 0 && (a.init_mode != 1 || aligned16(a.bias)) && (!a.add || (aligned16(a.add) && a.ldadd % 4 == 0));
   const bool vec = operands_vec4(a);
   const int waste128 = ((a.N + 127) / 128) * 128 - a.N, waste160 = ((a.N + 159) / 160) * 160 - a.N;
@@ -614,6 +622,9 @@
     a.prec = 0;
     a.colstats = nullptr;
     a.colstats_rows = nullptr;
+    if (!(a.init_mode != 0 && !a.relu)) a.lpart = nullptr;
+    if (a.lpart_done) *a.lpart_done = a.lpart ? 1 : 0;
+    a.lpart_done = nullptr;
     a.alt_seg_order = options().gemm_alt_taps && is_two_tap_shift(a);
     prep[i] = a;
     first[i + 1] = first[i] + (a.M + 127) / 128;
diff --git a/tdnn-f_nas_amd/csrc/rows_gemm_kernels.h b/tdnn-f_nas_amd/csrc/rows_gemm_kernels.h
--- a/tdnn-f_nas_amd/csrc/rows_gemm_kernels.h
+++ b/tdnn-f_nas_amd/csrc/rows_gemm_kernels.h
@@ -2,6 +2,7 @@
 #include "common.h"
 #include "gemm_dev.h"
 #include "gemm_f32.h"
+#include "ng_l_tile.h"
 
 namespace tdnnf {
 namespace {
@@ -276,6 +277,27 @@
       for (int i = gx + t; i < p.sumsq_cap; i += 256) p.sumsq[i] = 0.0;
     __syncthreads();
   }
+  [[maybe_unused]] bool h_in_acc = false;
+  if constexpr (WN == 1 && TM == 1 && TN <= 3 && !POST) {
+    static_assert(SMEM_FLOATS >= kLTileLdsFloats, "the tile partial's images do not fit the staging LDS");
+    if (p.lpart && p.ksplit <= 1) {
+      h_in_acc = true;
+      const int row0 = m0 + wm * 32 + 4 * lh;
+#pragma unroll
+      for (int j = 0; j < TN; j++) {
+        const float bv = (p.init_mode == 1 && n0 + j * 32 + li < p.N) ? p.bias[n0 + j * 32 + li] : 0.f;
+#pragma unroll
+        for (int r = 0; r < 16; r++) acc[0][j][r] = row0 + (r & 3) + 8 * (r >> 2) < p.M ? acc[0][j][r] + bv : 0.f;
+      }
+      auto hval = [&](int c, int e) { return acc[0][c][e]; };
+      l_tile_partial<TN, f32x16>(hval, (p.N + 31) / 32, smem, p.lpart + (size_t)tile_m * l_tile_pairs(p.N) * 1024);
+      __syncthreads();
+    }
+  }
+  auto add_bias = [&]() {
+    if constexpr (WN == 1 && TM == 1 && TN <= 3 && !POST) return p.init_mode == 1 && !h_in_acc;
+    else return p.init_mode == 1;
+  };
   constexpr bool kColStats = 256 % (BN / 4) == 0 && (HALF * (BN / 4)) % 256 == 0;
   const bool colstats = kColStats && p.colstats && p.ksplit <= 1;
   float cs[4] = {0.f, 0.f, 0.f, 0.f}, cq[4] = {0.f, 0.f, 0.f, 0.f};
@@ -305,7 +327,7 @@
 #pragma unroll
         for (int u = 0; u < kGrp; u++) {
           const int idx = t + 256 * (g + u), m = m0 + pass * HALF + idx / (BN / 4), n = n0 + (idx % (BN / 4)) * 4;
-          const float *pp = p.init_mode == 0 ? p.C + (long long)m * p.ldc + n : (p.init_mode == 1 ? p.bias + n : zero);
+          const float *pp = p.init_mode == 0 ? p.C + (long long)m * p.ldc + n : (add_bias() ? p.bias + n : zero);
           const float *pa = (p.add && m >= p.add_lo && m < p.add_hi) ? p.add + (long long)(m - p.add_lo) * p.ldadd + n : zero;
           pre[u] = *reinterpret_cast<const float4 *>(pp);
           addv[u] = *reinterpret_cast<const float4 *>(pa);
@@ -361,7 +383,7 @@
       }
       float *c = p.C + (long long)m * p.ldc + n;
       if (cvec && n + 3 < p.N) {
-        if (p.init_mode == 1) {
+        if (add_bias()) {
           const float4 b = *reinterpret_cast<const float4 *>(p.bias + n);
           v.x += b.x; v.y += b.y; v.z += b.z; v.w += b.w;
         } else if (p.init_mode == 0) {
@@ -384,7 +406,7 @@
         for (int e = 0; e < 4; e++) {
           if (n + e < p.N) {
             float x = vv[e];
-            if (p.init_mode == 1) x += p.bias[n + e];
+            if (add_bias()) x += p.bias[n + e];
             else if (p.init_mode == 0) x += c[e];
             if (p.add && m >= p.add_lo && m < p.add_hi) x += p.add_scale * p.add[(long long)(m - p.add_lo) * p.ldadd + n + e];
             if (p.relu) x = floor_keep_nan(x, 0.f);
```

New measurement: 1.631 million. No clear change (-0.0%).
